# dongyangli-del/EEG_Image_decode

Hardware: AMD Instinct MI355X
Metric: EEG-CLIP contrastive train samples/sec (global batch) (higher is better)
Workload: dtype f32; 1 GPU; configs[1]: full ATM-S EEG encoder (63ch x 250t -> 1024-d) contrastive train step vs frozen 1024-d CLIP embeddings, 256 samples/GPU; global_batch=256, per_gpu_batch=256, parallelism=dp1, n_classes_for_accuracy=1654, optimizer=AdamW lr 3e-4 (fused)

## Files before the change

eeg_image_decode_amd/_abi.py:

```python
import ctypes as C

BIG = 1 << 62


class Dim(C.Structure):
    _fields_ = [("div", C.c_longlong), ("so", C.c_longlong), ("si", C.c_longlong)]


def dim(si, div=BIG, so=0):
    return Dim(int(div), int(so), int(si))


class GemmDesc(C.Structure):
    _fields_ = [
        ("M", C.c_int), ("N", C.c_int), ("K", C.c_int),
        ("A", C.c_void_p), ("Am", Dim), ("Ak", Dim),
        ("B", C.c_void_p), ("Bk", Dim), ("Bn", Dim),
        ("C", C.c_void_p), ("Cm", Dim), ("Cn", Dim),
        ("Cpre", C.c_void_p),
        ("bias_n", C.c_void_p), ("bias_m", C.c_void_p),
        ("R", C.c_void_p), ("Rm", Dim), ("Rn", Dim),
        ("alpha", C.c_float), ("accumulate", C.c_int), ("act", C.c_int),
        ("drop_p", C.c_float), ("seed", C.c_ulonglong), ("drop_site", C.c_uint),
        ("split_k", C.c_int),
        ("rowsum_a", C.c_void_p),
        ("precision", C.c_int),
        ("workspace", C.c_void_p), ("workspace_bytes", C.c_longlong),
    ]


class SplitItem(C.Structure):
    _fields_ = [("src", C.c_void_p), ("hi", C.c_void_p), ("lo", C.c_void_p), ("rows", C.c_int), ("cols", C.c_int), ("ld_src", C.c_longlong),
                ("ld_out", C.c_longlong), ("transpose", C.c_int), ("copy", C.c_void_p), ("ld_copy", C.c_longlong)]


class InfonceProblem(C.Structure):
    _fields_ = [("q_hi", C.c_void_p), ("q_lo", C.c_void_p), ("k_hi", C.c_void_p), ("k_lo", C.c_void_p), ("col0", C.c_int), ("weight", C.c_float),
                ("part", C.c_void_p), ("diag", C.c_void_p), ("lse", C.c_void_p), ("lse_k", C.c_void_p), ("G", C.c_void_p), ("ldg", C.c_longlong),
                ("part_k", C.c_void_p), ("diag_k", C.c_void_p), ("G_hi", C.c_void_p), ("G_lo", C.c_void_p)]


class TokenBlockDesc(C.Structure):
    _fields_ = ([("B", C.c_int), ("x", C.c_void_p), ("packed", C.c_void_p), ("bv", C.c_void_p), ("pe", C.c_void_p), ("tokens", C.c_void_p), ("ids", C.c_void_p)]
                + [(k, C.c_void_p) for k in ("bqkv", "bo", "ln1_g", "ln1_b", "b1", "b2", "ln2_g", "ln2_b", "ln3_g", "ln3_b")]
                + [(k, C.c_void_p) for k in ("h", "qkv", "r1", "mu1", "rs1", "f1", "r2", "n2", "mu2", "rs2", "n3", "mu3", "rs3")]
                + [(k, C.c_void_p) for k in ("xp", "hp", "ctxp", "n1p", "g1p")]
                + [("drop_p", C.c_float), ("eps", C.c_float), ("scale", C.c_float), ("seed", C.c_ulonglong)]
                + [(k, C.c_uint) for k in ("site_embed", "site_attn", "site_attn_out", "site_ffn_act", "site_ffn_out")]
                + [("packed_embed", C.c_void_p), ("embed_subject", C.c_void_p), ("bv_stride", C.c_longlong)]
                + [("cs_w25", C.c_void_p), ("cs_bias", C.c_void_p), ("cs_rows", C.c_void_p), ("cs_H", C.c_int)])


class TokenBlockBwdDesc(C.Structure):
    _fields_ = ([("B", C.c_int), ("packed", C.c_void_p)]
                + [(k, C.c_void_p) for k in ("dn3", "n2", "r2", "r1", "f1", "mu1", "rs1", "mu2", "rs2", "mu3", "rs3", "ln1_g", "ln2_g", "ln2_b", "ln3_g")]
                + [(k, C.c_void_p) for k in ("dr1", "dctx", "partials", "df2p", "dg1p", "da1p", "dr1p", "dqkvp")]
                + [(k, C.c_void_p) for k in ("dln3_g", "dln3_b", "dln2_g", "dln2_b", "dln1_g", "dln1_b")]
                + [("drop_p", C.c_float), ("seed", C.c_ulonglong)]
                + [(k, C.c_uint) for k in ("site_embed", "site_attn_out", "site_ffn_act", "site_ffn_out")])


class GemmPlanesDesc(C.Structure):
    _fields_ = [("a_hi", C.c_void_p), ("a_lo", C.c_void_p), ("b_hi", C.c_void_p), ("b_lo", C.c_void_p), ("lda", C.c_longlong), ("ldb", C.c_longlong),
                ("M", C.c_int), ("N", C.c_int), ("K", C.c_int), ("C", C.c_void_p), ("ldc", C.c_longlong), ("Cpre", C.c_void_p), ("ldcpre", C.c_longlong),
                ("bias", C.c_void_p), ("R", C.c_void_p), ("ldr", C.c_longlong), ("p_hi", C.c_void_p), ("p_lo", C.c_void_p), ("ldp", C.c_longlong),
                ("act", C.c_int), ("accumulate", C.c_int), ("planes_of", C.c_int)]


class HeadGemmDesc(C.Structure):
    _fields_ = [("a_hi", C.c_void_p), ("a_lo", C.c_void_p), ("b_hi", C.c_void_p), ("b_lo", C.c_void_p), ("lda", C.c_longlong), ("ldb", C.c_longlong),
                ("M", C.c_int), ("N", C.c_int), ("K", C.c_int), ("slices", C.c_int), ("slab_stride", C.c_longlong), ("bias", C.c_void_p),
                ("Cpre", C.c_void_p), ("ldcpre", C.c_longlong), ("act", C.c_int), ("aux", C.c_void_p), ("ldaux", C.c_longlong), ("R", C.c_void_p),
                ("ldr", C.c_longlong), ("C", C.c_void_p), ("ldc", C.c_longlong), ("p_hi", C.c_void_p), ("p_lo", C.c_void_p), ("ldp", C.c_longlong),
                ("b_kmajor", C.c_int)]


class Conv16Desc(C.Structure):
    _fields_ = [("in_", C.c_void_p), ("W", C.c_void_p), ("out", C.c_void_p), ("bias", C.c_void_p), ("residual", C.c_void_p),
                ("N", C.c_int), ("Hi", C.c_int), ("Wi", C.c_int), ("Cin", C.c_int), ("in_pad", C.c_int),
                ("Ho", C.c_int), ("Wo", C.c_int), ("Cout", C.c_int), ("out_pad", C.c_int),
                ("KS", C.c_int), ("stride", C.c_int), ("pad_top", C.c_int), ("pad_left", C.c_int), ("upsample", C.c_int), ("dtype", C.c_int),
                ("chan_bias", C.c_void_p)]


class Convt16Desc(C.Structure):
    _fields_ = [("in_", C.c_void_p), ("W", C.c_void_p), ("out", C.c_void_p), ("scale", C.c_void_p), ("shift", C.c_void_p),
                ("N", C.c_int), ("Hi", C.c_int), ("Wi", C.c_int), ("Cin", C.c_int), ("Ho", C.c_int), ("Wo", C.c_int), ("Cout", C.c_int),
                ("KS", C.c_int), ("stride", C.c_int), ("pad", C.c_int), ("relu", C.c_int), ("tap_mask", C.c_int), ("dtype", C.c_int)]


class Convt16BwdDataDesc(C.Structure):
    _fields_ = [("dz", C.c_void_p), ("W", C.c_void_p), ("dx", C.c_void_p), ("N", C.c_int), ("Hi", C.c_int), ("Wi", C.c_int), ("Cin", C.c_int), ("Cout", C.c_int),
                ("tap_mask", C.c_int), ("dtype", C.c_int)]


class Convt16BwdWeightDesc(C.Structure):
    _fields_ = [("x", C.c_void_p), ("dz", C.c_void_p), ("dW", C.c_void_p), ("db", C.c_void_p), ("workspace", C.c_void_p), ("workspace_floats", C.c_longlong),
                ("N", C.c_int), ("Hi", C.c_int), ("Wi", C.c_int), ("Cin", C.c_int), ("Cout", C.c_int), ("slabs", C.c_int), ("loss_scale", C.c_float),
                ("dtype", C.c_int)]


class Bn2d16FwdDesc(C.Structure):
    _fields_ = [("z", C.c_void_p), ("a", C.c_void_p), ("gamma", C.c_void_p), ("beta", C.c_void_p), ("mean", C.c_void_p), ("rstd", C.c_void_p),
                ("running_mean", C.c_void_p), ("running_var", C.c_void_p), ("workspace", C.c_void_p), ("workspace_floats", C.c_longlong), ("N", C.c_int), ("H", C.c_int), ("W", C.c_int), ("C", C.c_int),
                ("eps", C.c_float), ("momentum", C.c_float), ("dtype", C.c_int)]


class Bn2d16BwdDesc(C.Structure):
    _fields_ = [("da", C.c_void_p), ("a", C.c_void_p), ("z", C.c_void_p), ("gamma", C.c_void_p), ("mean", C.c_void_p), ("rstd", C.c_void_p), ("dgamma", C.c_void_p),
                ("dbeta", C.c_void_p), ("dz", C.c_void_p), ("workspace", C.c_void_p), ("workspace_floats", C.c_longlong), ("N", C.c_int), ("H", C.c_int), ("W", C.c_int), ("C", C.c_int),
                ("loss_scale", C.c_float), ("dtype", C.c_int)]


class WgradTokProblem(C.Structure):
    _fields_ = [("a", C.c_void_p), ("b", C.c_void_p), ("a_group_stride", C.c_longlong), ("m_groups", C.c_int), ("heads_m", C.c_int), ("heads_n", C.c_int),
                ("M", C.c_int), ("N", C.c_int), ("out", C.c_void_p), ("ldo", C.c_longlong), ("bias_out", C.c_void_p), ("bias_mfma", C.c_int),
                ("sample0", C.c_int), ("samples", C.c_int), ("sample_index", C.c_void_p)]


class CstackFwdDesc(C.Structure):
    _fields_ = [("B", C.c_int), ("H", C.c_int), ("x", C.c_void_p), ("xs_b", C.c_longlong), ("xs_h", C.c_longlong), ("w25", C.c_void_p), ("bias1", C.c_void_p),
                ("stat1", C.c_void_p), ("nstat1", C.c_int), ("count1", C.c_double), ("eps", C.c_float), ("momentum", C.c_float),
                ("gamma1", C.c_void_p), ("beta1", C.c_void_p), ("mean1", C.c_void_p), ("rstd1", C.c_void_p), ("run_mean1", C.c_void_p),
                ("run_var1", C.c_void_p), ("nbt1", C.c_void_p), ("packed", C.c_void_p), ("bias2", C.c_void_p), ("y2", C.c_void_p), ("stat2", C.c_void_p)]


class CstackBwdDesc(C.Structure):
    _fields_ = [("B", C.c_int), ("H", C.c_int), ("x", C.c_void_p), ("xs_b", C.c_longlong), ("xs_h", C.c_longlong), ("w25", C.c_void_p), ("bias1", C.c_void_p),
                ("mean1", C.c_void_p), ("rstd1", C.c_void_p), ("gamma1", C.c_void_p), ("beta1", C.c_void_p), ("packed_t", C.c_void_p), ("dy2", C.c_void_p),
                ("rows_out", C.c_void_p), ("stat", C.c_void_p), ("nstat", C.c_int), ("count", C.c_double), ("stat_local", C.c_void_p),
                ("nstat_local", C.c_int), ("dgamma", C.c_void_p), ("dbeta", C.c_void_p), ("dx", C.c_void_p), ("dw_partials", C.c_void_p), ("dw25", C.c_void_p)]


class WgradPlanesProblem(C.Structure):
    _fields_ = [("a_hi", C.c_void_p), ("a_lo", C.c_void_p), ("lda", C.c_longlong), ("b_hi", C.c_void_p), ("b_lo", C.c_void_p), ("ldb", C.c_longlong),
                ("rows", C.c_int), ("M", C.c_int), ("N", C.c_int), ("out", C.c_void_p), ("ldo", C.c_longlong), ("bias_out", C.c_void_p), ("slices", C.c_int)]


PLAN_MAX_ARGS = 28
PLAN_MEMSET, PLAN_JOIN, PLAN_SIDE, PLAN_SKIP, PLAN_SIDE2 = -2, -3, 1, 2, 4


class PlanArg(C.Union):
    _fields_ = [("p", C.c_void_p), ("i", C.c_longlong), ("u", C.c_ulonglong), ("d", C.c_double), ("f", C.c_float), ("i32", C.c_int), ("u32", C.c_uint)]


class PlanOp(C.Structure):
    _fields_ = [("fn", C.c_int), ("flags", C.c_int), ("a", PlanArg * PLAN_MAX_ARGS)]


ACT_NONE, ACT_GELU, ACT_SILU, ACT_GELU_GRAD = 0, 1, 2, 3
PREC_F32, PREC_BF16X3 = 0, 1
ABI_VERSION = 20
DT_BF16, DT_F16, DT_F32 = 0, 1, 2
SRC_U8_HWC, RESIZE_BILINEAR, RESIZE_BICUBIC = 3, 2, 3
_P, _I, _F, _L, _U64, _U, _D = C.c_void_p, C.c_int, C.c_float, C.c_longlong, C.c_ulonglong, C.c_uint, C.c_double

PROTOTYPES = {
    "eegclip_abi_version": [],
    "eegclip_gemm_f32": [C.POINTER(GemmDesc), _P],
    "eegclip_gemm_workspace_bytes": [C.POINTER(GemmDesc)],
    "eegclip_split_rows": [C.POINTER(SplitItem), _I, _P],
    "eegclip_gemm_f32_grouped": [_P, _I, _P],
    "eegclip_layernorm_fwd": [_P, _P, _P, _P, _P, _P, _I, _I, _F, _P],
    "eegclip_residual_layernorm_fwd": [_P, _P, _P, _F, _U64, _U, _P, _P, _P, _P, _P, _P, _P, _P, _P, _P, _I, _I, _F, _P],
    "eegclip_residual_layernorm_fwd_planes": [_P, _P, _P, _F, _U64, _U, _P, _P, _P, _P, _P, _P, _P, _P, _P, _P, _I, _I, _F, _P, _P, _P],
    "eegclip_layernorm_bwd": [_P, _P, _P, _P, _P, _P, _P, _P, _I, _I, _I, _P, _F, _U64, _U, _P],
    "eegclip_layernorm_bwd_full_workspace_floats": [_I, _I],
    "eegclip_layernorm_bwd_full": [_P, _P, _P, _P, _P, _P, _P, _P, _I, _I, _I, _P, _F, _U64, _U, _P, _P],
    "eegclip_layernorm_bwd_params_workspace_floats": [_I, _I],
    "eegclip_layernorm_bwd_params": [_P, _P, _P, _P, _P, _P, _I, _I, _P, _P],
    "eegclip_layernorm_silu_fwd": [_P, _P, _P, _P, _P, _P, _P, _I, _I, _F, _F, _U64, _U, _P],
    "eegclip_silu_bwd": [_P, _P, _P, _L, _I, _F, _U64, _U, _P],
    "eegclip_timestep_embedding": [_P, _I, _I, _P, _P],
    "eegclip_ddpm_add_noise": [_P, _P, _P, _P, _P, _P, _I, _I, _P],
    "eegclip_ddpm_step": [_P, _P, _P, _F, _F, _F, _F, _F, _F, _P, _P, _P, _L, _P],
    "eegclip_prior_stage_infer": [_P, _P, _P, _P, _P, _P, _P, _I, _P, _I, _I, _F, _P],
    "eegclip_mse_loss_grad": [_P, _P, _L, _P, _P, _P],
    "eegclip_mse_loss_grad_scaled": [_P, _P, _L, _F, _P, _P, _P],
    "eegclip_bn_stats": [_P, _I, _I, _I, _P, _P],
    "eegclip_bn_finalize": [_P, _D, _F, _F, _I, _P, _P, _P, _P, _I, _P, _P],
    "eegclip_bn_finalize_rows": [_P, _I, _D, _F, _F, _I, _P, _P, _P, _P, _P, _P, _P],
    "eegclip_bn_elu_fwd": [_P, _P, _P, _P, _P, _P, _I, _I, _I, _F, _U64, _U, _P],
    "eegclip_bn_elu_bwd": [_P, _P, _P, _P, _P, _P, _P, _P, _P, _P, _I, _I, _I, _F, _U64, _U, _P],
    "eegclip_bn_elu_bwd_stats": [_P, _P, _P, _P, _P, _P, _P, _I, _I, _I, _F, _U64, _U, _P],
    "eegclip_bn_elu_bwd_apply": [_P, _P, _P, _P, _P, _P, _P, _P, _D, _P, _P, _P, _I, _I, _I, _F, _U64, _U, _P],
    "eegclip_embed_finish": [_P, _P, _P, _I, _I, _I, _F, _U64, _U, _P],
    "eegclip_embed_finish_bwd": [_P, _P, _P, _I, _I, _I, _F, _U64, _U, _P],
    "eegclip_dropout_scale": [_P, _L, _F, _U64, _U, _P],
    "eegclip_gelu_bwd": [_P, _P, _P, _L, _I, _F, _U64, _U, _P],
    "eegclip_bias_act": [_P, _P, _P, _P, _P, _I, _I, _I, _F, _U64, _U, _P],
    "eegclip_axpby": [_P, _P, _L, _F, _F, _P],
    "eegclip_reduce_mid": [_P, _I, _I, _I, _P, _P],
    "eegclip_colsum_blocks": [_P, _I, _I, _I, _I, _L, _P, _P],
    "eegclip_sumsq": [_P, _L, _P, _P],
    "eegclip_stage_eeg": [_P, _P, _L, _I, _I, _I, _P, _I, _I, _P],
    "eegclip_gather_rows": [_P, _L, _P, _L, _P, _I, _I, _I, _P],
    "eegclip_adamw_step": [_P, _P, _P, _P, _L, _F, _F, _F, _F, _F, _L, _F, _P, _P],
    "eegclip_adamw_step_zero_grad": [_P, _P, _P, _P, _L, _F, _F, _F, _F, _F, _L, _F, _P, _P],
    "eegclip_clip_scale": [_P, _F, _P, _P],
    "eegclip_attention_fwd": [_P, _P, _I, _I, _I, _I, _I, _F, _F, _U64, _U, _P],
    "eegclip_attention_bwd": [_P, _P, _P, _I, _I, _I, _I, _I, _F, _F, _U64, _U, _P],
    "eegclip_attention_bwd_x3": [_P, _P, _P, _I, _I, _I, _I, _I, _I, _F, _F, _U64, _U, _P],
    "eegclip_proj1x1_fwd": [_P, _P, _P, _P, _P, _P, _P, _P, _P, _I, _F, _U64, _U, _P],
    "eegclip_proj1x1_fwd_rows": [_P, _P, _I, _D, _F, _F, _P, _P, _P, _P, _P, _P, _P, _P, _P, _P, _P, _I, _F, _U64, _U, _P],
    "eegclip_proj1x1_bwd_workspace_floats": [_I],
    "eegclip_proj1x1_bwd": [_P, _P, _P, _P, _P, _P, _P, _P, _P, _P, _P, _P, _P, _I, _F, _U64, _U, _P],
    "eegclip_cast_bf16": [_P, _P, _L, _P],
    "eegclip_logits_bf16": [_P, _P, _P, _I, _I, _I, _L, _P, _P],
    "eegclip_tsconv_fwd_workspace_floats": [_I, _I],
    "eegclip_tsconv_fwd": [_P, _L, _L, _P, _P, _P, _I, _I, _I, _I, _P, _P, _P],
    "eegclip_tsconv_bwd_w": [_P, _L, _L, _P, _P, _P, _I, _I, _I, _I, _P],
    "eegclip_tsconv_bwd_w_workspace_floats": [_I, _I],
    "eegclip_tsconv_bwd_x": [_P, _P, _P, _L, _L, _I, _I, _I, _I, _P],
    "eegclip_cross_attn_fwd": [_P, _P, _P, _P, _P, _P, _I, _I, _I, _I, _I, _I, _F, _I, _P],
    "eegclip_self_attn_supported": [_I, _L, _L, _L, _L],
    "eegclip_self_attn_fwd": [_P, _L, _P, _L, _P, _L, _P, _L, _I, _I, _I, _I, _I, _F, _I, _P],
    "eegclip_self_attn_causal_fwd": [_P, _L, _P, _L, _P, _L, _P, _L, _I, _I, _I, _I, _I, _F, _I, _P],
    "eegclip_self_attn_prefix_fwd": [_P, _L, _P, _L, _P, _L, _P, _L, _I, _I, _I, _I, _I, _F, _I, _P],
    "eegclip_attn80_supported": [_L, _L, _L, _L],
    "eegclip_attn80_fwd": [_P, _L, _P, _L, _P, _L, _P, _L, _I, _I, _I, _I, _F, _I, _P],
    "eegclip_gemm16_skinny": [_P, _L, _P, _L, _P, _L, _P, _P, _L, _I, _I, _I, _I, _I, _P],
    "eegclip_decode_attn16": [_P, _L, _P, _L, _L, _P, _L, _I, _I, _I, _I, _F, _I, _P],
    "eegclip_convt16": [C.POINTER(Convt16Desc), _P],
    "eegclip_convt16_pack_train": [_P, _P, _P, _I, _I, _I, _P],
    "eegclip_convt16_bwd_data": [C.POINTER(Convt16BwdDataDesc), _P],
    "eegclip_convt16_bwd_weight_slabs": [_I, _I, _I, _I, _I],
    "eegclip_convt16_bwd_weight_workspace_floats": [_I, _I, _I, _I, _I, _I],
    "eegclip_convt16_bwd_weight": [C.POINTER(Convt16BwdWeightDesc), _P],
    "eegclip_bn2d16_workspace_floats": [_I, _I, _I, _I],
    "eegclip_bn2d16_fwd": [C.POINTER(Bn2d16FwdDesc), _P],
    "eegclip_bn2d16_bwd": [C.POINTER(Bn2d16BwdDesc), _P],
    "eegclip_sconv_fwd": [_P, _P, _P, _P, _P, _P, _P, _P, _P, _I, _I, _I, _P, _P],
    "eegclip_sconv_fwd_workspace_floats": [_I],
    "eegclip_sconv_bwd_w_workspace_floats": [_I, _I],
    "eegclip_sconv_bwd_w": [_P, _P, _P, _P, _P, _P, _P, _P, _I, _I, _I, _P],
# ... 111 lines not shown
```

eeg_image_decode_amd/atms.py:

```python
import os
import weakref
import ctypes
import math

import numpy as np
import torch
import torch.nn as nn

from . import _abi
from ._lib import EegclipError, current_stream, lib, raw_stream, require_cuda
from .loss import ClipLoss
from .plan import Plan

D = _abi.dim
ACT_GELU = _abi.ACT_GELU
ACT_GELU_GRAD = _abi.ACT_GELU_GRAD

N_CH, T_LEN, D_MODEL, N_HEADS, D_HEAD, D_FF = 63, 250, 250, 4, 62, 256
L_TOK = N_CH + 1
HE = N_HEADS * D_HEAD
C_TS, W_TS, F_TS, P_DIM = 40, 36, 1440, 1024
EPS = 1e-5
SITE_EMBED, SITE_ATTN, SITE_ATTN_OUT, SITE_FFN_ACT, SITE_FFN_OUT, SITE_CONV, SITE_PROJ = range(7)

# ... 312 lines not shown
        self.n_subj = model.table_subjects if self.joint else 0
        self.ve_keys = [(_E + f"value_embedding.{s}.weight", _E + f"value_embedding.{s}.bias") for s in range(self.n_subj)]
        if self.joint:
            self.live_base = [k for k in _LIVE if ".value_embedding." not in k]
            live = self.live_base + [k for pair in self.ve_keys for k in pair]
        else:
            live = self.live_base = list(_LIVE)
        dead = [k for k in sd_params if k not in live and k not in (_TOK_TABLE, _TOK_SHARED)]
        order = live + [_TOK_TABLE, _TOK_SHARED] + dead
        assert sorted(order) == sorted(sd_params), "parameter list drifted from the reference state_dict"
        offs, off = {}, 0
        for k in order:
            offs[k] = off
            off += (sd_params[k].numel() + 3) // 4 * 4
        self.flat = torch.zeros(off, dtype=torch.float32, device=dev)
        self.gflat = torch.zeros(off, dtype=torch.float32, device=dev)
        self.anchor = torch.zeros(1, device=dev, requires_grad=True)
        self._clear_for = self._attached = None
        self._live_cache, self._attached_ptrs = {}, {}
        self.P, self.G, self.params = {}, {}, {}
        for k in order:
            p = sd_params[k]
            n = p.numel()
            view = self.flat[offs[k]:offs[k] + n].view(p.shape)
            view.copy_(p.data)
            p.data = view
            self.P[k] = view
            self.G[k] = self.gflat[offs[k]:offs[k] + n].view(p.shape)
            self.params[k] = p
            p._eegclip_grad_owner = weakref.ref(self)
        n_live = offs[_TOK_TABLE]
        self.segments = [(0, n_live, list(live)),
                         (offs[_TOK_TABLE], sd_params[_TOK_TABLE].numel(), [_TOK_TABLE]),
                         (offs[_TOK_SHARED], sd_params[_TOK_SHARED].numel(), [_TOK_SHARED]),
                         (offs[dead[0]] if dead else off, off - (offs[dead[0]] if dead else off), dead)]
        self.offs = offs
        a0, a1 = 0, offs["proj_eeg.2.bias"] + (sd_params["proj_eeg.2.bias"].numel() + 3) // 4 * 4
        assert offs["logit_scale"] == 0 and a1 == offs[self.live_base[self.live_base.index("proj_eeg.2.bias") + 1]]
        self.early_bucket = (a0, a1)
        self.early_work = None
        self._check = (self.params["logit_scale"], self.params[_CHECK_KEY])
        self.buffers = dict(model.named_buffers())
        self.bufs, self.plans, self.version = {}, {}, {}
        self.last_key = None
        self.grad_fresh = True
        lib()

    def _head_planes_enabled(self, pl):
        return pl.precision == _abi.PREC_BF16X3 and os.environ.get("EEGCLIP_HEAD_GEMM", "1") != "0"

    def _head_weight_planes(self):
        P = self.P
        w1, w2 = P["proj_eeg.0.weight"], P["proj_eeg.1.fn.1.weight"]
        span = (w2.data_ptr() - w1.data_ptr()) // 4 + w2.numel()
        assert w2.data_ptr() > w1.data_ptr() and span % 8 == 0 and span < 4 * w1.numel(), "projection-head weights are not adjacent in the flat buffer"
        if not hasattr(self, "hw_planes"):
            self.hw_planes = torch.empty(2, span, dtype=torch.bfloat16, device=self.device)
        o2 = (w2.data_ptr() - w1.data_ptr()) // 4
        self.hw = dict(w1=(_p(self.hw_planes[0]), _p(self.hw_planes[1])), w2=(_p(self.hw_planes[0]) + 2 * o2, _p(self.hw_planes[1]) + 2 * o2))
        return _abi.SplitItem(src=_p(w1), hi=_p(self.hw_planes[0]), lo=_p(self.hw_planes[1]), rows=1, cols=span, ld_src=span, ld_out=span, transpose=0)

    def _lean(self, pl, train, W):
        return bool(train and W == 1 and self._cstack_enabled(pl) and self._head_planes_enabled(pl))

    def _head_gemm(self, pl, b, tag, a_planes, K, w, N, B, kmajor=False):
        S = int(lib().eegclip_head_gemm_slices(B, N, K))
        if tag not in b or b[tag].shape != (S, B, N):
            b[tag] = torch.empty(S, B, N, dtype=torch.float32, device=self.device)
        pl.call_desc("eegclip_head_gemm", _abi.HeadGemmDesc(a_hi=a_planes[0], a_lo=a_planes[1], b_hi=w[0], b_lo=w[1], lda=K, ldb=N if kmajor else K, M=B, N=N, K=K,
                                                           slices=S, slab_stride=B * N, C=_p(b[tag]), ldc=N, b_kmajor=int(kmajor)))
        return _p(b[tag]), S, B * N

    def _token_block_enabled(self, pl):
        if self.joint and self.n_subj > WGRAD_TOK_MAX_PROBLEMS:
            return False
        return pl.precision == _abi.PREC_BF16X3 and os.environ.get("EEGCLIP_TOKEN_BLOCK", "1") != "0"

    def _token_planes(self, b, B, *names):
        for n in names:
            if n not in b:
                b[n] = torch.empty((3, B, 2, L_TOK, 256) if n == "dqkvp" else (B, 2, L_TOK, 256), dtype=torch.bfloat16, device=self.device)
        return [_p(b[n]) for n in names]

    def saved_f32(self, B, name):
        b = self.bufs[B]
        key = name + "p"
        if key not in b:
            return b[name]
        t = b[key].to(torch.float32)
        v = t[..., 0, :, :] + t[..., 1, :, :]
        if name in ("ctx", "dqkv"):
            v = v.reshape(*v.shape[:-1], N_HEADS, 64)[..., :D_HEAD].reshape(*v.shape[:-1], HE)
            if name == "dqkv":
                v = v.permute(1, 2, 0, 3).reshape(B * L_TOK, 3 * HE)
                return v
        else:
            v = v[..., :D_FF if name in ("g1", "dg1") else D_MODEL]
        return v.reshape(B * L_TOK, -1)

    def stale(self, model):
        a, b = self._check
        return (a.data_ptr() != self.flat.data_ptr() or b.data.data_ptr() != self.P[_CHECK_KEY].data_ptr()
                or model.logit_scale.device != self.device)

    def _alloc(self, B):
        dev = self.device

        def f(*s):
            return torch.empty(*s, dtype=torch.float32, device=dev)

        R = B * L_TOK
        b = dict(
            h=f(B, L_TOK, D_MODEL), qkv=f(R, 3 * HE), ctx=f(R, HE), r1=f(R, D_MODEL), n1=f(R, D_MODEL), mu1=f(R), rs1=f(R),
            f1=f(R, D_FF), g1=f(R, D_FF), r2=f(R, D_MODEL), n2=f(R, D_MODEL), mu2=f(R), rs2=f(R), n3=f(B, L_TOK, D_MODEL), mu3=f(R), rs3=f(R),
            z2=f(B, C_TS, W_TS),
            feat=f(B, F_TS), u=f(B, P_DIM), gu=f(B, P_DIM), s=f(B, P_DIM), out=f(B, P_DIM), mu4=f(B), rs4=f(B),
            bn=f(4, C_TS), ids=torch.zeros(B, dtype=torch.long, device=dev),
        )
        if self.joint:
            jmeta = torch.zeros(2 * B, dtype=torch.int32, device=dev)
            b.update(xs=f(B, N_CH, T_LEN), hs=f(B, L_TOK, D_MODEL), jmeta=jmeta, subj32=jmeta[:B], perm=jmeta[B:])
        nsum = 2 * 2 * C_TS
        ny2 = (B * C_TS * W_TS + 1) // 2
        nzf, nzb = nsum + B * P_DIM + ny2, nsum + (B * P_DIM + B * F_TS + 1) // 2
        zfb = torch.zeros(nzf + nzb, dtype=torch.float64, device=dev)
        zf, zb = zfb[:nzf], zfb[nzf:]
        sf, sb = zf[:nsum].view(2, 2 * C_TS), zb[:nsum].view(2, 2 * C_TS)
        zbf = zb[nsum:].view(torch.float32)
        b.update(zf=zf, zb=zb, zfb=zfb, zb_clean=True, sums=[sf[0], sf[1], sb[0], sb[1]], hacc=zf[nsum:nsum + B * P_DIM].view(torch.float32).view(2, B, P_DIM),
                 y2=zf[nsum + B * P_DIM:].view(torch.float32)[:B * C_TS * W_TS].view(B, C_TS, W_TS),
                 dgu=zbf[:B * P_DIM].view(B, P_DIM), dfeat=zbf[B * P_DIM:B * P_DIM + B * F_TS].view(B, F_TS))
        return b

    def _alloc_bwd(self, B, b):
        dev = self.device

        def f(*s):
            return torch.empty(*s, dtype=torch.float32, device=dev)

        R = B * L_TOK
        b.update(ds=f(B, P_DIM), dv=f(B, P_DIM), dz2=f(B, C_TS, W_TS), dy2=f(B, C_TS, W_TS),
                 dn3=torch.zeros(B, L_TOK, D_MODEL, dtype=torch.float32, device=dev),
                 dn2=f(R, D_MODEL), dr2=f(R, D_MODEL), df2=f(R, D_MODEL), dg1=f(R, D_FF), dr1=f(R, D_MODEL), da1=f(R, D_MODEL),
                 dctx=f(R, HE), dqkv=f(R, 3 * HE))

    def _build_fwd(self, B, train, shared, probs):
        P, b = self.P, self.bufs[B]
        pe_, pc_, pp_ = probs
        pl = Plan(f"atms_fwd[B={B}]")
        R = B * L_TOK
        pe = self.buffers[_E + "position_embedding.pe"]
        pl.tb_desc = None
        cstack = self._cstack_enabled(pl)
        head_planes = self._head_planes_enabled(pl)
        W = self._world() if train else 1
        lean = self._lean(pl, train, W)
        pl.lean = lean
        if cstack:
            if not lean:
                pl.memset(b["zfb"] if train else b["zf"], side=os.environ.get("EEGCLIP_START_SIDE", "1") != "0")
                pl.clears_zb = train
            if not hasattr(self, "cs_packed"):
                self.cs_packed = torch.empty(int(lib().eegclip_cstack_packed_bytes(N_CH)) // 2, dtype=torch.bfloat16, device=self.device)
                self.cs_packed_t = torch.empty(int(lib().eegclip_cstack_packed_t_bytes(N_CH)) // 2, dtype=torch.bfloat16, device=self.device)
            cs_prep = (_p(P[_TS + "4.weight"]), _p(self.cs_packed), _p(self.cs_packed_t), N_CH)
            if not self._token_block_enabled(pl):
                pl.call("eegclip_cstack_pack_all", *cs_prep)
        if self._token_block_enabled(pl):
            if not hasattr(self, "tb_packed"):
                self.tb_packed = torch.empty(int(lib().eegclip_token_block_packed_bytes()) // 2, dtype=torch.bfloat16, device=self.device)
            ve_w0, ve_b0 = (self.ve_keys[0] if self.joint else (_E + "value_embedding.weight", _E + "value_embedding.bias"))
            tb_prep = (_p(P[ve_w0]), _p(P[_LY + "attention.query_projection.weight"]), _p(P[_LY + "attention.out_projection.weight"]),
                       _p(P[_LY + "conv1.weight"]), _p(P[_LY + "conv2.weight"]), _p(self.tb_packed))
            if cstack:
                pl.call("eegclip_weight_prep", *tb_prep, *cs_prep)
            else:
                pl.call("eegclip_token_block_pack", *tb_prep)
            joint_args = {}
            if self.joint:
                ve_stride = (P[self.ve_keys[1][0]].data_ptr() - P[ve_w0].data_ptr()) // 4 if self.n_subj > 1 else D_MODEL * T_LEN
                assert all(P[w].data_ptr() - P[ve_w0].data_ptr() == 4 * ve_stride * i and P[bk].data_ptr() - P[ve_b0].data_ptr() == 4 * ve_stride * i
                           for i, (w, bk) in enumerate(self.ve_keys)), "value embeddings are not equally spaced in the flat buffer"
                if not hasattr(self, "tb_packed_embed"):
                    self.tb_packed_embed = torch.empty(int(lib().eegclip_token_block_packed_embed_bytes(self.n_subj)) // 2, dtype=torch.bfloat16,
                                                       device=self.device)
                pl.call("eegclip_token_block_pack_embed", _p(P[ve_w0]), ve_stride, self.n_subj, _p(self.tb_packed_embed))
                joint_args = dict(packed_embed=_p(self.tb_packed_embed), embed_subject=_p(b["subj32"]), bv_stride=ve_stride)
            tok = P[_TOK_SHARED] if shared else P[_TOK_TABLE]
            xp, hp, ctxp, n1p, g1p = self._token_planes(b, B, "xp", "hp", "ctxp", "n1p", "g1p")
            stats_args = {}
            pl.stats1_in_block = bool(cstack and train and os.environ.get("EEGCLIP_STATS1_TAIL", "1") != "0")
            if pl.stats1_in_block:
                if "cs_rows" not in b:
                    b["cs_rows"] = torch.empty(2, B, 2 * C_TS, dtype=torch.float64, device=self.device)
                stats_args = dict(cs_w25=_p(P[_TS + "0.weight"]), cs_bias=_p(P[_TS + "0.bias"]), cs_rows=_p(b["cs_rows"][0]), cs_H=N_CH)
            pl.tb_desc = pl.call_desc("eegclip_token_block_fwd", _abi.TokenBlockDesc(
                B=B, x=0, packed=_p(self.tb_packed), bv=_p(P[ve_b0]), pe=_p(pe), tokens=_p(tok), ids=None if shared else _p(b["ids"]), **joint_args, **stats_args,
                bqkv=_p(P[_LY + "attention.query_projection.bias"]), bo=_p(P[_LY + "attention.out_projection.bias"]), ln1_g=_p(P[_LY + "norm1.weight"]),
                ln1_b=_p(P[_LY + "norm1.bias"]), b1=_p(P[_LY + "conv1.bias"]), b2=_p(P[_LY + "conv2.bias"]), ln2_g=_p(P[_LY + "norm2.weight"]),
                ln2_b=_p(P[_LY + "norm2.bias"]), ln3_g=_p(P["encoder.encoder.norm.weight"]), ln3_b=_p(P["encoder.encoder.norm.bias"]),
                h=_p(b["h"]), qkv=_p(b["qkv"]), r1=_p(b["r1"]), mu1=_p(b["mu1"]), rs1=_p(b["rs1"]), f1=_p(b["f1"]),
                r2=_p(b["r2"]), n2=None, mu2=_p(b["mu2"]), rs2=_p(b["rs2"]), n3=_p(b["n3"]), mu3=_p(b["mu3"]), rs3=_p(b["rs3"]),
                xp=xp, hp=hp, ctxp=ctxp, n1p=n1p, g1p=g1p,
                drop_p=pe_, eps=EPS, scale=1.0 / math.sqrt(D_HEAD), seed=0, site_embed=SITE_EMBED, site_attn=SITE_ATTN, site_attn_out=SITE_ATTN_OUT,
                site_ffn_act=SITE_FFN_ACT, site_ffn_out=SITE_FFN_OUT), seeded=pe_ > 0.0)
        else:
            hmap = D(D_MODEL, div=N_CH, so=L_TOK * D_MODEL)
            if not self.joint:
                pl.x_gemm = pl.gemm(B * N_CH, D_MODEL, T_LEN, 0, D(T_LEN), D(1), _p(P[_E + "value_embedding.weight"]), D(1), D(T_LEN),
                        _p(b["h"]) + 4 * D_MODEL, hmap, D(1), bias_n=_p(P[_E + "value_embedding.bias"]),
                        R=_p(pe), Rm=D(D_MODEL, div=N_CH, so=0), Rn=D(1))
            else:
                XR = N_CH * T_LEN
                pl.j_gather = len(pl.ops)
                pl.call("eegclip_gather_rows", _p(b["xs"]), XR, 0, XR, _p(b["perm"]), B, XR, 0)
                pl.j_gemm = [pl.desc(N_CH, D_MODEL, T_LEN, 0, D(T_LEN), D(1), _p(P[w]), D(1), D(T_LEN), 0, hmap, D(1), bias_n=_p(P[bk]),
                                     R=_p(pe), Rm=D(D_MODEL, div=N_CH, so=0), Rn=D(1)) for w, bk in self.ve_keys]
                pl.j_arr, pl.j_group = pl.gemm_grouped(self.n_subj)
                pl.j_scatter = len(pl.ops)
                pl.call("eegclip_gather_rows", _p(b["h"]) + 4 * D_MODEL, L_TOK * D_MODEL, _p(b["hs"]) + 4 * D_MODEL, L_TOK * D_MODEL, _p(b["perm"]), B,
                        N_CH * D_MODEL, 1)
            tok = P[_TOK_SHARED] if shared else P[_TOK_TABLE]
            pl.call("eegclip_embed_finish", _p(b["h"]), _p(tok), None if shared else _p(b["ids"]), B, L_TOK, D_MODEL, pe_, 0, SITE_EMBED, seed_at=7)
            pl.gemm(R, 3 * HE, D_MODEL, _p(b["h"]), D(D_MODEL), D(1), _p(P[_LY + "attention.query_projection.weight"]), D(1), D(D_MODEL),
                    _p(b["qkv"]), D(3 * HE), D(1), bias_n=_p(P[_LY + "attention.query_projection.bias"]))
            pl.call("eegclip_attention_fwd", _p(b["qkv"]), _p(b["ctx"]), B, L_TOK, N_HEADS, D_HEAD, 3 * HE, 1.0 / math.sqrt(D_HEAD), pe_, 0,
                    SITE_ATTN, seed_at=9)
            pl.gemm(R, D_MODEL, HE, _p(b["ctx"]), D(HE), D(1), _p(P[_LY + "attention.out_projection.weight"]), D(1), D(HE),
                    _p(b["r1"]), D(D_MODEL), D(1), bias_n=_p(P[_LY + "attention.out_projection.bias"]))
            pl.call("eegclip_residual_layernorm_fwd", _p(b["r1"]), _p(b["h"]), _p(b["r1"]), pe_, 0, SITE_ATTN_OUT, _p(P[_LY + "norm1.weight"]),
                    _p(P[_LY + "norm1.bias"]), _p(b["n1"]), _p(b["mu1"]), _p(b["rs1"]), None, None, None, None, None, R, D_MODEL, EPS, seed_at=4)
            pl.gemm(R, D_FF, D_MODEL, _p(b["n1"]), D(D_MODEL), D(1), _p(P[_LY + "conv1.weight"]), D(1), D(D_MODEL), _p(b["g1"]), D(D_FF), D(1),
                    Cpre=_p(b["f1"]), bias_n=_p(P[_LY + "conv1.bias"]), act=ACT_GELU, drop_p=pe_, drop_site=SITE_FFN_ACT)
            pl.gemm(R, D_MODEL, D_FF, _p(b["g1"]), D(D_FF), D(1), _p(P[_LY + "conv2.weight"]), D(1), D(D_FF), _p(b["r2"]), D(D_MODEL), D(1),
                    bias_n=_p(P[_LY + "conv2.bias"]))
            pl.call("eegclip_residual_layernorm_fwd", _p(b["r2"]), _p(b["n1"]), _p(b["r2"]), pe_, 0, SITE_FFN_OUT, _p(P[_LY + "norm2.weight"]),
                    _p(P[_LY + "norm2.bias"]), _p(b["n2"]), _p(b["mu2"]), _p(b["rs2"]), _p(P["encoder.encoder.norm.weight"]),
                    _p(P["encoder.encoder.norm.bias"]), _p(b["n3"]), _p(b["mu3"]), _p(b["rs3"]), R, D_MODEL, EPS, seed_at=4)
        sums, bn = b["sums"], b["bn"]
        bn2_rows = None
        if cstack:
            if not lean:
                pl.join()
            bn2_rows = self._build_fwd_cstack(pl, b, B, train, W)
        else:
            pl.memset(b["zfb"] if train else b["zf"])
            pl.clears_zb = train
            self._build_fwd_conv_y1(pl, b, B, train, W)
        run2 = (_p(self.buffers[_TS + "5.running_mean"]), _p(self.buffers[_TS + "5.running_var"]), _p(self.buffers[_TS + "5.num_batches_tracked"]))
        if head_planes:
            if "featp" not in b:
                b["featp_buf"] = torch.zeros(2 * B * F_TS + 128, dtype=torch.bfloat16, device=self.device)
                b["featp"] = b["featp_buf"][:2 * B * F_TS].view(2, B, F_TS)
                b["gup"] = torch.empty(2, B, P_DIM, dtype=torch.bfloat16, device=self.device)
            rows_args = (_p(bn2_rows), B, float(B * W_TS), EPS, 0.1, _p(bn[2]), _p(bn[3]), *run2) if bn2_rows is not None else \
                (None, 0, 1.0, EPS, 0.1, _p(bn[2]), _p(bn[3]), None, None, None)
            pl.rider_items = (_abi.SplitItem * 4)()
            pl.rider_items[0] = self._head_weight_planes()
            pl._keep.append(pl.rider_items)
            pl.rider_op = len(pl.ops)
            pl.call("eegclip_proj1x1_fwd_rows_planes", _p(b["y2"]), *rows_args, _p(P[_TS + "5.weight"]), _p(P[_TS + "5.bias"]),
                    _p(P["enc_eeg.0.projection.0.weight"]), _p(P["enc_eeg.0.projection.0.bias"]), _p(b["z2"]), _p(b["feat"]), B, pc_, 0, SITE_CONV,
                    _p(b["featp"][0]), _p(b["featp"][1]), pl.rider_items, 1, seed_at=19)
        elif bn2_rows is not None:
            pl.call("eegclip_proj1x1_fwd_rows", _p(b["y2"]), _p(bn2_rows), B, float(B * W_TS), EPS, 0.1, _p(bn[2]), _p(bn[3]), *run2,
                    _p(P[_TS + "5.weight"]), _p(P[_TS + "5.bias"]), _p(P["enc_eeg.0.projection.0.weight"]), _p(P["enc_eeg.0.projection.0.bias"]),
                    _p(b["z2"]), _p(b["feat"]), B, pc_, 0, SITE_CONV, seed_at=19)
        else:
            pl.call("eegclip_proj1x1_fwd", _p(b["y2"]), _p(bn[2]), _p(bn[3]), _p(P[_TS + "5.weight"]), _p(P[_TS + "5.bias"]),
                    _p(P["enc_eeg.0.projection.0.weight"]), _p(P["enc_eeg.0.projection.0.bias"]), _p(b["z2"]), _p(b["feat"]), B, pc_, 0, SITE_CONV,
                    seed_at=11)
        pl.head_planes = head_planes
        if head_planes:
            fp, gp = (_p(b["featp"][0]), _p(b["featp"][1])), (_p(b["gup"][0]), _p(b["gup"][1]))
            fused_epi = os.environ.get("EEGCLIP_HEAD_FUSED_EPI", "0") == "1"
            if fused_epi:
                pl.call_desc("eegclip_head_gemm", _abi.HeadGemmDesc(a_hi=fp[0], a_lo=fp[1], b_hi=self.hw["w1"][0], b_lo=self.hw["w1"][1], lda=F_TS, ldb=F_TS, M=B,
                                                                   N=P_DIM, K=F_TS, slices=1, slab_stride=0, bias=_p(P["proj_eeg.0.bias"]), Cpre=_p(b["u"]),
                                                                   ldcpre=P_DIM, act=ACT_GELU, C=_p(b["gu"]), ldc=P_DIM, p_hi=gp[0], p_lo=gp[1], ldp=P_DIM))
            else:
                sl1 = self._head_gemm(pl, b, "hslab1", fp, F_TS, self.hw["w1"], P_DIM, B)
                pl.call("eegclip_head_act", *sl1, _p(P["proj_eeg.0.bias"]), _p(b["u"]), _p(b["gu"]), *gp, B, P_DIM)
            sl2 = self._head_gemm(pl, b, "hslab2", gp, P_DIM, self.hw["w2"], P_DIM, B)
            pl.out_op = len(pl.ops)
            pl.call("eegclip_residual_layernorm_fwd_slabs", sl2[0], _p(b["u"]), _p(b["s"]), pp_, 0, SITE_PROJ, _p(P["proj_eeg.2.weight"]),
                    _p(P["proj_eeg.2.bias"]), 0, _p(b["mu4"]), _p(b["rs4"]), None, None, None, None, None, B, P_DIM, EPS, None, None, sl2[1], sl2[2],
                    _p(P["proj_eeg.1.fn.1.bias"]), seed_at=4)
            return pl
        skh = _head_split(B)
        if skh > 1:
            pl.gemm(B, P_DIM, F_TS, _p(b["feat"]), D(F_TS), D(1), _p(P["proj_eeg.0.weight"]), D(1), D(F_TS), _p(b["hacc"][0]), D(P_DIM), D(1),
                    accumulate=1, split_k=skh)
            pl.call("eegclip_bias_act", _p(b["hacc"][0]), _p(P["proj_eeg.0.bias"]), _p(b["u"]), None, _p(b["gu"]), B, P_DIM, ACT_GELU, 0.0, 0, 0)
            pl.gemm(B, P_DIM, P_DIM, _p(b["gu"]), D(P_DIM), D(1), _p(P["proj_eeg.1.fn.1.weight"]), D(1), D(P_DIM), _p(b["hacc"][1]), D(P_DIM), D(1),
                    bias_n=_p(P["proj_eeg.1.fn.1.bias"]), accumulate=1, split_k=skh)
            w_lin = b["hacc"][1]
        else:
            pl.gemm(B, P_DIM, F_TS, _p(b["feat"]), D(F_TS), D(1), _p(P["proj_eeg.0.weight"]), D(1), D(F_TS), _p(b["gu"]), D(P_DIM), D(1),
                    Cpre=_p(b["u"]), bias_n=_p(P["proj_eeg.0.bias"]), act=ACT_GELU)
            pl.gemm(B, P_DIM, P_DIM, _p(b["gu"]), D(P_DIM), D(1), _p(P["proj_eeg.1.fn.1.weight"]), D(1), D(P_DIM), _p(b["s"]), D(P_DIM), D(1),
                    bias_n=_p(P["proj_eeg.1.fn.1.bias"]))
            w_lin = b["s"]
        pl.out_op = len(pl.ops)
        pl.call("eegclip_residual_layernorm_fwd", _p(w_lin), _p(b["u"]), _p(b["s"]), pp_, 0, SITE_PROJ, _p(P["proj_eeg.2.weight"]),
                _p(P["proj_eeg.2.bias"]), 0, _p(b["mu4"]), _p(b["rs4"]), None, None, None, None, None, B, P_DIM, EPS, seed_at=4)
        return pl
# ... 126 lines not shown
                pl.call_desc("eegclip_head_gemm", _abi.HeadGemmDesc(a_hi=vp[0], a_lo=vp[1], b_hi=self.hw["w2"][0], b_lo=self.hw["w2"][1], lda=P_DIM, ldb=P_DIM, M=B,
                                                                   N=P_DIM, K=P_DIM, slices=1, slab_stride=0, act=ACT_GELU_GRAD, aux=_p(b["u"]), ldaux=P_DIM,
                                                                   R=_p(b["ds"]), ldr=P_DIM, C=_p(b["ds"]), ldc=P_DIM, p_hi=up[0], p_lo=up[1], ldp=P_DIM, b_kmajor=1))
            else:
                sl = self._head_gemm(pl, b, "dgu_slabs", vp, P_DIM, self.hw["w2"], P_DIM, B, kmajor=True)
                pl.call("eegclip_head_act_bwd", *sl, _p(b["u"]), _p(b["ds"]), _p(b["ds"]), *up, B * P_DIM)
            if wplanes:
                gp_, fp_ = (_p(b["gup"][0]), _p(b["gup"][1])), (_p(b["featp"][0]), _p(b["featp"][1]))
                probs = (_abi.WgradPlanesProblem * 2)(
                    _abi.WgradPlanesProblem(a_hi=vp[0], a_lo=vp[1], lda=P_DIM, b_hi=gp_[0], b_lo=gp_[1], ldb=P_DIM, rows=B, M=P_DIM, N=P_DIM,
                                            out=_p(G["proj_eeg.1.fn.1.weight"]), ldo=P_DIM, bias_out=_p(G["proj_eeg.1.fn.1.bias"]), slices=1),
                    _abi.WgradPlanesProblem(a_hi=up[0], a_lo=up[1], lda=P_DIM, b_hi=fp_[0], b_lo=fp_[1], ldb=F_TS, rows=B, M=P_DIM, N=F_TS,
                                            out=_p(G["proj_eeg.0.weight"]), ldo=F_TS, bias_out=_p(G["proj_eeg.0.bias"]), slices=1))
                pl._keep.append(probs)
                later(lambda: pl.call("eegclip_wgrad_planes", probs, 2, side=head_side))
            else:
                later(lambda: wgrad("proj_eeg.0.weight", _p(b["ds"]), P_DIM, _p(b["feat"]), F_TS, P_DIM, F_TS, B, bias="proj_eeg.0.bias"))
            dfeat_slabs = self._head_gemm(pl, b, "dfeat_slabs", up, P_DIM, self.hw["w1"], F_TS, B, kmajor=True)
        else:
            head_side_ops = []
            self._build_bwd_head_f32(pl, b, B, pp_, ln_side, wgrad)
        W = self._world() if train else 1
        zsum = None
        if not train:
            zsum = torch.zeros(2 * C_TS, dtype=torch.float64, device=self.device)
            pl._keep.append(zsum)

            def conv_bias_grad(bias_key, gamma_key, rstd, s):
                return lambda: G[bias_key].add_((P[gamma_key] * rstd * s[:C_TS].to(torch.float32)))
        if "pj_ws" not in b:
            b["pj_ws"] = torch.empty(int(lib().eegclip_proj1x1_bwd_workspace_floats(B)) // 2, dtype=torch.float64, device=self.device)
        lean = dfeat_slabs is not None and self._lean(pl, train, W)
        pl.lean = lean
        if lean:
            if "pj_bn_rows" not in b:
                b["pj_bn_rows"] = torch.empty(B, 2 * C_TS, dtype=torch.float64, device=self.device)
            pl.call("eegclip_proj1x1_bwd_rows", *dfeat_slabs, _p(b["z2"]), _p(P["enc_eeg.0.projection.0.weight"]), _p(b["y2"]), _p(bn[2]), _p(bn[3]),
                    _p(P[_TS + "5.weight"]), _p(P[_TS + "5.bias"]), _p(b["dz2"]), _p(b["pj_ws"]), _p(b["pj_bn_rows"]), B, pc_, 0, SITE_CONV, seed_at=15)
            pl.call("eegclip_bn_elu_bwd_apply_rows", _p(b["dz2"]), _p(b["y2"]), _p(bn[2]), _p(bn[3]), _p(P[_TS + "5.weight"]), _p(P[_TS + "5.bias"]),
                    _p(b["pj_bn_rows"]), B, 2 * C_TS, 0, float(B * W_TS),
                    _p(b["dy2"]), _p(G[_TS + "5.weight"]), _p(G[_TS + "5.bias"]), B, C_TS, W_TS, pc_, 0, SITE_CONV, seed_at=18)
            for f in head_side_ops:
                f()
            pl.call("eegclip_proj1x1_bwd_reduce", _p(b["pj_ws"]), B, _p(G["enc_eeg.0.projection.0.weight"]), _p(G["enc_eeg.0.projection.0.bias"]), None, side=True)
        else:
            if dfeat_slabs is not None:
                pl.call("eegclip_proj1x1_bwd_slabs", *dfeat_slabs, _p(b["z2"]), _p(P["enc_eeg.0.projection.0.weight"]), _p(b["y2"]), _p(bn[2]), _p(bn[3]),
                        _p(P[_TS + "5.weight"]), _p(P[_TS + "5.bias"]), _p(b["dz2"]), _p(G["enc_eeg.0.projection.0.weight"]),
                        _p(G["enc_eeg.0.projection.0.bias"]), _p(sums[2]), _p(b["pj_ws"]), B, pc_, 0, SITE_CONV, seed_at=17)
            else:
                pl.call("eegclip_proj1x1_bwd", _p(b["dfeat"]), _p(b["z2"]), _p(P["enc_eeg.0.projection.0.weight"]), _p(b["y2"]), _p(bn[2]), _p(bn[3]),
                        _p(P[_TS + "5.weight"]), _p(P[_TS + "5.bias"]), _p(b["dz2"]), _p(G["enc_eeg.0.projection.0.weight"]),
                        _p(G["enc_eeg.0.projection.0.bias"]), _p(sums[2]), _p(b["pj_ws"]), B, pc_, 0, SITE_CONV, seed_at=15)
            local2 = None
            if W > 1:
                local2 = torch.zeros_like(sums[2])
                pl._keep.append(local2)

                def exchange2():
                    local2.copy_(sums[2])
                    self._allreduce(sums[2])
                pl.callback(exchange2, "allreduce_bn2_bwd")
            if not train:
                pl.callback(conv_bias_grad(_TS + "4.bias", _TS + "5.weight", bn[3], sums[2]), "conv2_bias_grad_eval")
            pl.call("eegclip_bn_elu_bwd_apply", _p(b["dz2"]), _p(b["y2"]), _p(bn[2]), _p(bn[3]), _p(P[_TS + "5.weight"]), _p(P[_TS + "5.bias"]),
                    _p(sums[2]) if train else _p(zsum), (_p(local2) if local2 is not None else None) if train else _p(sums[2]), float(W * B * W_TS), _p(b["dy2"]), _p(G[_TS + "5.weight"]), _p(G[_TS + "5.bias"]), B, C_TS,
                    W_TS, pc_, 0, SITE_CONV, seed_at=16)
            for f in head_side_ops:
                f()
        if self._cstack_bwd_enabled(pl):
            self._build_bwd_cstack(pl, b, B, train, W, zsum, conv_bias_grad if not train else None, early_reduce, defer_small)
        else:
            self._build_bwd_conv_y1(pl, b, B, train, W, zsum, conv_bias_grad if not train else None, early_reduce)
        fused = self._token_block_enabled(pl) and hasattr(self, "tb_packed")
        if fused:
            if "tb_part" not in b:
                b["tb_part"] = torch.empty(int(lib().eegclip_token_block_bwd_workspace_floats(B)), dtype=torch.float32, device=self.device)
            df2p, dg1p, da1p, dr1p, dqkvp = self._token_planes(b, B, "df2p", "dg1p", "da1p", "dr1p", "dqkvp")
            xp, hp, ctxp, n1p, g1p = self._token_planes(b, B, "xp", "hp", "ctxp", "n1p", "g1p")
            bd = _abi.TokenBlockBwdDesc(
                B=B, packed=_p(self.tb_packed), dn3=_p(b["dn3"]), n2=None, r2=_p(b["r2"]), r1=_p(b["r1"]), f1=_p(b["f1"]), mu1=_p(b["mu1"]),
                rs1=_p(b["rs1"]), mu2=_p(b["mu2"]), rs2=_p(b["rs2"]), mu3=_p(b["mu3"]), rs3=_p(b["rs3"]), ln1_g=_p(P[_LY + "norm1.weight"]),
                ln2_g=_p(P[_LY + "norm2.weight"]), ln2_b=_p(P[_LY + "norm2.bias"]), ln3_g=_p(P["encoder.encoder.norm.weight"]),
                dr1=_p(b["dr1"]), dctx=_p(b["dctx"]), partials=_p(b["tb_part"]), df2p=df2p, dg1p=dg1p, da1p=da1p, dr1p=dr1p, dqkvp=dqkvp,
                dln3_g=_p(G["encoder.encoder.norm.weight"]), dln3_b=_p(G["encoder.encoder.norm.bias"]), dln2_g=_p(G[_LY + "norm2.weight"]),
                dln2_b=_p(G[_LY + "norm2.bias"]), dln1_g=_p(G[_LY + "norm1.weight"]), dln1_b=_p(G[_LY + "norm1.bias"]),
                drop_p=pe_, seed=0, site_embed=SITE_EMBED, site_attn_out=SITE_ATTN_OUT, site_ffn_act=SITE_FFN_ACT, site_ffn_out=SITE_FFN_OUT)
            pl._keep.append(bd)
            if pe_ > 0.0:
                pl._seed_descs.append(bd)
            variant = 0

            def wgrad_tok(tag, problems, side=True, slices=None, index=None):
                arr = (_abi.WgradTokProblem * len(problems))()
                for i, (name, a, mg, x, M, N, hm, hn, bias, bm) in enumerate(problems):
                    arr[i] = _abi.WgradTokProblem(a=a, b=x, a_group_stride=B * 65536 if mg > 1 else 0, m_groups=mg, heads_m=hm, heads_n=hn, M=M, N=N,
                                                  out=_p(G[name]), ldo=N, bias_out=_p(G[bias]) if bias else None, bias_mfma=bm, sample_index=index)
                groups = sum(q[2] for q in problems)
                slices = slices or (wsk if wsk > 0 else int(lib().eegclip_wgrad_tok_slices(groups, B)))
                key = "wk:" + tag
                if key not in b:
                    b[key] = torch.empty(int(lib().eegclip_wgrad_tok_workspace_floats(arr, len(problems), B, slices)), dtype=torch.float32, device=self.device)
                pl._keep.append(arr)
                ops = (len(pl.ops), len(pl.ops) + 1)
                pl.call("eegclip_wgrad_tok", arr, len(problems), B, slices, _p(b[key]), variant, side=side)
                pl.call("eegclip_wgrad_tok_reduce", arr, len(problems), B, slices, _p(b[key]), side=side)
                return arr, ops

            merge = int(os.environ.get("EEGCLIP_WGRAD_MERGE", "2"))
            late = []
            ffn_out = [
                (_LY + "conv2.weight", df2p, 1, g1p, D_MODEL, D_FF, 0, 0, _LY + "conv2.bias", 1),
                (_LY + "conv1.weight", dg1p, 1, n1p, D_FF, D_MODEL, 0, 0, _LY + "conv1.bias", 0),
                (_LY + "attention.out_projection.weight", da1p, 1, ctxp, D_MODEL, HE, 0, 1, _LY + "attention.out_projection.bias", 0)]
            qkv_w = [(_LY + "attention.query_projection.weight", dqkvp, 3, hp, 3 * HE, D_MODEL, 1, 0, _LY + "attention.query_projection.bias", 0)]
            pl.call("eegclip_token_block_bwd", ctypes.byref(bd), 0)
            if defer_small:
                pl.deferred.append(lambda: pl.call("eegclip_token_block_bwd", ctypes.byref(bd), 2, side=True))
            else:
                pl.call("eegclip_token_block_bwd", ctypes.byref(bd), 2, side=ln_side)
            if merge >= 2:
                late += ffn_out
            else:
                wgrad_tok("ffn_out", ffn_out)
            pl.call(attn_bwd, _p(b["qkv"]), _p(b["dctx"]), dqkvp, 1, B, L_TOK, N_HEADS, D_HEAD, 3 * HE, 1.0 / math.sqrt(D_HEAD),
                    pe_, 0, SITE_ATTN, seed_at=11)
            if merge >= 1:
                late += qkv_w
            else:
                wgrad_tok("qkv", qkv_w)
            pl.call("eegclip_token_block_bwd", ctypes.byref(bd), 1)
        else:
            pl.call("eegclip_layernorm_bwd_full", _p(b["dn3"]), _p(b["n2"]), _p(P["encoder.encoder.norm.weight"]), _p(b["mu3"]), _p(b["rs3"]), _p(b["dn2"]),
                    _p(G["encoder.encoder.norm.weight"]), _p(G["encoder.encoder.norm.bias"]), R, D_MODEL, 0, None, 0.0, 0, 0, lnf_ws)
            pl.call("eegclip_layernorm_bwd_full", _p(b["dn2"]), _p(b["r2"]), _p(P[_LY + "norm2.weight"]), _p(b["mu2"]), _p(b["rs2"]), _p(b["dr2"]),
                    _p(G[_LY + "norm2.weight"]), _p(G[_LY + "norm2.bias"]), R, D_MODEL, 0, _p(b["df2"]), pe_, 0, SITE_FFN_OUT, lnf_ws, seed_at=13)
            wgrad(_LY + "conv2.weight", _p(b["df2"]), D_MODEL, _p(b["g1"]), D_FF, D_MODEL, D_FF, R, bias=_LY + "conv2.bias")
            pl.gemm(R, D_FF, D_MODEL, _p(b["df2"]), D(D_MODEL), D(1), _p(P[_LY + "conv2.weight"]), D(D_FF), D(1), _p(b["dg1"]), D(D_FF), D(1),
                    act=ACT_GELU_GRAD, R=_p(b["f1"]), Rm=D(D_FF), Rn=D(1), drop_p=pe_, drop_site=SITE_FFN_ACT)
            wgrad(_LY + "conv1.weight", _p(b["dg1"]), D_FF, _p(b["n1"]), D_MODEL, D_FF, D_MODEL, R, bias=_LY + "conv1.bias")
            pl.gemm(R, D_MODEL, D_FF, _p(b["dg1"]), D(D_FF), D(1), _p(P[_LY + "conv1.weight"]), D(D_MODEL), D(1), _p(b["dr2"]), D(D_MODEL), D(1),
                    accumulate=1)
            pl.call("eegclip_layernorm_bwd_full", _p(b["dr2"]), _p(b["r1"]), _p(P[_LY + "norm1.weight"]), _p(b["mu1"]), _p(b["rs1"]), _p(b["dr1"]),
                    _p(G[_LY + "norm1.weight"]), _p(G[_LY + "norm1.bias"]), R, D_MODEL, 0, _p(b["da1"]), pe_, 0, SITE_ATTN_OUT, lnf_ws, seed_at=13)
            wgrad(_LY + "attention.out_projection.weight", _p(b["da1"]), D_MODEL, _p(b["ctx"]), HE, D_MODEL, HE, R,
                  bias=_LY + "attention.out_projection.bias")
            pl.gemm(R, HE, D_MODEL, _p(b["da1"]), D(D_MODEL), D(1), _p(P[_LY + "attention.out_projection.weight"]), D(HE), D(1), _p(b["dctx"]), D(HE), D(1))
            if attn_bwd == "eegclip_attention_bwd_x3":
                pl.call(attn_bwd, _p(b["qkv"]), _p(b["dctx"]), _p(b["dqkv"]), 0, B, L_TOK, N_HEADS, D_HEAD, 3 * HE, 1.0 / math.sqrt(D_HEAD),
                        pe_, 0, SITE_ATTN, seed_at=11)
            else:
                pl.call(attn_bwd, _p(b["qkv"]), _p(b["dctx"]), _p(b["dqkv"]), B, L_TOK, N_HEADS, D_HEAD, 3 * HE, 1.0 / math.sqrt(D_HEAD),
                        pe_, 0, SITE_ATTN, seed_at=10)
            wgrad(_LY + "attention.query_projection.weight", _p(b["dqkv"]), 3 * HE, _p(b["h"]), D_MODEL, 3 * HE, D_MODEL, R,
                  bias=_LY + "attention.query_projection.bias")
            pl.gemm(R, D_MODEL, 3 * HE, _p(b["dqkv"]), D(3 * HE), D(1), _p(P[_LY + "attention.query_projection.weight"]), D(D_MODEL), D(1),
                    _p(b["dr1"]), D(D_MODEL), D(1), accumulate=2, drop_p=pe_, drop_site=SITE_EMBED)
        tokg = G[_TOK_SHARED] if shared else G[_TOK_TABLE]
        pl.call("eegclip_embed_finish_bwd", _p(b["dr1"]), _p(tokg), None if shared else _p(b["ids"]), B, L_TOK, D_MODEL, 0.0, 0, SITE_EMBED, side=True)
        for f in pl.deferred:
            f()
        hmap = D(D_MODEL, div=N_CH, so=L_TOK * D_MODEL)
        if want_dx:
            b["dx"] = torch.empty(B, N_CH, T_LEN, dtype=torch.float32, device=self.device)
        pl.x_gemm = None
        if fused:
            if not self.joint:
                wgrad_tok("embed" + ("+%d" % len(late) if late else ""), late + [(_E + "value_embedding.weight", dr1p, 1, xp, D_MODEL, T_LEN, 0, 0, _E + "value_embedding.bias", 0)], side=False)
            else:
                if late:
                    wgrad_tok("block", late, side=False)
                pl.j_wk_template = [(w, dr1p, 1, xp, D_MODEL, T_LEN, 0, 0, bk, 0) for w, bk in self.ve_keys]
                pl.j_wk_slices = [0] + [max(1, min(32, 2 * B // 4, (64 // n) // 8 * 8 if 64 // n >= 8 else 64 // n)) for n in range(1, self.n_subj + 1)]
                pl.j_wk_arr, pl.j_wk_ops = wgrad_tok("embed_joint", pl.j_wk_template, side=False, slices=8, index=_p(b["perm"]))
                need = max(int(lib().eegclip_wgrad_tok_workspace_floats(pl.j_wk_arr, n, B, pl.j_wk_slices[n])) for n in range(1, self.n_subj + 1))
                if b["wk:embed_joint"].numel() < need:
                    b["wk:embed_joint"] = torch.empty(need, dtype=torch.float32, device=self.device)
                    for op in pl.j_wk_ops:
                        pl.set_arg(op, 4, _p(b["wk:embed_joint"]))
                pl.j_wk_all = (_abi.WgradTokProblem * self.n_subj)(*pl.j_wk_arr)
                pl._keep.append(pl.j_wk_all)
        elif not self.joint:
            pl.x_gemm = pl.gemm(D_MODEL, T_LEN, B * N_CH, _p(b["dr1"]) + 4 * D_MODEL, D(1), hmap, 0, D(T_LEN), D(1),
                    _p(G[_E + "value_embedding.weight"]), D(T_LEN), D(1), accumulate=1, split_k=sk(B * N_CH),
                    rowsum_a=_p(G[_E + "value_embedding.bias"]))
        if not self.joint:
            if want_dx:
                pl.gemm(B * N_CH, T_LEN, D_MODEL, _p(b["dr1"]) + 4 * D_MODEL, hmap, D(1),
                        _p(P[_E + "value_embedding.weight"]), D(T_LEN), D(1), _p(b["dx"]), D(T_LEN), D(1))
        elif fused and not want_dx:
            pass
        else:
            XR = N_CH * T_LEN
            pl.j_gather = len(pl.ops)
            pl.call("eegclip_gather_rows", _p(b["hs"]) + 4 * D_MODEL, L_TOK * D_MODEL, _p(b["dr1"]) + 4 * D_MODEL, L_TOK * D_MODEL, _p(b["perm"]), B,
                    N_CH * D_MODEL, 0)
            if not fused:
                pl.j_gemm = [pl.desc(D_MODEL, T_LEN, N_CH, 0, D(1), hmap, 0, D(T_LEN), D(1), _p(G[w]), D(T_LEN), D(1), accumulate=1, split_k=1,
                                     rowsum_a=_p(G[bk])) for w, bk in self.ve_keys]
                pl.j_arr, pl.j_group = pl.gemm_grouped(self.n_subj)
            if want_dx:
                b["dxs"] = torch.empty(B, N_CH, T_LEN, dtype=torch.float32, device=self.device)
                pl.j_dx = [pl.desc(N_CH, T_LEN, D_MODEL, 0, hmap, D(1), _p(P[w]), D(T_LEN), D(1), 0, D(T_LEN), D(1)) for w, _ in self.ve_keys]
                pl.j_dx_arr, pl.j_dx_group = pl.gemm_grouped(self.n_subj)
                pl.j_scatter = len(pl.ops)
                pl.call("eegclip_gather_rows", _p(b["dx"]), XR, _p(b["dxs"]), XR, _p(b["perm"]), B, XR, 1)
        return pl

    def _build_bwd_head_f32(self, pl, b, B, pp_, ln_side, wgrad):
        P, G = self.P, self.G
        pl.call("eegclip_layernorm_bwd", 0, _p(b["s"]), _p(P["proj_eeg.2.weight"]), _p(b["mu4"]), _p(b["rs4"]), _p(b["ds"]),
                None, None, B, P_DIM, 0, _p(b["dv"]), pp_, 0, SITE_PROJ, seed_at=13)
        pl.dout_par_op = len(pl.ops)
        pl.call("eegclip_layernorm_bwd", 0, _p(b["s"]), None, _p(b["mu4"]), _p(b["rs4"]), None,
                _p(G["proj_eeg.2.weight"]), _p(G["proj_eeg.2.bias"]), B, P_DIM, 0, None, 0.0, 0, 0, side=ln_side)
        wgrad("proj_eeg.1.fn.1.weight", _p(b["dv"]), P_DIM, _p(b["gu"]), P_DIM, P_DIM, P_DIM, B, bias="proj_eeg.1.fn.1.bias")
        skh = _head_split(B)
        pl.gemm(B, P_DIM, P_DIM, _p(b["dv"]), D(P_DIM), D(1), _p(P["proj_eeg.1.fn.1.weight"]), D(P_DIM), D(1), _p(b["dgu"]), D(P_DIM), D(1),
                accumulate=int(skh > 1), split_k=skh)
        pl.call("eegclip_gelu_bwd", _p(b["dgu"]), _p(b["u"]), _p(b["ds"]), B * P_DIM, 1, 0.0, 0, 0)
        wgrad("proj_eeg.0.weight", _p(b["ds"]), P_DIM, _p(b["feat"]), F_TS, P_DIM, F_TS, B, bias="proj_eeg.0.bias")
        pl.gemm(B, F_TS, P_DIM, _p(b["ds"]), D(P_DIM), D(1), _p(P["proj_eeg.0.weight"]), D(F_TS), D(1), _p(b["dfeat"]), D(F_TS), D(1),
                accumulate=int(skh > 1), split_k=skh)

    def _build_bwd_cstack(self, pl, b, B, train, W, zsum, conv_bias_grad, early_reduce, defer_small=False):
# ... 275 lines not shown
```

eeg_image_decode_amd/csrc/attention_x3.hip:

```cpp
#include "eeg_common.h"

namespace eeg {

constexpr int AX_L = 64;
constexpr int AX_RS = 144;
constexpr int AX_PLANE = AX_L * AX_RS;
constexpr int AX_TENSOR = 2 * AX_PLANE;

struct ax_args {
    const float* qkv;
    const float* dctx;
    float* dqkv;
    unsigned char* dqkvp;
    int B, H, E, ld;
    float scale, drop_p;
    unsigned long long seed;
    unsigned site;
};

typedef float ax_f2 __attribute__((ext_vector_type(2)));
typedef float ax_f4u __attribute__((ext_vector_type(4), aligned(4)));

__device__ __forceinline__ bf16x8 ax_tr_frag(const unsigned char* plane, int r0, int r1, int c0, int lane) {
    const int l = lane & 15;
    const s16x4 a = lds_read_tr16(plane + (r0 + (l >> 2)) * AX_RS + 2 * (c0 + 4 * (l & 3)));
    const s16x4 b = lds_read_tr16(plane + (r1 + (l >> 2)) * AX_RS + 2 * (c0 + 4 * (l & 3)));
    return bf16x8{a[0], a[1], a[2], a[3], b[0], b[1], b[2], b[3]};
}
__device__ __forceinline__ bf16x8 ax_frag(const unsigned char* plane, int row, int k0) {
    return *reinterpret_cast<const bf16x8*>(plane + row * AX_RS + 2 * k0);
}
__device__ __forceinline__ bf16x8 ax_pack8(u32x2_t a, u32x2_t b) {
    typedef unsigned u4 __attribute__((ext_vector_type(4)));
    const u4 v{a[0], a[1], b[0], b[1]};
    return __builtin_bit_cast(bf16x8, v);
}
__device__ __forceinline__ f32x4 ax_mfma3(bf16x8 ah, bf16x8 al, bf16x8 bh, bf16x8 bl, f32x4 c) {
    c = mfma_bf16_16x16x32(al, bh, c);
    c = mfma_bf16_16x16x32(ah, bl, c);
    return mfma_bf16_16x16x32(ah, bh, c);
}
__device__ __forceinline__ void ax_store4(float* p, int valid, f32x4 v) {
    if (valid >= 4) *reinterpret_cast<ax_f4u*>(p) = ax_f4u{v[0], v[1], v[2], v[3]};
    else if (valid >= 2) {
        *reinterpret_cast<ax_f2*>(p) = ax_f2{v[0], v[1]};
        if (valid == 3) p[2] = v[2];
    } else if (valid == 1) p[0] = v[0];
}

__device__ __forceinline__ void ax_store4_planes(unsigned char* row_base, int e0, f32x4 v) {
    u32x2_t hi, lo;
    x3_split4(v[0], v[1], v[2], v[3], hi, lo);
    *reinterpret_cast<u32x2_t*>(row_base + 2 * e0) = hi;
    *reinterpret_cast<u32x2_t*>(row_base + 32768 + 2 * e0) = lo;
}

template <bool TRAIN>
__global__ __launch_bounds__(256, 2) void attention_bwd_x3_kernel(const ax_args a) {
    EEG_LDS_BASE(float, ldsf);
    unsigned char* lds = reinterpret_cast<unsigned char*>(ldsf);
    unsigned char* Qp = lds;
    unsigned char* Kp = lds + AX_TENSOR;
    unsigned char* Vp = lds + 2 * AX_TENSOR;
    unsigned char* Op = lds + 3 * AX_TENSOR;
    const int t = threadIdx.x, lane = t & 63, w = wave_uniform(t >> 6), fr = lane & 15, g = lane >> 4;
    const int bh = blockIdx.x, b = bh / a.H, h = bh - b * a.H;
    const int E = a.E, HE = a.H * E;
    const float* qrow0 = a.qkv + (long long)b * AX_L * a.ld + h * E;
    const float* orow0 = a.dctx + (long long)b * AX_L * HE + h * E;

    {
        ax_f2 v[4][8];
#pragma unroll
        for (int j = 0; j < 8; ++j) {
            const int idx = t + 256 * j, row = idx >> 5, col = 2 * (idx & 31);
            const bool ok = col < E;
            const float* qr = qrow0 + (long long)row * a.ld + col;
            v[0][j] = ok ? *reinterpret_cast<const ax_f2*>(qr) : ax_f2{0.f, 0.f};
            v[1][j] = ok ? *reinterpret_cast<const ax_f2*>(qr + HE) : ax_f2{0.f, 0.f};
            v[2][j] = ok ? *reinterpret_cast<const ax_f2*>(qr + 2 * HE) : ax_f2{0.f, 0.f};
            v[3][j] = ok ? *reinterpret_cast<const ax_f2*>(orow0 + (long long)row * HE + col) : ax_f2{0.f, 0.f};
        }
#pragma unroll
        for (int x = 0; x < 4; ++x)
#pragma unroll
            for (int j = 0; j < 8; ++j) {
                const int idx = t + 256 * j, row = idx >> 5, col = 2 * (idx & 31);
                const unsigned hi = x3_pack2(v[x][j][0], v[x][j][1]);
                const float r0 = v[x][j][0] - __uint_as_float(hi << 16), r1 = v[x][j][1] - __uint_as_float(hi & 0xffff0000u);
                unsigned char* dst = lds + x * AX_TENSOR + row * AX_RS + 2 * col;
                *reinterpret_cast<unsigned*>(dst) = hi;
                *reinterpret_cast<unsigned*>(dst + AX_PLANE) = x3_pack2(r0, r1);
            }
    }
    __syncthreads();

    f32x4 s[4], dp[4];
#pragma unroll
    for (int kt = 0; kt < 4; ++kt) { s[kt] = f32x4{0.f, 0.f, 0.f, 0.f}; dp[kt] = f32x4{0.f, 0.f, 0.f, 0.f}; }
#pragma unroll
    for (int ks = 0; ks < 2; ++ks) {
        const int k0 = 32 * ks + 8 * g;
        const bf16x8 qh = ax_frag(Qp, 16 * w + fr, k0), ql = ax_frag(Qp + AX_PLANE, 16 * w + fr, k0);
        const bf16x8 oh = ax_frag(Op, 16 * w + fr, k0), ol = ax_frag(Op + AX_PLANE, 16 * w + fr, k0);
#pragma unroll
        for (int kt = 0; kt < 4; ++kt) {
            const bf16x8 kh = ax_frag(Kp, 16 * kt + fr, k0), kl = ax_frag(Kp + AX_PLANE, 16 * kt + fr, k0);
            const bf16x8 vh = ax_frag(Vp, 16 * kt + fr, k0), vl = ax_frag(Vp + AX_PLANE, 16 * kt + fr, k0);
            s[kt] = ax_mfma3(kh, kl, qh, ql, s[kt]);
            dp[kt] = ax_mfma3(vh, vl, oh, ol, dp[kt]);
        }
    }
    float mx = -INFINITY;
#pragma unroll
    for (int kt = 0; kt < 4; ++kt)
#pragma unroll
        for (int r = 0; r < 4; ++r) {
            s[kt][r] *= a.scale;
            mx = fmaxf(mx, s[kt][r]);
        }
    mx = fmaxf(mx, __shfl_xor(mx, 16, 64));
    mx = fmaxf(mx, __shfl_xor(mx, 32, 64));
    float sum = 0.f;
#pragma unroll
    for (int kt = 0; kt < 4; ++kt)
#pragma unroll
        for (int r = 0; r < 4; ++r) {
            s[kt][r] = expf(s[kt][r] - mx);
            sum += s[kt][r];
        }
    sum += __shfl_xor(sum, 16, 64);
    sum += __shfl_xor(sum, 32, 64);
    const float inv = 1.0f / sum;
    const bool drop = TRAIN && a.drop_p > 0.f;
    const float ksc = drop ? 1.f / (1.f - a.drop_p) : 1.f;
    f32x4 pd[4];
    float dq_sum = 0.f;
#pragma unroll
    for (int kt = 0; kt < 4; ++kt) {
        bool keep[4] = {true, true, true, true};
        if (drop) {
            const unsigned long long idx0 = ((unsigned long long)bh * AX_L + 16 * w + fr) * AX_L + 16 * kt + 4 * g;
            dropout_keep4(a.seed, a.site, idx0, a.drop_p, keep);
        }
#pragma unroll
        for (int r = 0; r < 4; ++r) {
            const float p = s[kt][r] * inv;
            const float d = keep[r] ? dp[kt][r] * ksc : 0.f;
            pd[kt][r] = keep[r] ? p * ksc : 0.f;
            s[kt][r] = p;
            dp[kt][r] = d;
            dq_sum += p * d;
        }
    }
    dq_sum += __shfl_xor(dq_sum, 16, 64);
    dq_sum += __shfl_xor(dq_sum, 32, 64);
#pragma unroll
    for (int kt = 0; kt < 4; ++kt)
#pragma unroll
        for (int r = 0; r < 4; ++r) dp[kt][r] = s[kt][r] * (dp[kt][r] - dq_sum);

    {
        f32x4 dq[4];
#pragma unroll
        for (int et = 0; et < 4; ++et) dq[et] = f32x4{0.f, 0.f, 0.f, 0.f};
#pragma unroll
        for (int m = 0; m < 2; ++m) {
            u32x2_t h0, l0, h1, l1;
            x3_split4(dp[2 * m][0], dp[2 * m][1], dp[2 * m][2], dp[2 * m][3], h0, l0);
            x3_split4(dp[2 * m + 1][0], dp[2 * m + 1][1], dp[2 * m + 1][2], dp[2 * m + 1][3], h1, l1);
            const bf16x8 bhf = ax_pack8(h0, h1), blf = ax_pack8(l0, l1);
#pragma unroll
            for (int et = 0; et < 4; ++et) {
                const bf16x8 ah = ax_tr_frag(Kp, 32 * m + 4 * g, 32 * m + 16 + 4 * g, 16 * et, lane);
                const bf16x8 al = ax_tr_frag(Kp + AX_PLANE, 32 * m + 4 * g, 32 * m + 16 + 4 * g, 16 * et, lane);
                dq[et] = ax_mfma3(ah, al, bhf, blf, dq[et]);
            }
        }
        float* out = a.dqkv + ((long long)b * AX_L + 16 * w + fr) * a.ld + h * E;
        unsigned char* outp = a.dqkvp + (long long)b * 65536 + (16 * w + fr) * 512 + 128 * h;
#pragma unroll
        for (int et = 0; et < 4; ++et) {
            const int e0 = 16 * et + 4 * g;
            f32x4 v = dq[et];
#pragma unroll
            for (int r = 0; r < 4; ++r) v[r] *= a.scale;
            if (a.dqkvp) ax_store4_planes(outp, e0, v);
            else if (e0 < E) ax_store4(out + e0, E - e0, v);
        }
    }
    __syncthreads();
#pragma unroll
    for (int kt = 0; kt < 4; ++kt) {
        u32x2_t hi, lo;
        const int off = (16 * w + fr) * AX_RS + 2 * (16 * kt + 4 * g);
        x3_split4(pd[kt][0], pd[kt][1], pd[kt][2], pd[kt][3], hi, lo);
        *reinterpret_cast<u32x2_t*>(Kp + off) = hi;
        *reinterpret_cast<u32x2_t*>(Kp + AX_PLANE + off) = lo;
        x3_split4(dp[kt][0], dp[kt][1], dp[kt][2], dp[kt][3], hi, lo);
        *reinterpret_cast<u32x2_t*>(Vp + off) = hi;
        *reinterpret_cast<u32x2_t*>(Vp + AX_PLANE + off) = lo;
    }
    __syncthreads();

    f32x4 dv[4], dk[4];
#pragma unroll
    for (int et = 0; et < 4; ++et) { dv[et] = f32x4{0.f, 0.f, 0.f, 0.f}; dk[et] = f32x4{0.f, 0.f, 0.f, 0.f}; }
#pragma unroll
    for (int ks = 0; ks < 2; ++ks) {
        const int q0 = 32 * ks + 8 * g;
        const bf16x8 ph = ax_tr_frag(Kp, q0, q0 + 4, 16 * w, lane), pl = ax_tr_frag(Kp + AX_PLANE, q0, q0 + 4, 16 * w, lane);
        const bf16x8 sh = ax_tr_frag(Vp, q0, q0 + 4, 16 * w, lane), sl = ax_tr_frag(Vp + AX_PLANE, q0, q0 + 4, 16 * w, lane);
#pragma unroll
        for (int et = 0; et < 4; ++et) {
            const bf16x8 oh = ax_tr_frag(Op, q0, q0 + 4, 16 * et, lane), ol = ax_tr_frag(Op + AX_PLANE, q0, q0 + 4, 16 * et, lane);
            const bf16x8 qh = ax_tr_frag(Qp, q0, q0 + 4, 16 * et, lane), ql = ax_tr_frag(Qp + AX_PLANE, q0, q0 + 4, 16 * et, lane);
            dv[et] = ax_mfma3(oh, ol, ph, pl, dv[et]);
            dk[et] = ax_mfma3(qh, ql, sh, sl, dk[et]);
        }
    }
    if (a.dqkvp) {
        const long long grp = (long long)a.B * 65536;
        unsigned char* outp = a.dqkvp + (long long)b * 65536 + (16 * w + fr) * 512 + 128 * h;
#pragma unroll
        for (int et = 0; et < 4; ++et) {
            const int e0 = 16 * et + 4 * g;
            f32x4 v = dk[et];
#pragma unroll
            for (int r = 0; r < 4; ++r) v[r] *= a.scale;
            ax_store4_planes(outp + grp, e0, v);
            ax_store4_planes(outp + 2 * grp, e0, dv[et]);
        }
        return;
    }
    float* outk = a.dqkv + ((long long)b * AX_L + 16 * w + fr) * a.ld + HE + h * E;
#pragma unroll
    for (int et = 0; et < 4; ++et) {
        const int e0 = 16 * et + 4 * g;
        if (e0 < E) {
            f32x4 v = dk[et];
#pragma unroll
            for (int r = 0; r < 4; ++r) v[r] *= a.scale;
            ax_store4(outk + e0, E - e0, v);
            ax_store4(outk + HE + e0, E - e0, dv[et]);
        }
    }
}

}

using namespace eeg;

extern "C" int eegclip_attention_bwd_x3(const float* qkv, const float* dctx, void* dqkv, int dqkv_planes, int B, int L, int H, int E, int ld, float scale,
                                        float drop_p, unsigned long long seed, unsigned site, void* stream) {
    if (dqkv_planes && (H > 4 || (reinterpret_cast<uintptr_t>(dqkv) & 15u))) return dqkv && H <= 4 ? EEGCLIP_EALIGN : EEGCLIP_EINVAL;
    if (!qkv || !dctx || !dqkv || B < 1 || L != AX_L || H < 1 || E < 2 || E > 64 || (E & 1) || (ld & 1) || ld < 3 * H * E || drop_p < 0.f || drop_p >= 1.f)
        return EEGCLIP_EINVAL;
    if ((reinterpret_cast<uintptr_t>(qkv) | reinterpret_cast<uintptr_t>(dctx) | reinterpret_cast<uintptr_t>(dqkv)) & 7u) return EEGCLIP_EALIGN;
    const ax_args a{qkv, dctx, dqkv_planes ? nullptr : static_cast<float*>(dqkv), dqkv_planes ? static_cast<unsigned char*>(dqkv) : nullptr, B, H, E, ld, scale,
                    drop_p, seed, site};
    const size_t lds = 4 * AX_TENSOR;
    if (drop_p > 0.f) EEG_LAUNCH(attention_bwd_x3_kernel<true>, dim3(B * H), dim3(256), lds, stream, a);
    else              EEG_LAUNCH(attention_bwd_x3_kernel<false>, dim3(B * H), dim3(256), lds, stream, a);
    return (int)hipGetLastError();
}
```

eeg_image_decode_amd/csrc/token_block.hip:

```cpp
#include "cstack_common.h"

#include <stdio.h>
#include <stdlib.h>

namespace eeg {

constexpr int TB_THREADS = 512;
constexpr int TB_L = 64, TB_D = 250, TB_T = 250, TB_NCH = 63, TB_H = 4, TB_E = 62, TB_HE = 248, TB_FF = 256;
constexpr int TB_AP_PLANE = 64 * 512;
constexpr int TB_AP_BYTES = 2 * TB_AP_PLANE;
constexpr int TB_XF_BYTES = 64 * 1024;
constexpr int TB_HQ_PLANE = 64 * 128;
constexpr int TB_HQ_BYTES = 6 * TB_HQ_PLANE;
constexpr int TB_LDS = TB_AP_BYTES + 2 * TB_HQ_BYTES;
constexpr int TB_KS = 8;
constexpr int TB_TILE = 1024;
constexpr int TB_NT_V = 16, TB_NT_QKV = 48, TB_NT_O = 16, TB_NT_1 = 16, TB_NT_2 = 16;
constexpr int TB_NMAT = 11;
constexpr long long TB_OFF_V = 0;
constexpr long long TB_OFF_QKV = TB_OFF_V + (long long)TB_NT_V * TB_KS * TB_TILE;
constexpr long long TB_OFF_O = TB_OFF_QKV + (long long)TB_NT_QKV * TB_KS * TB_TILE;
constexpr long long TB_OFF_1 = TB_OFF_O + (long long)TB_NT_O * TB_KS * TB_TILE;
constexpr long long TB_OFF_2 = TB_OFF_1 + (long long)TB_NT_1 * TB_KS * TB_TILE;
constexpr long long TB_MAT_ELEMS = 16LL * TB_KS * TB_TILE;
// ... 128 lines not shown

template <int NT, unsigned TM, int PF = 2, bool ZERO = true, class PRE = tb_none, class NEXT = tb_none, bool RING = true>
__device__ __forceinline__ void tb_gemm(const unsigned char* AP, const unsigned short* wp, int lane, f32x4 (&acc)[4][NT], PRE& pre, const unsigned short* wpn,
                                        NEXT& nxt) {
    constexpr bool HAS_PRE = tb_frag_nt<PRE>::nt != 0;
    constexpr int NTN = tb_frag_nt<NEXT>::nt;
    static_assert(!HAS_PRE || tb_frag_nt<PRE>::nt == NT, "the carried fragments are this GEMM's");
    const int fr = lane & 15, g = lane >> 4;
    if (ZERO) {
#pragma unroll
        for (int mt = 0; mt < 4; ++mt)
#pragma unroll
            for (int j = 0; j < NT; ++j) acc[mt][j] = f32x4{0.f, 0.f, 0.f, 0.f};
    }
    bf16x8 bh[PF + 1][NT], bl[PF + 1][NT];
    auto issue = [&](int ks) {
        const int slot = ks % (PF + 1);
#pragma unroll
        for (int j = 0; j < NT; ++j) tb_load_frag<RING>(bh[slot][j], bl[slot][j], reinterpret_cast<const bf16x8*>(wp + (long long)(j * TB_KS + ks) * TB_TILE) + lane);
    };
    if constexpr (HAS_PRE) {
#pragma unroll
        for (int p = 0; p < PF; ++p)
#pragma unroll
            for (int j = 0; j < NT; ++j) { bh[p][j] = pre.h[p][j]; bl[p][j] = pre.l[p][j]; }
    } else {
#pragma unroll
        for (int p = 0; p < PF; ++p) issue(p);
    }
#pragma unroll
    for (int ks = 0; ks < TB_KS; ++ks) {
        const int cur = ks % (PF + 1);
        int younger = 0;
        if (ks + PF < TB_KS) {
            issue(ks + PF);
            younger = 2 * NT * PF;
        } else {
            younger = 2 * NT * (TB_KS - 1 - ks);
            if constexpr (NTN != 0) {
                tb_request(wpn, lane, ks + PF - TB_KS, nxt);
                younger += 2 * NTN * (ks + PF - TB_KS + 1);
            }
        }
        if (RING && !(HAS_PRE && ks < PF)) tb_wait_frags<NT>(younger, bh[cur], bl[cur]);
        bf16x8 ah[4], al[4];
#pragma unroll
        for (int mt = 0; mt < 4; ++mt) {
            const int off = (16 * mt + fr) * 512 + (((4 * ks + g) ^ fr) << 4);
            ah[mt] = *reinterpret_cast<const bf16x8*>(AP + off);
            al[mt] = *reinterpret_cast<const bf16x8*>(AP + TB_AP_PLANE + off);
        }
#pragma unroll
        for (int pr = 0; pr < 3; ++pr)
#pragma unroll
            for (int j = 0; j < NT; ++j)
#pragma unroll
                for (int mt = 0; mt < 4; ++mt) {
                    const bf16x8 bw = pr == 0 ? bl[cur][j] : bh[cur][j];
                    const bf16x8 aw = pr == 1 ? al[mt] : ah[mt];
                    if ((TM >> j) & 1u) acc[mt][j] = mfma_bf16_16x16x32(bw, aw, acc[mt][j]);
                    else acc[mt][j] = mfma_bf16_16x16x32(aw, bw, acc[mt][j]);
                }
    }
}
template <int NT, unsigned TM, int PF = 2, bool ZERO = true>
__device__ __forceinline__ void tb_gemm(const unsigned char* AP, const unsigned short* wp, int lane, f32x4 (&acc)[4][NT]) {
    tb_none none;
    tb_gemm<NT, TM, PF, ZERO>(AP, wp, lane, acc, none, nullptr, none);
}

__device__ __forceinline__ void tb_store_planes4(unsigned char* hi_plane, int plane_stride, int off, float v0, float v1, float v2, float v3) {
    u32x2_t h, l;
    x3_split4(v0, v1, v2, v3, h, l);
    *reinterpret_cast<u32x2_t*>(hi_plane + off) = h;
    *reinterpret_cast<u32x2_t*>(hi_plane + plane_stride + off) = l;
}
__device__ __forceinline__ void tb_store_planes2(unsigned char* hi_plane, int plane_stride, int off, float v0, float v1) {
    const unsigned h = x3_pack2(v0, v1);
    const float r0 = v0 - __uint_as_float(h << 16), r1 = v1 - __uint_as_float(h & 0xffff0000u);
    *reinterpret_cast<unsigned*>(hi_plane + off) = h;
    *reinterpret_cast<unsigned*>(hi_plane + plane_stride + off) = x3_pack2(r0, r1);
}

__device__ __forceinline__ f32x4 tb_ld4(const float* p, int valid) {
    if (valid >= 4) {
        const tb_f4u t = *reinterpret_cast<const tb_f4u*>(p);
        return f32x4{t[0], t[1], t[2], t[3]};
    }
    const tb_f2 t = *reinterpret_cast<const tb_f2*>(p);
    return f32x4{t[0], t[1], 0.f, 0.f};
}
__device__ __forceinline__ void tb_st4(float* p, int valid, f32x4 v) {
    if (valid >= 4) *reinterpret_cast<tb_f4u*>(p) = tb_f4u{v[0], v[1], v[2], v[3]};
    else *reinterpret_cast<tb_f2*>(p) = tb_f2{v[0], v[1]};
}


template <int ONES_FROM>
__device__ __forceinline__ void tb_planes_out(const unsigned char* AP, unsigned char* dst, int t) {
    const unsigned lds_off = (unsigned)((t >> 5) * 512 + (((t & 31) ^ (t >> 5)) << 4)), g_off = (unsigned)t * 16u;
#pragma unroll
    for (int half = 0; half < 2; ++half) {
        tb_u4 v[4];
#pragma unroll
        for (int j = 0; j < 4; ++j) {
            v[j] = *reinterpret_cast<const tb_u4*>(AP + half * TB_AP_PLANE + j * 8192 + lds_off);
            if (ONES_FROM < 64 && half == 0 && (t & 31) == 31 && (ONES_FROM == 0 || j > 0 || (t >> 5) >= ONES_FROM)) v[j][3] = (v[j][3] & 0xffffu) | 0x3F800000u;
        }
#pragma unroll
        for (int j = 0; j < 4; ++j) *reinterpret_cast<tb_u4*>(dst + (half * 4 + j) * 8192 + g_off) = v[j];
    }
}

struct tb_fwd_args {
    const float* x;
    const unsigned short* packed;
    const float *bv, *pe, *tokens;
    const long long* ids;
    const float *bqkv, *bo, *ln1_g, *ln1_b, *b1, *b2, *ln2_g, *ln2_b, *ln3_g, *ln3_b;
    float *h, *qkv, *r1, *mu1, *rs1, *f1, *r2, *n2, *mu2, *rs2, *n3, *mu3, *rs3;
    unsigned char *xp, *hp, *ctxp, *n1p, *g1p;
    float drop_p, eps, scale;
    unsigned long long seed;
    unsigned site_embed, site_attn, site_attn_out, site_ffn_act, site_ffn_out;
    unsigned dbg;
    unsigned long long* tstamp;
    const unsigned short* packed_embed;
    const int* embed_subject;
    long long bv_stride;
    const float *cs_w25, *cs_bias;
    double* cs_rows;
    int cs_H;
};

template <class ARGS>
__device__ __forceinline__ ARGS tb_args_again(const ARGS& a) {
#if defined(EEG_EMU) || !defined(__HIP_DEVICE_COMPILE__)
    return a;
#else
    auto p = (const __attribute__((address_space(4))) ARGS*)__builtin_amdgcn_kernarg_segment_ptr();
    asm volatile("" : "+s"(p));
    return *p;
#endif
}

__device__ __forceinline__ void tb_stamp(const tb_fwd_args& a, int b, int t, int k) {
#if !defined(EEG_EMU)
    if (a.tstamp && t == 0) a.tstamp[b * 16 + k] = __builtin_amdgcn_s_memtime();
#endif
}

template <bool TRANS>
__device__ __forceinline__ void tb_qkv_tile_out(const tb_fwd_args& a, int b, int head, int which, int tt, int lane, f32x4 bias, f32x4 (&v)[4]) {
    const int fr = lane & 15, g = lane >> 4;
    const int cbase = which * TB_HE + head * TB_E;
    if (TRANS) {
        const int d0 = 16 * tt + 4 * g, valid = TB_E - d0;
#pragma unroll
        for (int mt = 0; mt < 4; ++mt) {
            const int m = 16 * mt + fr;
#pragma unroll
            for (int i = 0; i < 4; ++i) v[mt][i] = i < valid ? v[mt][i] + bias[i] : 0.f;
            if (!(a.dbg & 1u)) tb_st4(a.qkv + (long long)b * (TB_L * 3 * TB_HE) + (unsigned)(m * (3 * TB_HE) + cbase + d0), valid, v[mt]);
        }
    } else {
        const int d = 16 * tt + fr;
#pragma unroll
        for (int mt = 0; mt < 4; ++mt)
#pragma unroll
            for (int i = 0; i < 4; ++i) {
                v[mt][i] = d < TB_E ? v[mt][i] + bias[0] : 0.f;
                if (d < TB_E && !(a.dbg & 1u)) (a.qkv + (long long)b * (TB_L * 3 * TB_HE))[(unsigned)((16 * mt + 4 * g + i) * (3 * TB_HE) + cbase + d)] = v[mt][i];
            }
    }
}
template <bool TRANS>
__device__ __forceinline__ void tb_qkv_tile_lds(unsigned char* HQ, int which, int tt, int lane, const f32x4 (&v)[4]) {
    const int fr = lane & 15, g = lane >> 4;
    unsigned char* base = HQ + which * (2 * TB_HQ_PLANE);
#pragma unroll
    for (int mt = 0; mt < 4; ++mt) {
        const int off = TRANS ? hq_off(16 * mt + fr, 16 * tt + 4 * g) : hq_off(16 * tt + fr, 16 * mt + 4 * g);
        tb_store_planes4(base, TB_HQ_PLANE, off, v[mt][0], v[mt][1], v[mt][2], v[mt][3]);
    }
}

template <int V>
struct tb_qkv_variant {
    static constexpr unsigned mask = V == 0 ? 7u : V == 1 ? 7u : V == 2 ? 3u : 0u;
};

template <int V, class PRE, class NEXT>
__device__ __forceinline__ void tb_qkv_pass(const tb_fwd_args& a, const unsigned char* AP, int b, int head, int lane, f32x4 (&acc)[4][3], PRE& pre,
                                            const unsigned short* wpn, NEXT& nxt) {
    tb_gemm<3, tb_qkv_variant<V>::mask, 2, true>(AP, a.packed + TB_OFF_QKV + (long long)(head * 12 + 3 * V) * TB_KS * TB_TILE, lane, acc, pre, wpn, nxt);
    const int fr = lane & 15, g = lane >> 4;
    f32x4 bias[3];
#pragma unroll
    for (int jj = 0; jj < 3; ++jj) {
        const int j = 3 * V + jj, which = j >> 2, tt = j & 3, cbase = which * TB_HE + head * TB_E;
        if ((tb_qkv_variant<V>::mask >> jj) & 1u) {
            const int d0 = 16 * tt + 4 * g;
            bias[jj] = tb_ld4(a.bqkv + cbase + d0, TB_E - d0 >= 4 ? 4 : 2);
        } else {
            const int d = 16 * tt + fr;
            const float bv = d < TB_E ? a.bqkv[cbase + d] : 0.f;
            bias[jj] = f32x4{bv, bv, bv, bv};
        }
    }
    tb_retire(nxt);
#pragma unroll
    for (int jj = 0; jj < 3; ++jj) {
        const int j = 3 * V + jj, which = j >> 2, tt = j & 3;
        f32x4 v[4] = {acc[0][jj], acc[1][jj], acc[2][jj], acc[3][jj]};
        if ((tb_qkv_variant<V>::mask >> jj) & 1u) tb_qkv_tile_out<true>(a, b, head, which, tt, lane, bias[jj], v);
        else tb_qkv_tile_out<false>(a, b, head, which, tt, lane, bias[jj], v);
#pragma unroll
        for (int mt = 0; mt < 4; ++mt) acc[mt][jj] = v[mt];
    }
}
template <int V>
__device__ __forceinline__ void tb_qkv_to_lds(unsigned char* HQ, int lane, const f32x4 (&acc)[4][3]) {
#pragma unroll
    for (int jj = 0; jj < 3; ++jj) {
        const int j = 3 * V + jj, which = j >> 2, tt = j & 3;
        const f32x4 v[4] = {acc[0][jj], acc[1][jj], acc[2][jj], acc[3][jj]};
        if ((tb_qkv_variant<V>::mask >> jj) & 1u) tb_qkv_tile_lds<true>(HQ, which, tt, lane, v);
        else tb_qkv_tile_lds<false>(HQ, which, tt, lane, v);
    }
}

template <class PRE, class NEXT>
__device__ __forceinline__ void tb_qkv_round(const tb_fwd_args& a, const unsigned char* AP, unsigned char* HQ, int b, int head, int w, int lane, PRE& pre,
                                             const unsigned short* wpn, NEXT& nxt) {
    f32x4 cur[4][3];
    switch (w & 3) {
        case 0: tb_qkv_pass<0>(a, AP, b, head, lane, cur, pre, wpn, nxt); tb_qkv_to_lds<0>(HQ, lane, cur); break;
        case 1: tb_qkv_pass<1>(a, AP, b, head, lane, cur, pre, wpn, nxt); tb_qkv_to_lds<1>(HQ, lane, cur); break;
        case 2: tb_qkv_pass<2>(a, AP, b, head, lane, cur, pre, wpn, nxt); tb_qkv_to_lds<2>(HQ, lane, cur); break;
        default: tb_qkv_pass<3>(a, AP, b, head, lane, cur, pre, wpn, nxt); tb_qkv_to_lds<3>(HQ, lane, cur); break;
    }
}

template <bool TRAIN>
__device__ __forceinline__ void tb_attention(const tb_fwd_args& a, unsigned char* HQ, int b, int head, int qt, int lane, f32x4 (&c)[4]) {
    const int fr = lane & 15, g = lane >> 4;
    unsigned char* Q = HQ;
    const unsigned char* K = HQ + 2 * TB_HQ_PLANE;
    const unsigned char* VT = HQ + 4 * TB_HQ_PLANE;
    f32x4 s[4];
#pragma unroll
    for (int kt = 0; kt < 4; ++kt) s[kt] = f32x4{0.f, 0.f, 0.f, 0.f};
#pragma unroll
    for (int ks = 0; ks < 2; ++ks) {
        const int qo = hq_off(16 * qt + fr, 32 * ks + 8 * g);
        const bf16x8 qh = *reinterpret_cast<const bf16x8*>(Q + qo), ql = *reinterpret_cast<const bf16x8*>(Q + TB_HQ_PLANE + qo);
#pragma unroll
        for (int kt = 0; kt < 4; ++kt) {
            const int ko = hq_off(16 * kt + fr, 32 * ks + 8 * g);
            const bf16x8 kh = *reinterpret_cast<const bf16x8*>(K + ko), kl = *reinterpret_cast<const bf16x8*>(K + TB_HQ_PLANE + ko);
            s[kt] = mfma_bf16_16x16x32(kl, qh, s[kt]);
            s[kt] = mfma_bf16_16x16x32(kh, ql, s[kt]);
            s[kt] = mfma_bf16_16x16x32(kh, qh, s[kt]);
        }
    }
    float mx = -INFINITY;
#pragma unroll
    for (int kt = 0; kt < 4; ++kt)
#pragma unroll
        for (int i = 0; i < 4; ++i) {
            s[kt][i] *= a.scale;
            mx = fmaxf(mx, s[kt][i]);
        }
    mx = fmaxf(mx, __shfl_xor(mx, 16, 64));
    mx = fmaxf(mx, __shfl_xor(mx, 32, 64));
    float sum = 0.f;
#pragma unroll
    for (int kt = 0; kt < 4; ++kt)
#pragma unroll
        for (int i = 0; i < 4; ++i) {
            s[kt][i] = expf(s[kt][i] - mx);
            sum += s[kt][i];
        }
    sum += __shfl_xor(sum, 16, 64);
    sum += __shfl_xor(sum, 32, 64);
    const float inv = 1.0f / sum;
    const float ksc = (TRAIN && a.drop_p > 0.f) ? 1.f / (1.f - a.drop_p) : 1.f;
    wave_sync();
#pragma unroll
    for (int kt = 0; kt < 4; ++kt) {
        bool keep[4] = {true, true, true, true};
        if (TRAIN && a.drop_p > 0.f) {
            const unsigned long long idx0 = (((unsigned long long)(b * TB_H + head) * TB_L + 16 * qt + fr) * TB_L) + 16 * kt + 4 * g;
            dropout_keep4(a.seed, a.site_attn, idx0, a.drop_p, keep);
        }
        float p[4];
#pragma unroll
        for (int i = 0; i < 4; ++i) p[i] = keep[i] ? s[kt][i] * inv * ksc : 0.f;
        tb_store_planes4(Q, TB_HQ_PLANE, hq_off(16 * qt + fr, 16 * kt + 4 * g), p[0], p[1], p[2], p[3]);
    }
    wave_sync();
#pragma unroll
    for (int dt = 0; dt < 4; ++dt) c[dt] = f32x4{0.f, 0.f, 0.f, 0.f};
#pragma unroll
    for (int ks = 0; ks < 2; ++ks) {
        const int po = hq_off(16 * qt + fr, 32 * ks + 8 * g);
        const bf16x8 ph = *reinterpret_cast<const bf16x8*>(Q + po), pl = *reinterpret_cast<const bf16x8*>(Q + TB_HQ_PLANE + po);
#pragma unroll
        for (int dt = 0; dt < 4; ++dt) {
            const int vo = hq_off(16 * dt + fr, 32 * ks + 8 * g);
            const bf16x8 vh = *reinterpret_cast<const bf16x8*>(VT + vo), vl = *reinterpret_cast<const bf16x8*>(VT + TB_HQ_PLANE + vo);
            c[dt] = mfma_bf16_16x16x32(vl, ph, c[dt]);
            c[dt] = mfma_bf16_16x16x32(vh, pl, c[dt]);
            c[dt] = mfma_bf16_16x16x32(vh, ph, c[dt]);
        }
    }
}

struct tb_rows {
    tb_f2 v[8][2];
};
__device__ __forceinline__ void tb_request_rows(const float* rows, int w, int lane, tb_rows& o) {
#pragma unroll
// ... 308 lines not shown
        f32x4 acc[4][2];
        tb_gemm<2, 3u, 2, true, tb_none, tb_none, false>(AP, p6.packed + TB_OFF_1 + (long long)(2 * w) * TB_KS * TB_TILE, lane, acc, none, nullptr, none);
        f32x4 bias1[2];
#pragma unroll
        for (int j = 0; j < 2; ++j) bias1[j] = *reinterpret_cast<const f32x4*>(p6.b1 + 32 * w + 16 * j + 4 * g);
        tb_for_tiles(w, lane, TB_FF, acc, [&](int m, int n0, int valid, f32x4& v) {
            const f32x4 bias = bias1[(n0 >> 4) & 1];
            const long long ob = (long long)b * (TB_L * TB_FF);
            const unsigned ol = (unsigned)(m * TB_FF + n0);
            f32x4 f, gq;
#pragma unroll
            for (int i = 0; i < 4; ++i) f[i] = v[i] + bias[i];
            if (!(p6.dbg & 1u)) *reinterpret_cast<f32x4*>(p6.f1 + ob + ol) = f;
            bool keep[4] = {true, true, true, true};
            if (TRAIN && p6.drop_p > 0.f) dropout_keep4(p6.seed, p6.site_ffn_act, (unsigned long long)ob + ol, p6.drop_p, keep);
#pragma unroll
            for (int i = 0; i < 4; ++i) {
                const float ge = gelu_erf(f[i]);
                gq[i] = (TRAIN && p6.drop_p > 0.f) ? (keep[i] ? ge * ksc : 0.f) : ge;
            }
            v = gq;
        });
        if (!(p6.dbg & 1u)) tb_planes_out<0>(AP, p6.n1p + (long long)b * (2 * TB_AP_PLANE), t);
        raw_barrier();
#pragma unroll
        for (int p = 0; p < 2; ++p) tb_request(p6.packed + TB_OFF_2 + (long long)(2 * w) * TB_KS * TB_TILE, lane, p, c7);
        tb_for_tiles(w, lane, TB_FF, acc, [&](int m, int n0, int valid, f32x4& v) {
            tb_store_planes4(AP, TB_AP_PLANE, ap_off(m, n0), v[0], v[1], v[2], v[3]);
        });
    }
    raw_barrier();

    tb_stamp(a0, b, t, 7);
    const tb_fwd_args p7 = tb_args_again(a0);
    {
        f32x4 acc[4][2];
        tb_retire(c7);
        tb_gemm<2, 3u, 2, true>(AP, p7.packed + TB_OFF_2 + (long long)(2 * w) * TB_KS * TB_TILE, lane, acc, c7, nullptr, none);
        f32x4 bias2[2];
#pragma unroll
        for (int j = 0; j < 2; ++j) {
            const int n0 = 32 * w + 16 * j + 4 * g;
            bias2[j] = n0 < TB_D ? tb_ld4(p7.b2 + n0, TB_D - n0 >= 4 ? 4 : 2) : f32x4{0.f, 0.f, 0.f, 0.f};
        }
        if (!(p7.dbg & 1u)) tb_planes_out<64>(AP, p7.g1p + (long long)b * (2 * TB_AP_PLANE), t);
        raw_barrier();
#pragma unroll
        for (int j = 0; j < 2; ++j) {
            const int n0 = 32 * w + 16 * j + 4 * g;
            if (n0 >= TB_D) continue;
            const int valid = TB_D - n0 >= 4 ? 4 : TB_D - n0;
#pragma unroll
            for (int mt = 0; mt < 4; ++mt) {
                f32x4 o;
#pragma unroll
                for (int i = 0; i < 4; ++i) o[i] = i < valid ? acc[mt][j][i] + bias2[j][i] : 0.f;
                *reinterpret_cast<f32x4*>(AP + xf_off(16 * mt + fr, n0)) = o;
            }
        }
    }
    raw_barrier();
    tb_stamp(a0, b, t, 8);
    const tb_fwd_args p8 = tb_args_again(a0);
    tb_ln_rows<TRAIN, true>(p8, b, w, lane, AP, XF, nullptr, p8.site_ffn_out, p8.r2, p8.ln2_g, p8.ln2_b, p8.n2, p8.mu2, p8.rs2, p8.ln3_g, p8.ln3_b, p8.n3, p8.mu3, p8.rs3,
                            nullptr, nullptr, none);
    tb_stamp(a0, b, t, 9);
    if (a0.cs_rows) {
        __syncthreads();
        const tb_fwd_args p9 = tb_args_again(a0);
        cs_stats1_sample(lds, p9.n3, (long long)(TB_L * TB_D), (long long)TB_D, p9.cs_w25, p9.cs_bias, p9.cs_rows, b, p9.cs_H, 1);
    }
}


struct tb_bwd_args {
    const unsigned short* packed;
    const float *dn3, *n2, *r2, *r1, *f1, *mu1, *rs1, *mu2, *rs2, *mu3, *rs3, *ln1_g, *ln2_g, *ln2_b, *ln3_g;
    float *dr1, *dctx, *partials;
    unsigned char *df2p, *dg1p, *da1p, *dr1p;
    const unsigned char* dqkvp;
    float drop_p;
    unsigned long long seed;
    unsigned site_embed, site_attn_out, site_ffn_act, site_ffn_out;
};

__device__ __forceinline__ float tb_lane_value(float v, int src) {
#if defined(EEG_EMU)
    return __shfl(v, src, 64);
#else
    return __builtin_bit_cast(float, __builtin_amdgcn_readlane(__builtin_bit_cast(int, v), src));
#endif
}

__device__ __forceinline__ void tb_ln_bwd_row(const float (&dy)[4], const float (&x)[4], const float (&gam)[4], const bool (&ok)[2], float mu, float rs,
                                              float (&dx)[4], float (&pg)[4], float (&pb)[4]) {
    float xh[4], gq[4];
    float s1 = 0.f, s2 = 0.f;
#pragma unroll
    for (int e = 0; e < 4; ++e) {
        xh[e] = ok[e >> 1] ? (x[e] - mu) * rs : 0.f;
        gq[e] = dy[e] * gam[e];
        s1 += gq[e];
        s2 += gq[e] * xh[e];
        pg[e] += dy[e] * xh[e];
        pb[e] += dy[e];
    }
    const float c1 = wave_sum(s1) * (1.0f / (float)TB_D), c2 = wave_sum(s2) * (1.0f / (float)TB_D);
#pragma unroll
    for (int e = 0; e < 4; ++e) dx[e] = ok[e >> 1] ? rs * (gq[e] - c1 - xh[e] * c2) : 0.f;
}

template <int NV, class CARRY>
__device__ __forceinline__ void tb_reduce_partials(float* slab, int w, int lane, int t, const float (&pe)[NV][4], const float (&po)[NV][4], float* out, CARRY& carry) {
    float* mine = slab + w * (NV * 256);
#pragma unroll
    for (int v = 0; v < NV; ++v) *reinterpret_cast<f32x4*>(mine + v * 256 + 4 * lane) = f32x4{pe[v][0], pe[v][1], pe[v][2], pe[v][3]};
    wave_sync();
#pragma unroll
    for (int v = 0; v < NV; ++v)
#pragma unroll
        for (int e = 0; e < 4; ++e) {
            const int c = 4 * lane - 2 + e;
            if (c >= 0) mine[v * 256 + c] += po[v][e];
        }
    raw_barrier();
    tb_retire(carry);
    for (int i = t; i < NV * 256; i += TB_THREADS) {
        float sum = 0.f;
#pragma unroll
        for (int ww = 0; ww < 8; ++ww) sum += slab[ww * (NV * 256) + i];
        out[i] = sum;
    }
}

template <bool TRAIN>
__global__ __launch_bounds__(TB_THREADS, 2) void token_block_bwd_a_kernel(const tb_bwd_args a0) {
    EEG_LDS_BASE(unsigned char, lds);
    unsigned char* const AP = lds;
    unsigned char* const XF = lds + TB_AP_BYTES;
    float* const SC = reinterpret_cast<float*>(lds + TB_AP_BYTES + TB_XF_BYTES);
    const int t = threadIdx.x, lane = t & 63, w = wave_uniform(t >> 6);
    const int b = blockIdx.x;
    const float ksc = (TRAIN && a0.drop_p > 0.f) ? 1.f / (1.f - a0.drop_p) : 1.f;
    tb_none none;
    tb_frags<2> c2, c3, c5;

    const tb_bwd_args q1 = tb_args_again(a0);
    {
        float pe[4][4], po[4][4];
#pragma unroll
        for (int v = 0; v < 4; ++v)
#pragma unroll
            for (int e = 0; e < 4; ++e) { pe[v][e] = 0.f; po[v][e] = 0.f; }
        tb_f2 pg3[2][2], pg2[2][2], pb2[2][2];
#pragma unroll
        for (int par = 0; par < 2; ++par)
#pragma unroll
            for (int p = 0; p < 2; ++p) {
                const int cp = 4 * lane - 2 * par + 2 * p;
                const bool okc = cp >= 0 && cp < TB_D;
                pg3[par][p] = okc ? *reinterpret_cast<const tb_f2*>(q1.ln3_g + cp) : tb_f2{0.f, 0.f};
                pg2[par][p] = okc ? *reinterpret_cast<const tb_f2*>(q1.ln2_g + cp) : tb_f2{0.f, 0.f};
                pb2[par][p] = (okc && !q1.n2) ? *reinterpret_cast<const tb_f2*>(q1.ln2_b + cp) : tb_f2{0.f, 0.f};
            }
        float stat = 0.f;
        if (lane < 32) {
// ... 97 lines not shown
        tb_gemm<2, 3u, 2, true>(AP, q3.packed + TB_OFF_1T + (long long)(2 * w) * TB_KS * TB_TILE, lane, acc, c3, q3.packed + TB_OFF_OT + (long long)(2 * w) * TB_KS * TB_TILE, c5);
        tb_for_tiles(w, lane, TB_D, acc, [&](int m, int n0, int valid, f32x4& v) {
            f32x4* p = reinterpret_cast<f32x4*>(XF + xf_off(m, n0));
            f32x4 o = *p;
#pragma unroll
            for (int i = 0; i < 4; ++i) o[i] = i < valid ? o[i] + v[i] : 0.f;
            *p = o;
        });
        tb_retire(c5);
        tb_planes_out<64>(AP, q3.dg1p + (long long)b * (2 * TB_AP_PLANE), t);
    }
    raw_barrier();

    const tb_bwd_args q4 = tb_args_again(a0);
    {
        int lane4 = lane;
#if !defined(EEG_EMU)
        asm volatile("" : "+v"(lane4));
#endif
        float pe[2][4], po[2][4];
#pragma unroll
        for (int v = 0; v < 2; ++v)
#pragma unroll
            for (int e = 0; e < 4; ++e) { pe[v][e] = 0.f; po[v][e] = 0.f; }
        tb_f2 pg1[2][2], in_r1[8][2];
#pragma unroll
        for (int par = 0; par < 2; ++par)
#pragma unroll
            for (int p = 0; p < 2; ++p) {
                const int cp = 4 * lane4 - 2 * par + 2 * p;
                pg1[par][p] = (cp >= 0 && cp < TB_D) ? *reinterpret_cast<const tb_f2*>(q4.ln1_g + cp) : tb_f2{0.f, 0.f};
            }
#pragma unroll
        for (int rr = 0; rr < 8; ++rr)
#pragma unroll
            for (int p = 0; p < 2; ++p) {
                const int cp = 4 * lane4 - ((rr & 1) ? 2 : 0) + 2 * p;
                in_r1[rr][p] = (cp >= 0 && cp < TB_D) ? *reinterpret_cast<const tb_f2*>(q4.r1 + (long long)b * (TB_L * TB_D) + (unsigned)((8 * w + rr) * TB_D + cp)) : tb_f2{0.f, 0.f};
            }
#pragma unroll
        for (int rr = 0; rr < 8; ++rr) {
            const int r = 8 * w + rr, c0 = 4 * lane4 - ((rr & 1) ? 2 : 0);
            const long long row = (long long)b * TB_L + r, rbase = row * TB_D;
            float dy[4], x1[4], g1[4];
            bool ok[2];
#pragma unroll
            for (int p = 0; p < 2; ++p) {
                const int cp = c0 + 2 * p;
                ok[p] = cp >= 0 && cp < TB_D;
                tb_f2 v0 = tb_f2{0.f, 0.f};
                const tb_f2 v1 = in_r1[rr][p], v2 = pg1[rr & 1][p];
                if (ok[p]) v0 = *reinterpret_cast<const tb_f2*>(XF + xf_off(r, cp));
#pragma unroll
                for (int e = 0; e < 2; ++e) { dy[2 * p + e] = v0[e]; x1[2 * p + e] = v1[e]; g1[2 * p + e] = v2[e]; }
            }
            float dr1[4];
            if (rr & 1) tb_ln_bwd_row(dy, x1, g1, ok, q4.mu1[row], q4.rs1[row], dr1, po[0], po[1]);
            else tb_ln_bwd_row(dy, x1, g1, ok, q4.mu1[row], q4.rs1[row], dr1, pe[0], pe[1]);
            bool keep[4] = {true, true, true, true};
            if (TRAIN && q4.drop_p > 0.f && c0 < TB_D) dropout_keep4(q4.seed, q4.site_attn_out, (unsigned long long)(rbase + c0), q4.drop_p, keep);
#pragma unroll
            for (int p = 0; p < 2; ++p) {
                const int cp = c0 + 2 * p;
                const float d0 = (TRAIN && q4.drop_p > 0.f) ? (keep[2 * p] ? dr1[2 * p] * ksc : 0.f) : dr1[2 * p];
                const float d1 = (TRAIN && q4.drop_p > 0.f) ? (keep[2 * p + 1] ? dr1[2 * p + 1] * ksc : 0.f) : dr1[2 * p + 1];
                if (ok[p]) {
                    *reinterpret_cast<tb_f2*>(q4.dr1 + rbase + (unsigned)cp) = tb_f2{dr1[2 * p], dr1[2 * p + 1]};
                }
                if (cp >= 0 && cp < 256) tb_store_planes2(AP, TB_AP_PLANE, ap_off(r, cp), ok[p] ? d0 : 0.f, ok[p] ? d1 : 0.f);
            }
            if ((rr & 1) && lane4 == 63) tb_store_planes2(AP, TB_AP_PLANE, ap_off(r, 254), 0.f, 0.f);
        }
        raw_barrier();
        tb_reduce_partials<2>(SC, w, lane4, t, pe, po, tb_args_again(a0).partials + (long long)b * (6 * 256) + 4 * 256, none);
    }
    raw_barrier();

    const tb_bwd_args q5 = tb_args_again(a0);
    {
        f32x4 acc[4][2];
        tb_gemm<2, 3u, 2, true>(AP, q5.packed + TB_OFF_OT + (long long)(2 * w) * TB_KS * TB_TILE, lane, acc, c5, nullptr, none);
        tb_for_tiles(w, lane, 256, acc, [&](int m, int n0, int valid, f32x4& v) {
            const int head = n0 >> 6, d0 = n0 & 63;
            if (d0 < TB_E) tb_st4(q5.dctx + (long long)b * (TB_L * TB_HE) + (unsigned)(m * TB_HE + head * TB_E + d0), TB_E - d0 >= 4 ? 4 : 2, v);
        });
        tb_planes_out<64>(AP, q5.da1p + (long long)b * (2 * TB_AP_PLANE), t);
    }
}

template <bool TRAIN>
__global__ __launch_bounds__(TB_THREADS, 2) void token_block_bwd_b_kernel(const tb_bwd_args a) {
    EEG_LDS_BASE(unsigned char, lds);
    unsigned char* const AP = lds;
    unsigned char* const XF = lds + TB_AP_BYTES;
    const int t = threadIdx.x, lane = t & 63, w = wave_uniform(t >> 6);
    const int b = blockIdx.x;
    const float ksc = (TRAIN && a.drop_p > 0.f) ? 1.f / (1.f - a.drop_p) : 1.f;
    f32x4 acc[4][2];
    tb_none none;
    tb_frags<2> ck, cv;
    auto dma_planes = [&](int which, unsigned char* dst) {
        const unsigned char* src = a.dqkvp + ((long long)which * gridDim.x + b) * (2 * TB_AP_PLANE);
#pragma unroll
        for (int i = 0; i < 8; ++i) {
            const int plane = i >> 2, row = 8 * w + 2 * (i & 3) + (lane >> 5), c = lane & 31;
            lds_dma16(dst + plane * TB_AP_PLANE + (8 * w + 2 * (i & 3)) * 512, src + plane * TB_AP_PLANE + row * 512 + ((c ^ (row & 15)) << 4));
        }
    };
    dma_planes(0, AP);
    dma_planes(1, XF);
    wait_vmcnt<8>();
    raw_barrier();
    tb_gemm<2, 3u, 2, true>(AP, a.packed + TB_OFF_QT + (long long)(2 * w) * TB_KS * TB_TILE, lane, acc, none, a.packed + TB_OFF_QT + TB_MAT_ELEMS + (long long)(2 * w) * TB_KS * TB_TILE, ck);
    raw_barrier();
    dma_planes(2, AP);
#pragma unroll
    for (int p = 0; p < 2; ++p) tb_wait_frags<2>(8, ck.h[p], ck.l[p]);
    raw_barrier();
    tb_gemm<2, 3u, 2, false>(XF, a.packed + TB_OFF_QT + TB_MAT_ELEMS + (long long)(2 * w) * TB_KS * TB_TILE, lane, acc, ck, a.packed + TB_OFF_QT + 2 * TB_MAT_ELEMS + (long long)(2 * w) * TB_KS * TB_TILE, cv);
    tb_retire(cv);
    raw_barrier();
    tb_gemm<2, 3u, 2, false>(AP, a.packed + TB_OFF_QT + 2 * TB_MAT_ELEMS + (long long)(2 * w) * TB_KS * TB_TILE, lane, acc, cv, nullptr, none);
    raw_barrier();
    tb_for_tiles(w, lane, TB_D, acc, [&](int m, int n0, int valid, f32x4& v) {
        const f32x4 r = tb_ld4(a.dr1 + (long long)b * (TB_L * TB_D) + (unsigned)(m * TB_D + n0), valid);
        f32x4 o;
#pragma unroll
        for (int i = 0; i < 4; ++i) o[i] = i < valid ? r[i] + v[i] : 0.f;
        *reinterpret_cast<f32x4*>(XF + xf_off(m, n0)) = o;
    });
    __syncthreads();
    float* ob = a.dr1 + (long long)b * (TB_L * TB_D);
#pragma unroll
    for (int j = 0; j < 8; ++j) {
        const int q = t + TB_THREADS * j;
        if (q < TB_L * TB_D / 4) {
            const int i0 = 4 * q, row = i0 / TB_D, col = i0 - TB_D * row;
            const bool wrap = col + 2 >= TB_D;
            const int row2 = wrap ? row + 1 : row, col2 = wrap ? col + 2 - TB_D : col + 2;
            const tb_f2 p0 = *reinterpret_cast<const tb_f2*>(XF + xf_off(row, col)), p1 = *reinterpret_cast<const tb_f2*>(XF + xf_off(row2, col2));
            float v[4] = {p0[0], p0[1], p1[0], p1[1]};
            if (TRAIN && a.drop_p > 0.f) {
                bool keep[4];
                dropout_keep4(a.seed, a.site_embed, (unsigned long long)b * (TB_L * TB_D) + i0, a.drop_p, keep);
#pragma unroll
                for (int e = 0; e < 4; ++e) v[e] = keep[e] ? v[e] * ksc : 0.f;
            }
            *reinterpret_cast<f32x4*>(ob + i0) = f32x4{v[0], v[1], v[2], v[3]};
            if (a.dr1p) {
                tb_store_planes2(AP, TB_AP_PLANE, ap_off(row, col), v[0], v[1]);
                tb_store_planes2(AP, TB_AP_PLANE, ap_off(row2, col2), v[2], v[3]);
            }
        }
    }
    if (a.dr1p) {
        if (t < 128) {
            const int row = t & 63, plane = t >> 6;
#pragma unroll
            for (int k = 250; k < 256; k += 2) *reinterpret_cast<unsigned*>(AP + plane * TB_AP_PLANE + ap_off(row, k)) = 0u;
        }
        raw_barrier();
        tb_planes_out<64>(AP, a.dr1p + (long long)b * (2 * TB_AP_PLANE), t);
    }
}

struct tb_param_args {
    const float* partials;
    float* out[6];
    int B;
};
__global__ __launch_bounds__(256) void token_block_param_reduce_kernel(const tb_param_args a) {
    EEG_LDS_BASE(float, red);
    const int v = blockIdx.y, lane = threadIdx.x & 63, g = threadIdx.x >> 6;
    const int c = blockIdx.x * 64 + lane;
    const int per = (a.B + (int)gridDim.z - 1) / (int)gridDim.z, b0 = (int)blockIdx.z * per, b1 = b0 + per < a.B ? b0 + per : a.B;
    float s = 0.f;
#pragma unroll 4
    for (int b = b0 + g; b < b1; b += 4) s += a.partials[((long long)b * 6 + v) * 256 + c];
    red[g * 64 + lane] = s;
    __syncthreads();
    if (g == 0 && c < TB_D) atomicAdd(a.out[v] + c, (red[lane] + red[64 + lane]) + (red[128 + lane] + red[192 + lane]));
}

}

using namespace eeg;

extern "C" long long eegclip_token_block_packed_bytes(void) { return TB_PACKED_ELEMS * 2; }

extern "C" int eegclip_token_block_pack(const float* wv, const float* wqkv, const float* wo, const float* w1, const float* w2, void* packed, void* stream) {
    if (!wv || !wqkv || !wo || !w1 || !w2 || !packed) return EEGCLIP_EINVAL;
    if (reinterpret_cast<uintptr_t>(packed) & 15u) return EEGCLIP_EALIGN;
    const int tiles = (int)(TB_PACKED_ELEMS / TB_TILE);
    tb_pack_args a{{wv, wqkv, wo, w1, w2, w2, w1, wo, wqkv, wqkv, wqkv}, static_cast<unsigned short*>(packed), tiles, nullptr, nullptr, nullptr, 0};
    EEG_LAUNCH(token_block_pack_kernel, dim3(tiles), dim3(64), 0, stream, a);
    return (int)hipGetLastError();
}

extern "C" int eegclip_weight_prep(const float* wv, const float* wqkv, const float* wo, const float* w1, const float* w2, void* packed, const float* Ws,
                                   void* cs_packed, void* cs_packed_t, int H, void* stream) {
    if (!wv || !wqkv || !wo || !w1 || !w2 || !packed || !Ws || !cs_packed || H < 1 || H > CS_MAXH) return EEGCLIP_EINVAL;
    if ((reinterpret_cast<uintptr_t>(packed) | reinterpret_cast<uintptr_t>(cs_packed) | reinterpret_cast<uintptr_t>(cs_packed_t)) & 15u) return EEGCLIP_EALIGN;
    const int tiles = (int)(TB_PACKED_ELEMS / TB_TILE);
    tb_pack_args a{{wv, wqkv, wo, w1, w2, w2, w1, wo, wqkv, wqkv, wqkv}, static_cast<unsigned short*>(packed), tiles, Ws, static_cast<unsigned char*>(cs_packed),
                   static_cast<unsigned char*>(cs_packed_t), H};
    const int extra = (cs_pack_items(H, cs_packed_t != nullptr) + 63) / 64;
    EEG_LAUNCH(token_block_pack_kernel, dim3(tiles + extra), dim3(64), 0, stream, a);
    return (int)hipGetLastError();
}

namespace eeg {
__global__ __launch_bounds__(64) void token_block_pack_embed_kernel(const float* __restrict__ w0, long long w_stride, unsigned short* __restrict__ out) {
    const int tile = blockIdx.x, s = blockIdx.y;
    const int nt = tile / TB_KS, ks = tile % TB_KS;
    const int lane = threadIdx.x & 63;
    const int n = 16 * nt + (lane & 15), k0 = 32 * ks + 8 * (lane >> 4);
    const float* src = w0 + (long long)s * w_stride;
    unsigned hb[8], lb[8];
#pragma unroll
    for (int e = 0; e < 8; ++e) {
        const long long si = tb_src_index(0, n, k0 + e);
        const float v = si >= 0 ? src[si] : 0.f;
        const unsigned short h = f32_to_bf16_bits(v);
        hb[e] = h;
        lb[e] = f32_to_bf16_bits(v - bf16_bits_to_f32(h));
    }
    unsigned short* dst = out + (long long)s * TB_MAT_ELEMS + (long long)tile * TB_TILE + lane * 8;
    tb_u4 oh, ol;
#pragma unroll
    for (int e = 0; e < 4; ++e) {
        oh[e] = hb[2 * e] | (hb[2 * e + 1] << 16);
        ol[e] = lb[2 * e] | (lb[2 * e + 1] << 16);
    }
    *reinterpret_cast<tb_u4*>(dst) = oh;
    *reinterpret_cast<tb_u4*>(dst + 512) = ol;
}
}

extern "C" long long eegclip_token_block_packed_embed_bytes(int n_subjects) { return n_subjects < 1 ? 0 : (long long)n_subjects * TB_MAT_ELEMS * 2; }

extern "C" int eegclip_token_block_pack_embed(const float* w0, long long w_stride, int n_subjects, void* out, void* stream) {
    if (!w0 || !out || n_subjects < 1 || n_subjects > 65535 || w_stride < (long long)TB_D * TB_T) return EEGCLIP_EINVAL;
    if (reinterpret_cast<uintptr_t>(out) & 15u) return EEGCLIP_EALIGN;
    EEG_LAUNCH(token_block_pack_embed_kernel, dim3(16 * TB_KS, (unsigned)n_subjects), dim3(64), 0, stream, w0, w_stride, static_cast<unsigned short*>(out));
    return (int)hipGetLastError();
}

extern "C" int eegclip_token_block_fwd(const eegclip_token_block_desc* d, void* stream) {
    if (!d || d->B < 1 || !d->x || !d->packed || !d->bv || !d->pe || !d->tokens || !d->bqkv || !d->bo || !d->ln1_g || !d->ln1_b || !d->b1 || !d->b2 ||
        !d->ln2_g || !d->ln2_b || !d->ln3_g || !d->ln3_b || !d->h || !d->qkv || !d->ctxp || !d->r1 || !d->n1p || !d->mu1 || !d->rs1 || !d->f1 || !d->g1p ||
        !d->hp || !d->r2 || !d->mu2 || !d->rs2 || !d->n3 || !d->mu3 || !d->rs3 || d->drop_p < 0.f || d->drop_p >= 1.f)
        return EEGCLIP_EINVAL;
    const uintptr_t al16 = reinterpret_cast<uintptr_t>(d->packed) | reinterpret_cast<uintptr_t>(d->h) | reinterpret_cast<uintptr_t>(d->f1) |
                           reinterpret_cast<uintptr_t>(d->b1) | reinterpret_cast<uintptr_t>(d->xp) | reinterpret_cast<uintptr_t>(d->hp) |
                           reinterpret_cast<uintptr_t>(d->ctxp) | reinterpret_cast<uintptr_t>(d->n1p) | reinterpret_cast<uintptr_t>(d->g1p);
    const uintptr_t al8 = reinterpret_cast<uintptr_t>(d->x) | reinterpret_cast<uintptr_t>(d->qkv) |
                          reinterpret_cast<uintptr_t>(d->r1) | reinterpret_cast<uintptr_t>(d->r2) |
                          reinterpret_cast<uintptr_t>(d->n2) | reinterpret_cast<uintptr_t>(d->n3) | reinterpret_cast<uintptr_t>(d->bv) |
                          reinterpret_cast<uintptr_t>(d->pe) | reinterpret_cast<uintptr_t>(d->tokens) | reinterpret_cast<uintptr_t>(d->bqkv) |
                          reinterpret_cast<uintptr_t>(d->bo) | reinterpret_cast<uintptr_t>(d->b2) | reinterpret_cast<uintptr_t>(d->ln1_g) |
                          reinterpret_cast<uintptr_t>(d->ln1_b) | reinterpret_cast<uintptr_t>(d->ln2_g) | reinterpret_cast<uintptr_t>(d->ln2_b) |
                          reinterpret_cast<uintptr_t>(d->ln3_g) | reinterpret_cast<uintptr_t>(d->ln3_b);
    if ((al16 & 15u) || (al8 & 7u)) return EEGCLIP_EALIGN;
    tb_fwd_args a{d->x, static_cast<const unsigned short*>(d->packed), d->bv, d->pe, d->tokens, d->ids, d->bqkv, d->bo, d->ln1_g, d->ln1_b, d->b1, d->b2,
                  d->ln2_g, d->ln2_b, d->ln3_g, d->ln3_b, d->h, d->qkv, d->r1, d->mu1, d->rs1, d->f1, d->r2, d->n2, d->mu2, d->rs2,
                  d->n3, d->mu3, d->rs3, static_cast<unsigned char*>(d->xp), static_cast<unsigned char*>(d->hp), static_cast<unsigned char*>(d->ctxp),
                  static_cast<unsigned char*>(d->n1p), static_cast<unsigned char*>(d->g1p), d->drop_p, d->eps, d->scale, d->seed, d->site_embed, d->site_attn,
                  d->site_attn_out, d->site_ffn_act, d->site_ffn_out, 0u, nullptr, static_cast<const unsigned short*>(d->packed_embed), d->embed_subject,
                  d->embed_subject ? d->bv_stride : 0, d->cs_w25, d->cs_bias, d->cs_rows, d->cs_H};
    if (d->cs_rows && (!d->cs_w25 || !d->cs_bias || d->cs_H < 1 || d->cs_H > CS_MAXH || (reinterpret_cast<uintptr_t>(d->cs_rows) & 7u))) return EEGCLIP_EINVAL;
    static_assert(CS_LDS_S + CS_LDS_PS <= TB_LDS && CS_NT == TB_THREADS, "the conv stack's statistics pass runs in the block kernel's workgroup");
    if (d->embed_subject && (!d->packed_embed || (reinterpret_cast<uintptr_t>(d->packed_embed) & 15u) || d->bv_stride < 0 || (d->bv_stride & 1))) return EEGCLIP_EINVAL;
    static const unsigned dbg = getenv("EEGCLIP_TB_DEBUG") ? (unsigned)atoi(getenv("EEGCLIP_TB_DEBUG")) : 0u;
    if ((dbg & 1u) && (d->xp || d->hp || d->ctxp || d->n1p || d->g1p)) return EEGCLIP_EINVAL;
    a.dbg = dbg;
    a.tstamp = nullptr;
#if !defined(EEG_EMU)
    static unsigned long long* stamps = nullptr;
    static int calls = 0;
    if ((dbg & 2u) && d->B <= 4096) {
        if (!stamps && hipMalloc(&stamps, 4096 * 16 * sizeof(unsigned long long)) != hipSuccess) stamps = nullptr;
        a.tstamp = stamps;
    }
#endif
    if (d->drop_p > 0.f) EEG_LAUNCH(token_block_fwd_kernel<true>, dim3(d->B), dim3(TB_THREADS), TB_LDS, stream, a);
    else EEG_LAUNCH(token_block_fwd_kernel<false>, dim3(d->B), dim3(TB_THREADS), TB_LDS, stream, a);
#if !defined(EEG_EMU)
    if (a.tstamp && ++calls % 20 == 0) {
        hipStreamSynchronize((hipStream_t)stream);
        static unsigned long long host[4096 * 16];
        hipMemcpy(host, stamps, (size_t)d->B * 16 * sizeof(unsigned long long), hipMemcpyDeviceToHost);
        double ph[9] = {0};
        for (int b = 0; b < d->B; ++b)
            for (int k = 0; k < 9; ++k) ph[k] += (double)(host[b * 16 + k + 1] - host[b * 16 + k]);
        fprintf(stderr, "token_block_fwd phases (s_memtime ticks, mean of %d workgroups): x->planes %.0f | embed GEMM %.0f | dropout+h %.0f | qkv+attention %.0f | out-proj %.0f | "
                        "LN1 %.0f | FFN1 %.0f | FFN2 %.0f | LN2+LN3 %.0f\n", d->B, ph[0] / d->B, ph[1] / d->B, ph[2] / d->B, ph[3] / d->B, ph[4] / d->B, ph[5] / d->B,
                ph[6] / d->B, ph[7] / d->B, ph[8] / d->B);
        double q[4] = {0};
        for (int b = 0; b < d->B; ++b) {
            const unsigned long long* h = host + b * 16;
            q[0] += (double)(h[10] - h[3]); q[1] += (double)(h[11] - h[10]); q[2] += (double)(h[12] - h[11]); q[3] += (double)(h[13] - h[12]);
        }
        fprintf(stderr, "  qkv+attention: qkv(heads 0,1) %.0f | attention %.0f | qkv(heads 2,3) + h planes out %.0f | attention %.0f\n", q[0] / d->B, q[1] / d->B, q[2] / d->B,
                q[3] / d->B);
    }
#endif
    return (int)hipGetLastError();
}

extern "C" long long eegclip_token_block_bwd_workspace_floats(int B) { return B < 1 ? 0 : (long long)B * 6 * 256; }

extern "C" int eegclip_token_block_bwd(const eegclip_token_block_bwd_desc* d, int part, void* stream) {
    if (!d || d->B < 1 || !d->packed || d->drop_p < 0.f || d->drop_p >= 1.f || part < 0 || part > 2) return EEGCLIP_EINVAL;
    tb_bwd_args a{static_cast<const unsigned short*>(d->packed), d->dn3, d->n2, d->r2, d->r1, d->f1, d->mu1, d->rs1, d->mu2, d->rs2, d->mu3, d->rs3,
                  d->ln1_g, d->ln2_g, d->ln2_b, d->ln3_g, d->dr1, d->dctx, d->partials, static_cast<unsigned char*>(d->df2p), static_cast<unsigned char*>(d->dg1p),
                  static_cast<unsigned char*>(d->da1p), static_cast<unsigned char*>(d->dr1p), static_cast<const unsigned char*>(d->dqkvp), d->drop_p, d->seed,
                  d->site_embed, d->site_attn_out, d->site_ffn_act, d->site_ffn_out};
    if (part == 0) {
        if (!d->dn3 || (!d->n2 && !d->ln2_b) || !d->r2 || !d->r1 || !d->f1 || !d->mu1 || !d->rs1 || !d->mu2 || !d->rs2 || !d->mu3 || !d->rs3 || !d->ln1_g || !d->ln2_g ||
            !d->ln3_g || !d->df2p || !d->dg1p || !d->da1p || !d->dr1 || !d->dctx || !d->partials)
            return EEGCLIP_EINVAL;
        const uintptr_t al16 = reinterpret_cast<uintptr_t>(d->packed) | reinterpret_cast<uintptr_t>(d->f1) | reinterpret_cast<uintptr_t>(d->df2p) |
                               reinterpret_cast<uintptr_t>(d->dg1p) | reinterpret_cast<uintptr_t>(d->da1p);
        const uintptr_t al8 = reinterpret_cast<uintptr_t>(d->dn3) | reinterpret_cast<uintptr_t>(d->n2) | reinterpret_cast<uintptr_t>(d->r2) |
                              reinterpret_cast<uintptr_t>(d->r1) | reinterpret_cast<uintptr_t>(d->ln1_g) | reinterpret_cast<uintptr_t>(d->ln2_g) |
                              reinterpret_cast<uintptr_t>(d->ln3_g) | reinterpret_cast<uintptr_t>(d->dr1) | reinterpret_cast<uintptr_t>(d->dctx);
        if ((al16 & 15u) || (al8 & 7u)) return EEGCLIP_EALIGN;
        if (d->drop_p > 0.f) EEG_LAUNCH(token_block_bwd_a_kernel<true>, dim3(d->B), dim3(TB_THREADS), TB_LDS, stream, a);
        else EEG_LAUNCH(token_block_bwd_a_kernel<false>, dim3(d->B), dim3(TB_THREADS), TB_LDS, stream, a);
    } else if (part == 1) {
        if (!d->dqkvp || !d->dr1) return EEGCLIP_EINVAL;
        if ((reinterpret_cast<uintptr_t>(d->packed) | reinterpret_cast<uintptr_t>(d->dr1) | reinterpret_cast<uintptr_t>(d->dqkvp) | reinterpret_cast<uintptr_t>(d->dr1p)) & 15u)
            return EEGCLIP_EALIGN;
        if (d->drop_p > 0.f) EEG_LAUNCH(token_block_bwd_b_kernel<true>, dim3(d->B), dim3(TB_THREADS), TB_AP_BYTES + TB_XF_BYTES, stream, a);
        else EEG_LAUNCH(token_block_bwd_b_kernel<false>, dim3(d->B), dim3(TB_THREADS), TB_AP_BYTES + TB_XF_BYTES, stream, a);
    } else {
        if (!d->partials || !d->dln3_g || !d->dln3_b || !d->dln2_g || !d->dln2_b || !d->dln1_g || !d->dln1_b) return EEGCLIP_EINVAL;
        tb_param_args pa{d->partials, {d->dln3_g, d->dln3_b, d->dln2_g, d->dln2_b, d->dln1_g, d->dln1_b}, d->B};
        EEG_LAUNCH(token_block_param_reduce_kernel, dim3(4, 6, d->B < 16 ? d->B : 16), dim3(256), 256 * sizeof(float), stream, pa);
    }
    return (int)hipGetLastError();
}
```

include/eegclip.h:

```cpp
#ifndef EEGCLIP_H
#define EEGCLIP_H

#ifdef __cplusplus
extern "C" {
#endif

#define EEGCLIP_ABI_VERSION 20
#define EEGCLIP_EINVAL (-1)
#define EEGCLIP_EALIGN (-2)

int eegclip_abi_version(void);

typedef struct {
    long long div, so, si;
} eegclip_dim;

#define EEGCLIP_ACT_NONE 0
#define EEGCLIP_ACT_GELU 1
#define EEGCLIP_ACT_SILU 2
#define EEGCLIP_ACT_GELU_GRAD 3

#define EEGCLIP_PREC_F32 0
#define EEGCLIP_PREC_BF16X3 1

typedef struct {
    int M, N, K;
    const float* A;
    eegclip_dim Am, Ak;
    const float* B;
    eegclip_dim Bk, Bn;
    float* C;
    eegclip_dim Cm, Cn;
    float* Cpre;
    const float* bias_n;
    const float* bias_m;
    const float* R;
    eegclip_dim Rm, Rn;
    float alpha;
    int accumulate;
    int act;
    float drop_p;
    unsigned long long seed;
    unsigned int drop_site;
    int split_k;
    float* rowsum_a;
    int precision;
    float* workspace;
    long long workspace_bytes;
} eegclip_gemm_desc;

typedef struct {
    const float* src;
    void* hi;
    void* lo;
    int rows, cols;
    long long ld_src, ld_out;
    int transpose;
    float* copy;
    long long ld_copy;
} eegclip_split_item;
int eegclip_split_rows(const eegclip_split_item* items, int n, void* stream);
int eegclip_gemm_f32(const eegclip_gemm_desc* d, void* stream);
long long eegclip_gemm_workspace_bytes(const eegclip_gemm_desc* d);
int eegclip_gemm_f32_grouped(const eegclip_gemm_desc* descs, int n, void* stream);

int eegclip_layernorm_fwd(const float* x, const float* gamma, const float* beta, float* y, float* mean, float* rstd,
                          int rows, int cols, float eps, void* stream);
int eegclip_residual_layernorm_fwd(const float* x, const float* resid, float* x_out, float drop_p, unsigned long long seed, unsigned int site,
                                   const float* gamma, const float* beta, float* y, float* mean, float* rstd, const float* gamma2,
                                   const float* beta2, float* y2, float* mean2, float* rstd2, int rows, int cols, float eps, void* stream);
int eegclip_residual_layernorm_fwd_planes(const float* x, const float* resid, float* x_out, float drop_p, unsigned long long seed, unsigned int site,
                                          const float* gamma, const float* beta, float* y, float* mean, float* rstd, const float* gamma2,
                                          const float* beta2, float* y2, float* mean2, float* rstd2, int rows, int cols, float eps, void* y_hi, void* y_lo,
                                          void* stream);
int eegclip_layernorm_bwd(const float* dy, const float* x, const float* gamma, const float* mean, const float* rstd,
                          float* dx, float* dgamma, float* dbeta, int rows, int cols, int accumulate_dx, float* dx_drop, float drop_p,
                          unsigned long long seed, unsigned int site, void* stream);
long long eegclip_layernorm_bwd_full_workspace_floats(int rows, int cols);
int eegclip_layernorm_bwd_full(const float* dy, const float* x, const float* gamma, const float* mean, const float* rstd, float* dx, float* dgamma,
                               float* dbeta, int rows, int cols, int accumulate_dx, float* dx_drop, float drop_p, unsigned long long seed,
                               unsigned int site, float* workspace, void* stream);
long long eegclip_layernorm_bwd_params_workspace_floats(int rows, int cols);
int eegclip_layernorm_bwd_params(const float* dy, const float* x, const float* mean, const float* rstd, float* dgamma, float* dbeta,
                                 int rows, int cols, float* workspace, void* stream);

int eegclip_layernorm_silu_fwd(const float* x, const float* gamma, const float* beta, float* y_ln, float* y_act, float* mean, float* rstd,
                               int rows, int cols, float eps, float drop_p, unsigned long long seed, unsigned int site, void* stream);
int eegclip_silu_bwd(const float* dy, const float* pre, float* dx, long long n, int accumulate, float drop_p, unsigned long long seed,
                     unsigned int site, void* stream);

int eegclip_bn_stats(const float* x, int outer, int C, int inner, double* sums, void* stream);
int eegclip_bn_finalize(const double* sums, double count, float eps, float momentum, int C, float* mean, float* rstd,
                        float* running_mean, float* running_var, int train, long long* num_batches_tracked, void* stream);
int eegclip_bn_finalize_rows(const double* rows, int nrows, double count, float eps, float momentum, int C, float* mean, float* rstd,
                             float* running_mean, float* running_var, long long* num_batches_tracked, double* sums_out, void* stream);
int eegclip_bn_elu_fwd(const float* x, const float* mean, const float* rstd, const float* gamma, const float* beta, float* y,
                       int outer, int C, int inner, float drop_p, unsigned long long seed, unsigned int site, void* stream);
int eegclip_bn_elu_bwd(const float* dz, const float* x, const float* mean, const float* rstd, const float* gamma, const float* beta,
                       double* sums, float* dx, float* dgamma, float* dbeta, int outer, int C, int inner, float drop_p,
                       unsigned long long seed, unsigned int site, void* stream);

int eegclip_bn_elu_bwd_stats(const float* dz, const float* x, const float* mean, const float* rstd, const float* gamma, const float* beta,
                             double* sums, int outer, int C, int inner, float drop_p, unsigned long long seed, unsigned int site, void* stream);
int eegclip_bn_elu_bwd_apply(const float* dz, const float* x, const float* mean, const float* rstd, const float* gamma, const float* beta,
                             const double* sums, const double* sums_local, double count, float* dx, float* dgamma, float* dbeta, int outer, int C, int inner, float drop_p,
                             unsigned long long seed, unsigned int site, void* stream);

int eegclip_embed_finish(float* h, const float* tokens, const long long* ids, int B, int L, int D, float drop_p,
                         unsigned long long seed, unsigned int site, void* stream);
int eegclip_embed_finish_bwd(float* dh, float* dtokens, const long long* ids, int B, int L, int D, float drop_p,
                             unsigned long long seed, unsigned int site, void* stream);

int eegclip_dropout_scale(float* x, long long n, float drop_p, unsigned long long seed, unsigned int site, void* stream);
int eegclip_gelu_bwd(const float* dy, const float* pre, float* dx, long long n, int accumulate, float drop_p,
                     unsigned long long seed, unsigned int site, void* stream);
int eegclip_bias_act(const float* acc, const float* bias_n, float* pre, const float* resid, float* out, int M, int N, int act, float drop_p,
                     unsigned long long seed, unsigned int site, void* stream);
int eegclip_axpby(const float* x, float* y, long long n, float a, float b, void* stream);
int eegclip_reduce_mid(const float* x, int outer, int mid, int inner, float* out, void* stream);
int eegclip_colsum_blocks(const float* x, int nblk, int blk_rows, int row0, int cols, long long blk_stride, float* out, void* stream);
int eegclip_sumsq(const float* x, long long n, double* out, void* stream);
int eegclip_stage_eeg(const double* src, float* dst, long long n_items, int reps, int channels, int T, const int* tidx, int Tw, int mean_reps,
                      void* stream);
int eegclip_gather_rows(float* dst, long long dst_stride, const float* src, long long src_stride, const int* idx, int n, int row_floats,
                        int scatter, void* stream);

int eegclip_adamw_step(float* p, const float* g, float* m, float* v, long long n, float lr, float beta1, float beta2, float eps,
                       float weight_decay, long long step, float grad_scale, const float* grad_scale_dev, void* stream);
int eegclip_adamw_step_zero_grad(float* p, float* g, float* m, float* v, long long n, float lr, float beta1, float beta2, float eps,
                                 float weight_decay, long long step, float grad_scale, const float* grad_scale_dev, void* stream);
int eegclip_clip_scale(const double* sumsq, float max_norm, float* scale_out, void* stream);

int eegclip_timestep_embedding(const float* t, int n, int dim, float* out, void* stream);
int eegclip_ddpm_add_noise(const float* h, const float* noise, const long long* t, const float* sqrt_acp, const float* sqrt_1macp,
                           float* out, int n, int d, void* stream);
int eegclip_ddpm_step(const float* x, const float* eps_c, const float* eps_u, float guidance, float sa, float sb, float c0, float ct,
                      float sigma, const float* noise, float* out, float* out_dup, long long n, void* stream);
int eegclip_prior_stage_infer(const float* x, const float* gamma, const float* beta, const float* skip, float* act_out, const float* te,
                              const float* ce, int ce_rows, float* xin_out, int rows, int cols, float eps, void* stream);
int eegclip_mse_loss_grad(const float* pred, const float* target, long long n, float* loss, float* dpred, void* stream);
int eegclip_mse_loss_grad_scaled(const float* pred, const float* target, long long n, float weight, float* loss, float* dpred, void* stream);

int eegclip_attention_fwd(const float* qkv, float* ctx, int B, int L, int H, int E, int ld, float scale, float drop_p,
                          unsigned long long seed, unsigned int site, void* stream);
int eegclip_attention_bwd(const float* qkv, const float* dctx, float* dqkv, int B, int L, int H, int E, int ld, float scale,
                          float drop_p, unsigned long long seed, unsigned int site, void* stream);
int eegclip_attention_bwd_x3(const float* qkv, const float* dctx, void* dqkv, int dqkv_planes, int B, int L, int H, int E, int ld, float scale,
                          float drop_p, unsigned long long seed, unsigned int site, void* stream);

long long eegclip_tsconv_fwd_workspace_floats(int B, int H);
int eegclip_tsconv_fwd(const float* x, long long xs_b, long long xs_h, const float* w25, const float* bias, float* y, int B, int H,
                       int T, int C, double* sums, float* workspace, void* stream);
long long eegclip_tsconv_bwd_w_workspace_floats(int B, int H);
int eegclip_tsconv_bwd_w(const float* x, long long xs_b, long long xs_h, const float* dy, float* dw25, float* workspace, int B, int H,
                         int T, int C, void* stream);
int eegclip_tsconv_bwd_x(const float* dy, const float* w25, float* dx, long long xs_b, long long xs_h, int B, int H, int T, int C,
                         void* stream);

int eegclip_sconv_fwd(const float* y1, const float* mean, const float* rstd, const float* gamma, const float* beta, const float* Ws,
                      const float* bs, float* y2, double* sums2, int B, int H, int y2_is_zero, float* workspace, void* stream);
long long eegclip_sconv_fwd_workspace_floats(int B);
long long eegclip_sconv_bwd_w_workspace_floats(int B, int H);
int eegclip_sconv_bwd_w(const float* y1, const float* mean, const float* rstd, const float* gamma, const float* beta, const float* dy2,
                        float* dWs, float* workspace, int B, int H, int precision, void* stream);
long long eegclip_sconv_bwd_x_stats_workspace_floats(int B);
int eegclip_sconv_bwd_x_stats(const float* dy2, const float* Ws, const void* WsT_hi, const void* WsT_lo, const float* y1, const float* mean,
                              const float* rstd, const float* gamma, const float* beta, double* sums, float* workspace, int B, int H, void* stream);
int eegclip_sconv_bwd_x_apply(const float* dy2, const float* Ws, const void* WsT_hi, const void* WsT_lo, const float* y1, const float* mean,
                              const float* rstd, const float* gamma, const float* beta, const double* sums, const double* sums_local,
                              double count, float* dy1, float* dgamma, float* dbeta, int B, int H, void* stream);

int eegclip_lse_rows(const float* X, int rows, int cols, long long ld, const float* scale, float* lse, void* stream);
int eegclip_lse_cols(const float* X, int rows, int cols, long long ld, const float* scale, float* lse, void* stream);
int eegclip_infonce_grad(float* X, int rows, int cols, long long ld, int col0, int n_total, const float* scale, const float* lse_r,
                         const float* lse_c, float weight, float* loss, float* dscale, void* stream);
int eegclip_infonce_loss(const float* X, int n, long long ld, const float* scale, const float* lse_r, const float* lse_c, float weight,
                         float* loss, void* stream);

#define EEGCLIP_DT_BF16 0
#define EEGCLIP_DT_F16 1
#define EEGCLIP_DT_F32 2

int eegclip_gemm16(const void* A, long long lda, const void* W, long long ldw, void* C, long long ldc, const void* bias, const void* R, long long ldr,
                   int r_div, int M, int N, int K, int dtype, void* stream);
int eegclip_sampler_step(const void* x, const void* eps_u, const void* eps_c, const void* noise, void* out, void* scaled, float guidance, float cx,
                         float ce, float cn, float in_scale, long long n, int dtype, void* stream);

typedef struct {
    const void* q_hi;
    const void* q_lo;
    const void* k_hi;
    const void* k_lo;
    int col0;
    float weight;
    float* part;
    float* diag;
    float* lse;
    const float* lse_k;
    float* G;
    long long ldg;
    const float* part_k;
    const float* diag_k;
    void *G_hi, *G_lo;
} eegclip_infonce_problem;
int eegclip_split_bf16(const float* x, void* hi, void* lo, long long n, void* stream);
int eegclip_infonce_fused_supported(int n, int N, int D);
long long eegclip_infonce_fused_workspace_floats(int n, int N);
int eegclip_infonce_fused_fwd(const eegclip_infonce_problem* blocks, int n_blocks, int n, int N, int D, int planes, int n_total,
                              const float* scale, float* loss, void* stream);
int eegclip_infonce_fused_grad(const eegclip_infonce_problem* blocks, int n_blocks, int n, int N, int D, int planes, int n_total,
                               const float* scale, float* dscale, void* stream);
int eegclip_infonce_fused_grad_finalize(const eegclip_infonce_problem* blocks, int n_blocks, int n, int N, int D, int planes, int n_total,
                                        const float* scale, float* loss, float* dscale, void* stream);

int eegclip_proj1x1_fwd(const float* y2, const float* mean, const float* rstd, const float* gamma, const float* beta, const float* W,
                        const float* bias, float* z2, float* feat, int B, float drop_p, unsigned long long seed, unsigned int site, void* stream);
int eegclip_proj1x1_fwd_rows(const float* y2, const double* rows, int nrows, double count, float eps, float momentum, float* mean, float* rstd,
                             float* running_mean, float* running_var, long long* num_batches_tracked, const float* gamma, const float* beta, const float* W,
                             const float* bias, float* z2, float* feat, int B, float drop_p, unsigned long long seed, unsigned int site, void* stream);
long long eegclip_proj1x1_bwd_workspace_floats(int B);
int eegclip_proj1x1_bwd(const float* dfeat, const float* z2, const float* W, const float* y2, const float* mean, const float* rstd,
                        const float* gamma, const float* beta, float* dz2, float* dW, float* dbias, double* sums, float* workspace, int B,
                        float drop_p, unsigned long long seed, unsigned int site, void* stream);

int eegclip_cast_bf16(const float* x, void* y_bf16, long long n, void* stream);
int eegclip_logits_bf16(const void* a_bf16, const void* b_bf16, float* c, int M, int N, int K, long long ldc, const float* scale, void* stream);

int eegclip_cross_attn_fwd(const void* q, const void* k, const void* v, const void* k_ip, const void* v_ip, void* out, int B, int HW, int heads,
                           int head_dim, int S, int S_ip, float ip_scale, int dtype, void* stream);

int eegclip_self_attn_supported(int head_dim, long long ldq, long long ldk, long long ldv, long long ldo);
int eegclip_self_attn_fwd(const void* q, long long ldq, const void* k, long long ldk, const void* v, long long ldv, void* out, long long ldo, int B,
                          int Tq, int Tk, int heads, int head_dim, float scale, int dtype, void* stream);
int eegclip_self_attn_causal_fwd(const void* q, long long ldq, const void* k, long long ldk, const void* v, long long ldv, void* out, long long ldo, int B,
                                 int Tq, int Tk, int heads, int head_dim, float scale, int dtype, void* stream);
int eegclip_self_attn_prefix_fwd(const void* q, long long ldq, const void* k, long long ldk, const void* v, long long ldv, void* out, long long ldo, int B,
                                 int T, int prefix, int heads, int head_dim, float scale, int dtype, void* stream);

int eegclip_attn80_supported(long long ldq, long long ldk, long long ldv, long long ldo);
int eegclip_attn80_fwd(const void* q, long long ldq, const void* k, long long ldk, const void* v, long long ldv, void* out, long long ldo, int B, int Tq,
                       int Tk, int heads, float scale, int dtype, void* stream);

int eegclip_topk_rows(const float* X, int rows, int cols, long long ld, int k, const float* scale ,
                      long long* out_idx, void* stream);
int eegclip_count_equal(const long long* pred, int stride, const long long* labels, int n, int* count, void* stream);
int eegclip_top1_count(const float* X, int rows, int cols, long long ld, const float* scale, const long long* labels, int* count, void* stream);

typedef union {
    void* p;
    long long i;
    unsigned long long u;
    double d;
    float f;
    int i32;
    unsigned int u32;
} eegclip_plan_arg;
#define EEGCLIP_PLAN_MAX_ARGS 28
typedef struct {
    int fn;
    int flags;
    eegclip_plan_arg a[EEGCLIP_PLAN_MAX_ARGS];
} eegclip_plan_op;
#define EEGCLIP_PLAN_MEMSET (-2)
#define EEGCLIP_PLAN_JOIN (-3)
#define EEGCLIP_PLAN_SIDE 1
#define EEGCLIP_PLAN_SKIP 2
#define EEGCLIP_PLAN_SIDE2 4
int eegclip_plan_fn_id(const char* name);
int eegclip_plan_events(int n, void** out);
int eegclip_plan_events_destroy(int n, void* const* events);
int eegclip_plan_run(const eegclip_plan_op* ops, int begin, int end, int n_total, void* main_stream, void* side_stream, void* side_stream2,
                     void* const* events, void* join_event, void* join_event2, int* dirty, int* failed);

typedef struct {
    int B;
    const float* x;
    const void* packed;
    const float *bv, *pe, *tokens;
    const long long* ids;
    const float *bqkv, *bo, *ln1_g, *ln1_b, *b1, *b2, *ln2_g, *ln2_b, *ln3_g, *ln3_b;
    float *h, *qkv, *r1, *mu1, *rs1, *f1, *r2, *n2, *mu2, *rs2, *n3, *mu3, *rs3;
    void *xp, *hp, *ctxp, *n1p, *g1p;
    float drop_p, eps, scale;
    unsigned long long seed;
    unsigned int site_embed, site_attn, site_attn_out, site_ffn_act, site_ffn_out;
    const void* packed_embed;
    const int* embed_subject;
    long long bv_stride;
    const float *cs_w25, *cs_bias;
    double* cs_rows;
    int cs_H;
} eegclip_token_block_desc;
long long eegclip_token_block_packed_bytes(void);
int eegclip_token_block_pack(const float* wv, const float* wqkv, const float* wo, const float* w1, const float* w2, void* packed, void* stream);
int eegclip_weight_prep(const float* wv, const float* wqkv, const float* wo, const float* w1, const float* w2, void* packed, const float* Ws, void* cs_packed,
                        void* cs_packed_t, int H, void* stream);
long long eegclip_token_block_packed_embed_bytes(int n_subjects);
int eegclip_token_block_pack_embed(const float* w0, long long w_stride, int n_subjects, void* out, void* stream);
int eegclip_token_block_fwd(const eegclip_token_block_desc* d, void* stream);

typedef struct {
    int B;
    const void* packed;
    const float *dn3, *n2, *r2, *r1, *f1, *mu1, *rs1, *mu2, *rs2, *mu3, *rs3, *ln1_g, *ln2_g, *ln2_b, *ln3_g;
    float *dr1, *dctx, *partials;
    void *df2p, *dg1p, *da1p, *dr1p;
    const void* dqkvp;
    float *dln3_g, *dln3_b, *dln2_g, *dln2_b, *dln1_g, *dln1_b;
    float drop_p;
    unsigned long long seed;
    unsigned int site_embed, site_attn_out, site_ffn_act, site_ffn_out;
} eegclip_token_block_bwd_desc;
long long eegclip_token_block_bwd_workspace_floats(int B);
int eegclip_token_block_bwd(const eegclip_token_block_bwd_desc* d, int part, void* stream);

typedef struct {
    const void *a_hi, *a_lo, *b_hi, *b_lo;
    long long lda, ldb;
    int M, N, K;
    float* C;
    long long ldc;
    float* Cpre;
    long long ldcpre;
    const float* bias;
    const float* R;
    long long ldr;
    void *p_hi, *p_lo;
    long long ldp;
    int act, accumulate, planes_of;
} eegclip_gemm_planes_desc;
int eegclip_gemm_planes(const eegclip_gemm_planes_desc* d, void* stream);

int eegclip_split_transpose(const eegclip_split_item* items, int n, void* stream);

int eegclip_infonce_small_supported(int n, int T);
long long eegclip_infonce_small_workspace_floats(int n, int T);
int eegclip_infonce_small_fwd(const float* slabs, int nslabs, long long slab_stride, int n, int T, const float* scale, float* workspace, void* stream);
int eegclip_infonce_small_grad(int n, int T, const float* scale, const float* workspace, float w0, float w1, float w2, float w3, void* g_hi, void* g_lo,
                               long long ldg, float* loss, float* dscale, void* stream);

typedef struct {
    const void* in;
    const void* W;
    void* out;
    const void* bias;
    const void* residual;
    int N, Hi, Wi, Cin, in_pad;
    int Ho, Wo, Cout, out_pad;
    int KS, stride, pad_top, pad_left, upsample, dtype;
    const void* chan_bias;
} eegclip_conv16_desc;
int eegclip_conv16(const eegclip_conv16_desc* d, void* stream);
int eegclip_groupnorm16(const void* x, int N, int H, int W, int C, int pad, int groups, const void* gamma, const void* beta, float eps, int silu, void* y,
                        int out_pad, double* sums, int dtype, void* stream);
int eegclip_softmax_rows16(void* s, int rows, int cols, long long ld, float scale, int dtype, void* stream);
int eegclip_vae_sample16(const void* moments, const void* noise, void* z, long long pixels, int latent_channels, int dtype, void* stream);

int eegclip_vae_attn_supported(int head_dim, long long ldq, long long ldk, long long ldv, long long ldo);
int eegclip_vae_attn_fwd(const void* q, long long ldq, const void* k, long long ldk, const void* v, long long ldv, void* out, long long ldo, int B, int T,
                         int head_dim, float scale, int dtype, void* stream);

int eegclip_layernorm16(const void* x, long long ldx, const void* gamma, const void* beta, void* y, long long ldy, int rows, int C, float eps, int dtype,
                        void* stream);
int eegclip_geglu16(const void* x, void* y, int M, int D, int dtype, void* stream);
int eegclip_concat16(const void* a, const void* b, void* out, int N, int H, int W, int pad, int Ca, int Cb, int out_pad, int dtype, void* stream);

int eegclip_gather_rows16(const void* table, long long table_rows, const void* idx, int idx64, const void* add, int add_rows, void* out, int rows, int C,
                          int dtype, void* stream);
int eegclip_act16(const void* x, long long ldx, void* y, long long ldy, int M, int D, int kind, int dtype, void* stream);

int eegclip_patch_rows16(const void* pixels, int pix_dtype, const float* scale, const float* shift, void* out, int B, int H, int W, int patch, int dtype,
                         void* stream);
int eegclip_embed_ln16(const void* x, long long ldx, const void* pos, int T, const void* gamma, const void* beta, void* y, long long ldy, int rows, int C, float eps,
                       int dtype, void* stream);

#define EEGCLIP_SRC_U8_HWC 3
#define EEGCLIP_RESIZE_BILINEAR 2
#define EEGCLIP_RESIZE_BICUBIC 3
int eegclip_resize_coeffs(int in_size, int out_size, int first, int count, int filter, int* bounds, int* coeffs, int ksize);
int eegclip_resize_crop_normalize(const void* src, int src_kind, float a, float b, int B, int H, int W, int rh, int rw, int top, int left, int ch, int cw,
                                  int filter, const int* hbounds, const int* hcoeffs, int kh, const int* vbounds, const int* vcoeffs, int kv, const float* scale,
                                  const float* shift, void* out, int dtype, void* stream);

int eegclip_gemm16_skinny(const void* A, long long lda, const void* W, long long ldw, void* C, long long ldc, const void* bias, const void* R, long long ldr,
                          int M, int N, int K, int c_f32, int dtype, void* stream);
int eegclip_decode_attn16(const void* q, long long ldq, const void* kv, long long ld_row, long long sample_stride, void* out, long long ldo, int B, int Tk,
                          int heads, int head_dim, float scale, int dtype, void* stream);

typedef struct {
    const void* in;
    const void* W;
    void* out;
    const float* scale;
    const float* shift;
// ... 217 lines not shown
```

Baseline: 406,300 samples/s.

## Pass qkv and dctx to attention backward as pre-split bf16 planes

The fused token-block forward now writes Q/K/V directly as hi/lo bf16 planes (V transposed), and the backward block writes dctx as planes, instead of storing f32 tensors. The attention backward kernel gains a planes-input mode that copies these planes straight into LDS without per-element f32-to-bf16x3 splitting, and reads V through a transposed fragment loader. This is meant to cut global traffic and conversion work in attention backward. In exchange it adds buffer aliasing logic, a slow fallback path for reading f32 back out of the saved planes, and ABI changes.

```diff
diff --git a/eeg_image_decode_amd/_abi.py b/eeg_image_decode_amd/_abi.py
--- a/eeg_image_decode_amd/_abi.py
+++ b/eeg_image_decode_amd/_abi.py
@@ -48,7 +48,7 @@
                 + [("drop_p", C.c_float), ("eps", C.c_float), ("scale", C.c_float), ("seed", C.c_ulonglong)]
                 + [(k, C.c_uint) for k in ("site_embed", "site_attn", "site_attn_out", "site_ffn_act", "site_ffn_out")]
                 + [("packed_embed", C.c_void_p), ("embed_subject", C.c_void_p), ("bv_stride", C.c_longlong)]
-                + [("cs_w25", C.c_void_p), ("cs_bias", C.c_void_p), ("cs_rows", C.c_void_p), ("cs_H", C.c_int)])
+                + [("cs_w25", C.c_void_p), ("cs_bias", C.c_void_p), ("cs_rows", C.c_void_p), ("cs_H", C.c_int), ("qkvp", C.c_void_p)])
 
 
 class TokenBlockBwdDesc(C.Structure):
@@ -57,7 +57,8 @@
                 + [(k, C.c_void_p) for k in ("dr1", "dctx", "partials", "df2p", "dg1p", "da1p", "dr1p", "dqkvp")]
                 + [(k, C.c_void_p) for k in ("dln3_g", "dln3_b", "dln2_g", "dln2_b", "dln1_g", "dln1_b")]
                 + [("drop_p", C.c_float), ("seed", C.c_ulonglong)]
-                + [(k, C.c_uint) for k in ("site_embed", "site_attn_out", "site_ffn_act", "site_ffn_out")])
+                + [(k, C.c_uint) for k in ("site_embed", "site_attn_out", "site_ffn_act", "site_ffn_out")]
+                + [("dctxp", C.c_void_p)])
 
 
 class GemmPlanesDesc(C.Structure):
@@ -151,7 +152,7 @@
 
 ACT_NONE, ACT_GELU, ACT_SILU, ACT_GELU_GRAD = 0, 1, 2, 3
 PREC_F32, PREC_BF16X3 = 0, 1
-ABI_VERSION = 20
+ABI_VERSION = 21
 DT_BF16, DT_F16, DT_F32 = 0, 1, 2
 SRC_U8_HWC, RESIZE_BILINEAR, RESIZE_BICUBIC = 3, 2, 3
 _P, _I, _F, _L, _U64, _U, _D = C.c_void_p, C.c_int, C.c_float, C.c_longlong, C.c_ulonglong, C.c_uint, C.c_double
diff --git a/eeg_image_decode_amd/atms.py b/eeg_image_decode_amd/atms.py
--- a/eeg_image_decode_amd/atms.py
+++ b/eeg_image_decode_amd/atms.py
@@ -418,8 +418,25 @@
                 b[n] = torch.empty((3, B, 2, L_TOK, 256) if n == "dqkvp" else (B, 2, L_TOK, 256), dtype=torch.bfloat16, device=self.device)
         return [_p(b[n]) for n in names]
 
+    def _attn_io(self, b, B, name, planes):
+        key = name + (":planes" if planes else ":f32")
+        if key not in b:
+            if planes:
+                b[key] = torch.empty((3, B, 2, L_TOK, 256) if name == "qkv" else (B, 2, L_TOK, 256), dtype=torch.bfloat16, device=self.device)
+            else:
+                b[key] = torch.empty(B * L_TOK, 3 * HE if name == "qkv" else HE, dtype=torch.float32, device=self.device)
+        b[name] = b[key]
+        return _p(b[key])
+
     def saved_f32(self, B, name):
         b = self.bufs[B]
+        if name in ("qkv", "dctx") and b[name].dtype == torch.bfloat16:
+            t = b[name].to(torch.float32)
+            v = t[..., 0, :, :] + t[..., 1, :, :]
+            if name == "qkv":
+                v = torch.stack([v[0], v[1], v[2].reshape(B, 256, L_TOK).transpose(1, 2)])
+            v = v.reshape(*v.shape[:-1], N_HEADS, 64)[..., :D_HEAD].reshape(*v.shape[:-1], HE)
+            return v.permute(1, 2, 0, 3).reshape(B * L_TOK, 3 * HE) if name == "qkv" else v.reshape(B * L_TOK, HE)
         key = name + "p"
         if key not in b:
             return b[name]
@@ -447,7 +464,7 @@
 
         R = B * L_TOK
         b = dict(
-            h=f(B, L_TOK, D_MODEL), qkv=f(R, 3 * HE), ctx=f(R, HE), r1=f(R, D_MODEL), n1=f(R, D_MODEL), mu1=f(R), rs1=f(R),
+            h=f(B, L_TOK, D_MODEL), ctx=f(R, HE), r1=f(R, D_MODEL), n1=f(R, D_MODEL), mu1=f(R), rs1=f(R),
             f1=f(R, D_FF), g1=f(R, D_FF), r2=f(R, D_MODEL), n2=f(R, D_MODEL), mu2=f(R), rs2=f(R), n3=f(B, L_TOK, D_MODEL), mu3=f(R), rs3=f(R),
             z2=f(B, C_TS, W_TS),
             feat=f(B, F_TS), u=f(B, P_DIM), gu=f(B, P_DIM), s=f(B, P_DIM), out=f(B, P_DIM), mu4=f(B), rs4=f(B),
@@ -478,7 +495,7 @@
         b.update(ds=f(B, P_DIM), dv=f(B, P_DIM), dz2=f(B, C_TS, W_TS), dy2=f(B, C_TS, W_TS),
                  dn3=torch.zeros(B, L_TOK, D_MODEL, dtype=torch.float32, device=dev),
                  dn2=f(R, D_MODEL), dr2=f(R, D_MODEL), df2=f(R, D_MODEL), dg1=f(R, D_FF), dr1=f(R, D_MODEL), da1=f(R, D_MODEL),
-                 dctx=f(R, HE), dqkv=f(R, 3 * HE))
+                 dqkv=f(R, 3 * HE))
 
     def _build_fwd(self, B, train, shared, probs):
         P, b = self.P, self.bufs[B]
@@ -535,7 +552,7 @@
                 bqkv=_p(P[_LY + "attention.query_projection.bias"]), bo=_p(P[_LY + "attention.out_projection.bias"]), ln1_g=_p(P[_LY + "norm1.weight"]),
                 ln1_b=_p(P[_LY + "norm1.bias"]), b1=_p(P[_LY + "conv1.bias"]), b2=_p(P[_LY + "conv2.bias"]), ln2_g=_p(P[_LY + "norm2.weight"]),
                 ln2_b=_p(P[_LY + "norm2.bias"]), ln3_g=_p(P["encoder.encoder.norm.weight"]), ln3_b=_p(P["encoder.encoder.norm.bias"]),
-                h=_p(b["h"]), qkv=_p(b["qkv"]), r1=_p(b["r1"]), mu1=_p(b["mu1"]), rs1=_p(b["rs1"]), f1=_p(b["f1"]),
+                h=_p(b["h"]), qkv=None, qkvp=self._attn_io(b, B, "qkv", True), r1=_p(b["r1"]), mu1=_p(b["mu1"]), rs1=_p(b["rs1"]), f1=_p(b["f1"]),
                 r2=_p(b["r2"]), n2=None, mu2=_p(b["mu2"]), rs2=_p(b["rs2"]), n3=_p(b["n3"]), mu3=_p(b["mu3"]), rs3=_p(b["rs3"]),
                 xp=xp, hp=hp, ctxp=ctxp, n1p=n1p, g1p=g1p,
                 drop_p=pe_, eps=EPS, scale=1.0 / math.sqrt(D_HEAD), seed=0, site_embed=SITE_EMBED, site_attn=SITE_ATTN, site_attn_out=SITE_ATTN_OUT,
@@ -558,6 +575,7 @@
                         N_CH * D_MODEL, 1)
             tok = P[_TOK_SHARED] if shared else P[_TOK_TABLE]
             pl.call("eegclip_embed_finish", _p(b["h"]), _p(tok), None if shared else _p(b["ids"]), B, L_TOK, D_MODEL, pe_, 0, SITE_EMBED, seed_at=7)
+            self._attn_io(b, B, "qkv", False)
             pl.gemm(R, 3 * HE, D_MODEL, _p(b["h"]), D(D_MODEL), D(1), _p(P[_LY + "attention.query_projection.weight"]), D(1), D(D_MODEL),
                     _p(b["qkv"]), D(3 * HE), D(1), bias_n=_p(P[_LY + "attention.query_projection.bias"]))
             pl.call("eegclip_attention_fwd", _p(b["qkv"]), _p(b["ctx"]), B, L_TOK, N_HEADS, D_HEAD, 3 * HE, 1.0 / math.sqrt(D_HEAD), pe_, 0,
@@ -850,7 +868,7 @@
                 B=B, packed=_p(self.tb_packed), dn3=_p(b["dn3"]), n2=None, r2=_p(b["r2"]), r1=_p(b["r1"]), f1=_p(b["f1"]), mu1=_p(b["mu1"]),
                 rs1=_p(b["rs1"]), mu2=_p(b["mu2"]), rs2=_p(b["rs2"]), mu3=_p(b["mu3"]), rs3=_p(b["rs3"]), ln1_g=_p(P[_LY + "norm1.weight"]),
                 ln2_g=_p(P[_LY + "norm2.weight"]), ln2_b=_p(P[_LY + "norm2.bias"]), ln3_g=_p(P["encoder.encoder.norm.weight"]),
-                dr1=_p(b["dr1"]), dctx=_p(b["dctx"]), partials=_p(b["tb_part"]), df2p=df2p, dg1p=dg1p, da1p=da1p, dr1p=dr1p, dqkvp=dqkvp,
+                dr1=_p(b["dr1"]), dctx=None, dctxp=self._attn_io(b, B, "dctx", True), partials=_p(b["tb_part"]), df2p=df2p, dg1p=dg1p, da1p=da1p, dr1p=dr1p, dqkvp=dqkvp,
                 dln3_g=_p(G["encoder.encoder.norm.weight"]), dln3_b=_p(G["encoder.encoder.norm.bias"]), dln2_g=_p(G[_LY + "norm2.weight"]),
                 dln2_b=_p(G[_LY + "norm2.bias"]), dln1_g=_p(G[_LY + "norm1.weight"]), dln1_b=_p(G[_LY + "norm1.bias"]),
                 drop_p=pe_, seed=0, site_embed=SITE_EMBED, site_attn_out=SITE_ATTN_OUT, site_ffn_act=SITE_FFN_ACT, site_ffn_out=SITE_FFN_OUT)
@@ -891,7 +909,7 @@
                 late += ffn_out
             else:
                 wgrad_tok("ffn_out", ffn_out)
-            pl.call(attn_bwd, _p(b["qkv"]), _p(b["dctx"]), dqkvp, 1, B, L_TOK, N_HEADS, D_HEAD, 3 * HE, 1.0 / math.sqrt(D_HEAD),
+            pl.call(attn_bwd, self._attn_io(b, B, "qkv", True), _p(b["dctx"]), dqkvp, 3, B, L_TOK, N_HEADS, D_HEAD, 3 * HE, 1.0 / math.sqrt(D_HEAD),
                     pe_, 0, SITE_ATTN, seed_at=11)
             if merge >= 1:
                 late += qkv_w
@@ -909,6 +927,8 @@
             wgrad(_LY + "conv1.weight", _p(b["dg1"]), D_FF, _p(b["n1"]), D_MODEL, D_FF, D_MODEL, R, bias=_LY + "conv1.bias")
             pl.gemm(R, D_MODEL, D_FF, _p(b["dg1"]), D(D_FF), D(1), _p(P[_LY + "conv1.weight"]), D(D_MODEL), D(1), _p(b["dr2"]), D(D_MODEL), D(1),
                     accumulate=1)
+            self._attn_io(b, B, "qkv", False)
+            self._attn_io(b, B, "dctx", False)
             pl.call("eegclip_layernorm_bwd_full", _p(b["dr2"]), _p(b["r1"]), _p(P[_LY + "norm1.weight"]), _p(b["mu1"]), _p(b["rs1"]), _p(b["dr1"]),
                     _p(G[_LY + "norm1.weight"]), _p(G[_LY + "norm1.bias"]), R, D_MODEL, 0, _p(b["da1"]), pe_, 0, SITE_ATTN_OUT, lnf_ws, seed_at=13)
             wgrad(_LY + "attention.out_projection.weight", _p(b["da1"]), D_MODEL, _p(b["ctx"]), HE, D_MODEL, HE, R,
diff --git a/eeg_image_decode_amd/csrc/attention_x3.hip b/eeg_image_decode_amd/csrc/attention_x3.hip
--- a/eeg_image_decode_amd/csrc/attention_x3.hip
+++ b/eeg_image_decode_amd/csrc/attention_x3.hip
@@ -10,6 +10,8 @@
 struct ax_args {
     const float* qkv;
     const float* dctx;
+    const unsigned char* qkvp;
+    const unsigned char* dctxp;
     float* dqkv;
     unsigned char* dqkvp;
     int B, H, E, ld;
@@ -55,7 +57,7 @@
     *reinterpret_cast<u32x2_t*>(row_base + 32768 + 2 * e0) = lo;
 }
 
-template <bool TRAIN>
+template <bool TRAIN, bool PIN>
 __global__ __launch_bounds__(256, 2) void attention_bwd_x3_kernel(const ax_args a) {
     EEG_LDS_BASE(float, ldsf);
     unsigned char* lds = reinterpret_cast<unsigned char*>(ldsf);
@@ -66,10 +68,29 @@
     const int t = threadIdx.x, lane = t & 63, w = wave_uniform(t >> 6), fr = lane & 15, g = lane >> 4;
     const int bh = blockIdx.x, b = bh / a.H, h = bh - b * a.H;
     const int E = a.E, HE = a.H * E;
-    const float* qrow0 = a.qkv + (long long)b * AX_L * a.ld + h * E;
-    const float* orow0 = a.dctx + (long long)b * AX_L * HE + h * E;
-
-    {
+    if (PIN) {
+        typedef unsigned ax_u4 __attribute__((ext_vector_type(4)));
+        const long long grp = (long long)a.B * 65536;
+        const unsigned char* blk = a.qkvp + (long long)b * 65536;
+        const unsigned char* src[4] = {blk + 128 * h, blk + grp + 128 * h, blk + 2 * grp + 8192 * h, a.dctxp + (long long)b * 65536 + 128 * h};
+        ax_u4 v[4][4];
+#pragma unroll
+        for (int x = 0; x < 4; ++x)
+#pragma unroll
+            for (int j = 0; j < 4; ++j) {
+                const int idx = t + 256 * j, plane = idx >> 9, row = (idx >> 3) & 63, c = idx & 7;
+                v[x][j] = *reinterpret_cast<const ax_u4*>(src[x] + plane * 32768 + row * (x == 2 ? 128 : 512) + 16 * c);
+            }
+#pragma unroll
+        for (int x = 0; x < 4; ++x)
+#pragma unroll
+            for (int j = 0; j < 4; ++j) {
+                const int idx = t + 256 * j, plane = idx >> 9, row = (idx >> 3) & 63, c = idx & 7;
+                *reinterpret_cast<ax_u4*>(lds + x * AX_TENSOR + plane * AX_PLANE + row * AX_RS + 16 * c) = v[x][j];
+            }
+    } else {
+        const float* qrow0 = a.qkv + (long long)b * AX_L * a.ld + h * E;
+        const float* orow0 = a.dctx + (long long)b * AX_L * HE + h * E;
         ax_f2 v[4][8];
 #pragma unroll
         for (int j = 0; j < 8; ++j) {
@@ -106,7 +127,8 @@
 #pragma unroll
         for (int kt = 0; kt < 4; ++kt) {
             const bf16x8 kh = ax_frag(Kp, 16 * kt + fr, k0), kl = ax_frag(Kp + AX_PLANE, 16 * kt + fr, k0);
-            const bf16x8 vh = ax_frag(Vp, 16 * kt + fr, k0), vl = ax_frag(Vp + AX_PLANE, 16 * kt + fr, k0);
+            const bf16x8 vh = PIN ? ax_tr_frag(Vp, k0, k0 + 4, 16 * kt, lane) : ax_frag(Vp, 16 * kt + fr, k0);
+            const bf16x8 vl = PIN ? ax_tr_frag(Vp + AX_PLANE, k0, k0 + 4, 16 * kt, lane) : ax_frag(Vp + AX_PLANE, 16 * kt + fr, k0);
             s[kt] = ax_mfma3(kh, kl, qh, ql, s[kt]);
             dp[kt] = ax_mfma3(vh, vl, oh, ol, dp[kt]);
         }
@@ -251,16 +273,26 @@
 
 using namespace eeg;
 
-extern "C" int eegclip_attention_bwd_x3(const float* qkv, const float* dctx, void* dqkv, int dqkv_planes, int B, int L, int H, int E, int ld, float scale,
+extern "C" int eegclip_attention_bwd_x3(const void* qkv, const void* dctx, void* dqkv, int flags, int B, int L, int H, int E, int ld, float scale,
                                         float drop_p, unsigned long long seed, unsigned site, void* stream) {
-    if (dqkv_planes && (H > 4 || (reinterpret_cast<uintptr_t>(dqkv) & 15u))) return dqkv && H <= 4 ? EEGCLIP_EALIGN : EEGCLIP_EINVAL;
+    const bool pout = flags & 1, pin = flags & 2;
+    if (flags & ~3) return EEGCLIP_EINVAL;
+    if (pout && (H > 4 || (reinterpret_cast<uintptr_t>(dqkv) & 15u))) return dqkv && H <= 4 ? EEGCLIP_EALIGN : EEGCLIP_EINVAL;
     if (!qkv || !dctx || !dqkv || B < 1 || L != AX_L || H < 1 || E < 2 || E > 64 || (E & 1) || (ld & 1) || ld < 3 * H * E || drop_p < 0.f || drop_p >= 1.f)
         return EEGCLIP_EINVAL;
-    if ((reinterpret_cast<uintptr_t>(qkv) | reinterpret_cast<uintptr_t>(dctx) | reinterpret_cast<uintptr_t>(dqkv)) & 7u) return EEGCLIP_EALIGN;
-    const ax_args a{qkv, dctx, dqkv_planes ? nullptr : static_cast<float*>(dqkv), dqkv_planes ? static_cast<unsigned char*>(dqkv) : nullptr, B, H, E, ld, scale,
-                    drop_p, seed, site};
+    if (pin && H > 4) return EEGCLIP_EINVAL;
+    if ((reinterpret_cast<uintptr_t>(qkv) | reinterpret_cast<uintptr_t>(dctx)) & (pin ? 15u : 7u)) return EEGCLIP_EALIGN;
+    if (reinterpret_cast<uintptr_t>(dqkv) & 7u) return EEGCLIP_EALIGN;
+    const ax_args a{pin ? nullptr : static_cast<const float*>(qkv), pin ? nullptr : static_cast<const float*>(dctx),
+                    pin ? static_cast<const unsigned char*>(qkv) : nullptr, pin ? static_cast<const unsigned char*>(dctx) : nullptr,
+                    pout ? nullptr : static_cast<float*>(dqkv), pout ? static_cast<unsigned char*>(dqkv) : nullptr, B, H, E, ld, scale, drop_p, seed, site};
     const size_t lds = 4 * AX_TENSOR;
-    if (drop_p > 0.f) EEG_LAUNCH(attention_bwd_x3_kernel<true>, dim3(B * H), dim3(256), lds, stream, a);
-    else              EEG_LAUNCH(attention_bwd_x3_kernel<false>, dim3(B * H), dim3(256), lds, stream, a);
+    if (drop_p > 0.f) {
+        if (pin) EEG_LAUNCH((attention_bwd_x3_kernel<true, true>), dim3(B * H), dim3(256), lds, stream, a);
+        else     EEG_LAUNCH((attention_bwd_x3_kernel<true, false>), dim3(B * H), dim3(256), lds, stream, a);
+    } else {
+        if (pin) EEG_LAUNCH((attention_bwd_x3_kernel<false, true>), dim3(B * H), dim3(256), lds, stream, a);
+        else     EEG_LAUNCH((attention_bwd_x3_kernel<false, false>), dim3(B * H), dim3(256), lds, stream, a);
+    }
     return (int)hipGetLastError();
 }
diff --git a/eeg_image_decode_amd/csrc/token_block.hip b/eeg_image_decode_amd/csrc/token_block.hip
--- a/eeg_image_decode_amd/csrc/token_block.hip
+++ b/eeg_image_decode_amd/csrc/token_block.hip
@@ -234,6 +234,20 @@
     *reinterpret_cast<unsigned*>(hi_plane + plane_stride + off) = x3_pack2(r0, r1);
 }
 
+__device__ __forceinline__ void tb_store_planes8_global(unsigned char* row_hi, int plane_stride, int g, f32x4 a, f32x4 b) {
+    u32x2_t ha, la, hb, lb;
+    x3_split4(a[0], a[1], a[2], a[3], ha, la);
+    x3_split4(b[0], b[1], b[2], b[3], hb, lb);
+    const bool odd = g & 1;
+    const u32x2_t sh = odd ? ha : hb, sl = odd ? la : lb;
+    const unsigned rh0 = __shfl_xor(sh[0], 16, 64), rh1 = __shfl_xor(sh[1], 16, 64), rl0 = __shfl_xor(sl[0], 16, 64), rl1 = __shfl_xor(sl[1], 16, 64);
+    const tb_u4 H = odd ? tb_u4{rh0, rh1, hb[0], hb[1]} : tb_u4{ha[0], ha[1], rh0, rh1};
+    const tb_u4 Lo = odd ? tb_u4{rl0, rl1, lb[0], lb[1]} : tb_u4{la[0], la[1], rl0, rl1};
+    const int off = odd ? 32 + 8 * (g - 1) : 8 * g;
+    *reinterpret_cast<tb_u4*>(row_hi + off) = H;
+    *reinterpret_cast<tb_u4*>(row_hi + plane_stride + off) = Lo;
+}
+
 __device__ __forceinline__ f32x4 tb_ld4(const float* p, int valid) {
     if (valid >= 4) {
         const tb_f4u t = *reinterpret_cast<const tb_f4u*>(p);
@@ -283,6 +297,7 @@
     const float *cs_w25, *cs_bias;
     double* cs_rows;
     int cs_H;
+    unsigned char* qkvp;
 };
 
 template <class ARGS>
@@ -313,7 +328,7 @@
             const int m = 16 * mt + fr;
 #pragma unroll
             for (int i = 0; i < 4; ++i) v[mt][i] = i < valid ? v[mt][i] + bias[i] : 0.f;
-            if (!(a.dbg & 1u)) tb_st4(a.qkv + (long long)b * (TB_L * 3 * TB_HE) + (unsigned)(m * (3 * TB_HE) + cbase + d0), valid, v[mt]);
+            if (a.qkv && !(a.dbg & 1u)) tb_st4(a.qkv + (long long)b * (TB_L * 3 * TB_HE) + (unsigned)(m * (3 * TB_HE) + cbase + d0), valid, v[mt]);
         }
     } else {
         const int d = 16 * tt + fr;
@@ -322,24 +337,37 @@
 #pragma unroll
             for (int i = 0; i < 4; ++i) {
                 v[mt][i] = d < TB_E ? v[mt][i] + bias[0] : 0.f;
-                if (d < TB_E && !(a.dbg & 1u)) (a.qkv + (long long)b * (TB_L * 3 * TB_HE))[(unsigned)((16 * mt + 4 * g + i) * (3 * TB_HE) + cbase + d)] = v[mt][i];
+                if (d < TB_E && a.qkv && !(a.dbg & 1u)) (a.qkv + (long long)b * (TB_L * 3 * TB_HE))[(unsigned)((16 * mt + 4 * g + i) * (3 * TB_HE) + cbase + d)] = v[mt][i];
             }
     }
 }
 template <bool TRANS>
-__device__ __forceinline__ void tb_qkv_tile_lds(unsigned char* HQ, int which, int tt, int lane, const f32x4 (&v)[4]) {
+__device__ __forceinline__ void tb_qkv_tile_lds(unsigned char* HQ, unsigned char* gp, int head, int which, int tt, int lane, const f32x4 (&v)[4]) {
     const int fr = lane & 15, g = lane >> 4;
     unsigned char* base = HQ + which * (2 * TB_HQ_PLANE);
+    if (gp) gp += TRANS ? fr * 512 + 128 * head + 2 * (16 * tt + 4 * g) : (64 * head + 16 * tt + fr) * 128;
+    if (!TRANS && gp) {
+        tb_store_planes8_global(gp, TB_AP_PLANE, g, v[0], v[1]);
+        tb_store_planes8_global(gp + 64, TB_AP_PLANE, g, v[2], v[3]);
+    }
 #pragma unroll
     for (int mt = 0; mt < 4; ++mt) {
         const int off = TRANS ? hq_off(16 * mt + fr, 16 * tt + 4 * g) : hq_off(16 * tt + fr, 16 * mt + 4 * g);
-        tb_store_planes4(base, TB_HQ_PLANE, off, v[mt][0], v[mt][1], v[mt][2], v[mt][3]);
+        u32x2_t h, l;
+        x3_split4(v[mt][0], v[mt][1], v[mt][2], v[mt][3], h, l);
+        *reinterpret_cast<u32x2_t*>(base + off) = h;
+        *reinterpret_cast<u32x2_t*>(base + TB_HQ_PLANE + off) = l;
+        if (TRANS && gp) {
+            *reinterpret_cast<u32x2_t*>(gp + mt * 8192) = h;
+            *reinterpret_cast<u32x2_t*>(gp + TB_AP_PLANE + mt * 8192) = l;
+        }
     }
 }
 
 template <int V>
 struct tb_qkv_variant {
     static constexpr unsigned mask = V == 0 ? 7u : V == 1 ? 7u : V == 2 ? 3u : 0u;
+    static constexpr int pair = V == 0 ? 0 : V == 1 ? 1 : V == 2 ? 0 : -1;
 };
 
 template <int V, class PRE, class NEXT>
@@ -372,13 +400,22 @@
     }
 }
 template <int V>
-__device__ __forceinline__ void tb_qkv_to_lds(unsigned char* HQ, int lane, const f32x4 (&acc)[4][3]) {
+__device__ __forceinline__ void tb_qkv_to_lds(const tb_fwd_args& a, unsigned char* HQ, int b, int head, int lane, const f32x4 (&acc)[4][3]) {
 #pragma unroll
     for (int jj = 0; jj < 3; ++jj) {
         const int j = 3 * V + jj, which = j >> 2, tt = j & 3;
         const f32x4 v[4] = {acc[0][jj], acc[1][jj], acc[2][jj], acc[3][jj]};
-        if ((tb_qkv_variant<V>::mask >> jj) & 1u) tb_qkv_tile_lds<true>(HQ, which, tt, lane, v);
-        else tb_qkv_tile_lds<false>(HQ, which, tt, lane, v);
+        const bool paired = tb_qkv_variant<V>::pair >= 0 && (jj == tb_qkv_variant<V>::pair || jj == tb_qkv_variant<V>::pair + 1);
+        unsigned char* gp = a.qkvp && !paired ? a.qkvp + ((long long)which * gridDim.x + b) * (2 * TB_AP_PLANE) : nullptr;
+        if ((tb_qkv_variant<V>::mask >> jj) & 1u) tb_qkv_tile_lds<true>(HQ, gp, head, which, tt, lane, v);
+        else tb_qkv_tile_lds<false>(HQ, gp, head, which, tt, lane, v);
+    }
+    constexpr int PJ = tb_qkv_variant<V>::pair;
+    if (PJ >= 0 && a.qkvp) {
+        const int j = 3 * V + PJ, which = j >> 2, tt = j & 3, fr = lane & 15, g = lane >> 4;
+        unsigned char* row = a.qkvp + ((long long)which * gridDim.x + b) * (2 * TB_AP_PLANE) + fr * 512 + 128 * head + 32 * tt;
+#pragma unroll
+        for (int mt = 0; mt < 4; ++mt) tb_store_planes8_global(row + mt * 8192, TB_AP_PLANE, g, acc[mt][PJ > 0 ? PJ : 0], acc[mt][PJ + 1]);
     }
 }
 
@@ -387,10 +424,10 @@
                                              const unsigned short* wpn, NEXT& nxt) {
     f32x4 cur[4][3];
     switch (w & 3) {
-        case 0: tb_qkv_pass<0>(a, AP, b, head, lane, cur, pre, wpn, nxt); tb_qkv_to_lds<0>(HQ, lane, cur); break;
-        case 1: tb_qkv_pass<1>(a, AP, b, head, lane, cur, pre, wpn, nxt); tb_qkv_to_lds<1>(HQ, lane, cur); break;
-        case 2: tb_qkv_pass<2>(a, AP, b, head, lane, cur, pre, wpn, nxt); tb_qkv_to_lds<2>(HQ, lane, cur); break;
-        default: tb_qkv_pass<3>(a, AP, b, head, lane, cur, pre, wpn, nxt); tb_qkv_to_lds<3>(HQ, lane, cur); break;
+        case 0: tb_qkv_pass<0>(a, AP, b, head, lane, cur, pre, wpn, nxt); tb_qkv_to_lds<0>(a, HQ, b, head, lane, cur); break;
+        case 1: tb_qkv_pass<1>(a, AP, b, head, lane, cur, pre, wpn, nxt); tb_qkv_to_lds<1>(a, HQ, b, head, lane, cur); break;
+        case 2: tb_qkv_pass<2>(a, AP, b, head, lane, cur, pre, wpn, nxt); tb_qkv_to_lds<2>(a, HQ, b, head, lane, cur); break;
+        default: tb_qkv_pass<3>(a, AP, b, head, lane, cur, pre, wpn, nxt); tb_qkv_to_lds<3>(a, HQ, b, head, lane, cur); break;
     }
 }
 
@@ -865,6 +902,7 @@
     float drop_p;
     unsigned long long seed;
     unsigned site_embed, site_attn_out, site_ffn_act, site_ffn_out;
+    unsigned char* dctxp;
 };
 
 __device__ __forceinline__ float tb_lane_value(float v, int src) {
@@ -1128,8 +1166,13 @@
         tb_gemm<2, 3u, 2, true>(AP, q5.packed + TB_OFF_OT + (long long)(2 * w) * TB_KS * TB_TILE, lane, acc, c5, nullptr, none);
         tb_for_tiles(w, lane, 256, acc, [&](int m, int n0, int valid, f32x4& v) {
             const int head = n0 >> 6, d0 = n0 & 63;
-            if (d0 < TB_E) tb_st4(q5.dctx + (long long)b * (TB_L * TB_HE) + (unsigned)(m * TB_HE + head * TB_E + d0), TB_E - d0 >= 4 ? 4 : 2, v);
+            if (q5.dctx && d0 < TB_E) tb_st4(q5.dctx + (long long)b * (TB_L * TB_HE) + (unsigned)(m * TB_HE + head * TB_E + d0), TB_E - d0 >= 4 ? 4 : 2, v);
         });
+        if (q5.dctxp) {
+            unsigned char* row = q5.dctxp + (long long)b * (2 * TB_AP_PLANE) + (lane & 15) * 512 + 64 * w;
+#pragma unroll
+            for (int mt = 0; mt < 4; ++mt) tb_store_planes8_global(row + mt * 8192, TB_AP_PLANE, lane >> 4, acc[mt][0], acc[mt][1]);
+        }
         tb_planes_out<64>(AP, q5.da1p + (long long)b * (2 * TB_AP_PLANE), t);
     }
 }
@@ -1294,12 +1337,13 @@
 
 extern "C" int eegclip_token_block_fwd(const eegclip_token_block_desc* d, void* stream) {
     if (!d || d->B < 1 || !d->x || !d->packed || !d->bv || !d->pe || !d->tokens || !d->bqkv || !d->bo || !d->ln1_g || !d->ln1_b || !d->b1 || !d->b2 ||
-        !d->ln2_g || !d->ln2_b || !d->ln3_g || !d->ln3_b || !d->h || !d->qkv || !d->ctxp || !d->r1 || !d->n1p || !d->mu1 || !d->rs1 || !d->f1 || !d->g1p ||
+        !d->ln2_g || !d->ln2_b || !d->ln3_g || !d->ln3_b || !d->h || (!d->qkv && !d->qkvp) || !d->ctxp || !d->r1 || !d->n1p || !d->mu1 || !d->rs1 || !d->f1 || !d->g1p ||
         !d->hp || !d->r2 || !d->mu2 || !d->rs2 || !d->n3 || !d->mu3 || !d->rs3 || d->drop_p < 0.f || d->drop_p >= 1.f)
         return EEGCLIP_EINVAL;
     const uintptr_t al16 = reinterpret_cast<uintptr_t>(d->packed) | reinterpret_cast<uintptr_t>(d->h) | reinterpret_cast<uintptr_t>(d->f1) |
                            reinterpret_cast<uintptr_t>(d->b1) | reinterpret_cast<uintptr_t>(d->xp) | reinterpret_cast<uintptr_t>(d->hp) |
-                           reinterpret_cast<uintptr_t>(d->ctxp) | reinterpret_cast<uintptr_t>(d->n1p) | reinterpret_cast<uintptr_t>(d->g1p);
+                           reinterpret_cast<uintptr_t>(d->ctxp) | reinterpret_cast<uintptr_t>(d->n1p) | reinterpret_cast<uintptr_t>(d->g1p) |
+                           reinterpret_cast<uintptr_t>(d->qkvp);
     const uintptr_t al8 = reinterpret_cast<uintptr_t>(d->x) | reinterpret_cast<uintptr_t>(d->qkv) |
                           reinterpret_cast<uintptr_t>(d->r1) | reinterpret_cast<uintptr_t>(d->r2) |
                           reinterpret_cast<uintptr_t>(d->n2) | reinterpret_cast<uintptr_t>(d->n3) | reinterpret_cast<uintptr_t>(d->bv) |
@@ -1313,12 +1357,12 @@
                   d->n3, d->mu3, d->rs3, static_cast<unsigned char*>(d->xp), static_cast<unsigned char*>(d->hp), static_cast<unsigned char*>(d->ctxp),
                   static_cast<unsigned char*>(d->n1p), static_cast<unsigned char*>(d->g1p), d->drop_p, d->eps, d->scale, d->seed, d->site_embed, d->site_attn,
                   d->site_attn_out, d->site_ffn_act, d->site_ffn_out, 0u, nullptr, static_cast<const unsigned short*>(d->packed_embed), d->embed_subject,
-                  d->embed_subject ? d->bv_stride : 0, d->cs_w25, d->cs_bias, d->cs_rows, d->cs_H};
+                  d->embed_subject ? d->bv_stride : 0, d->cs_w25, d->cs_bias, d->cs_rows, d->cs_H, static_cast<unsigned char*>(d->qkvp)};
     if (d->cs_rows && (!d->cs_w25 || !d->cs_bias || d->cs_H < 1 || d->cs_H > CS_MAXH || (reinterpret_cast<uintptr_t>(d->cs_rows) & 7u))) return EEGCLIP_EINVAL;
     static_assert(CS_LDS_S + CS_LDS_PS <= TB_LDS && CS_NT == TB_THREADS, "the conv stack's statistics pass runs in the block kernel's workgroup");
     if (d->embed_subject && (!d->packed_embed || (reinterpret_cast<uintptr_t>(d->packed_embed) & 15u) || d->bv_stride < 0 || (d->bv_stride & 1))) return EEGCLIP_EINVAL;
     static const unsigned dbg = getenv("EEGCLIP_TB_DEBUG") ? (unsigned)atoi(getenv("EEGCLIP_TB_DEBUG")) : 0u;
-    if ((dbg & 1u) && (d->xp || d->hp || d->ctxp || d->n1p || d->g1p)) return EEGCLIP_EINVAL;
+    if ((dbg & 1u) && (d->xp || d->hp || d->ctxp || d->n1p || d->g1p || d->qkvp)) return EEGCLIP_EINVAL;
     a.dbg = dbg;
     a.tstamp = nullptr;
 #if !defined(EEG_EMU)
@@ -1361,13 +1405,13 @@
     tb_bwd_args a{static_cast<const unsigned short*>(d->packed), d->dn3, d->n2, d->r2, d->r1, d->f1, d->mu1, d->rs1, d->mu2, d->rs2, d->mu3, d->rs3,
                   d->ln1_g, d->ln2_g, d->ln2_b, d->ln3_g, d->dr1, d->dctx, d->partials, static_cast<unsigned char*>(d->df2p), static_cast<unsigned char*>(d->dg1p),
                   static_cast<unsigned char*>(d->da1p), static_cast<unsigned char*>(d->dr1p), static_cast<const unsigned char*>(d->dqkvp), d->drop_p, d->seed,
-                  d->site_embed, d->site_attn_out, d->site_ffn_act, d->site_ffn_out};
+                  d->site_embed, d->site_attn_out, d->site_ffn_act, d->site_ffn_out, static_cast<unsigned char*>(d->dctxp)};
     if (part == 0) {
         if (!d->dn3 || (!d->n2 && !d->ln2_b) || !d->r2 || !d->r1 || !d->f1 || !d->mu1 || !d->rs1 || !d->mu2 || !d->rs2 || !d->mu3 || !d->rs3 || !d->ln1_g || !d->ln2_g ||
-            !d->ln3_g || !d->df2p || !d->dg1p || !d->da1p || !d->dr1 || !d->dctx || !d->partials)
+            !d->ln3_g || !d->df2p || !d->dg1p || !d->da1p || !d->dr1 || (!d->dctx && !d->dctxp) || !d->partials)
             return EEGCLIP_EINVAL;
         const uintptr_t al16 = reinterpret_cast<uintptr_t>(d->packed) | reinterpret_cast<uintptr_t>(d->f1) | reinterpret_cast<uintptr_t>(d->df2p) |
-                               reinterpret_cast<uintptr_t>(d->dg1p) | reinterpret_cast<uintptr_t>(d->da1p);
+                               reinterpret_cast<uintptr_t>(d->dg1p) | reinterpret_cast<uintptr_t>(d->da1p) | reinterpret_cast<uintptr_t>(d->dctxp);
         const uintptr_t al8 = reinterpret_cast<uintptr_t>(d->dn3) | reinterpret_cast<uintptr_t>(d->n2) | reinterpret_cast<uintptr_t>(d->r2) |
                               reinterpret_cast<uintptr_t>(d->r1) | reinterpret_cast<uintptr_t>(d->ln1_g) | reinterpret_cast<uintptr_t>(d->ln2_g) |
                               reinterpret_cast<uintptr_t>(d->ln3_g) | reinterpret_cast<uintptr_t>(d->dr1) | reinterpret_cast<uintptr_t>(d->dctx);
diff --git a/include/eegclip.h b/include/eegclip.h
--- a/include/eegclip.h
+++ b/include/eegclip.h
@@ -5,7 +5,7 @@
 extern "C" {
 #endif
 
-#define EEGCLIP_ABI_VERSION 20
+#define EEGCLIP_ABI_VERSION 21
 #define EEGCLIP_EINVAL (-1)
 #define EEGCLIP_EALIGN (-2)
 
@@ -145,7 +145,7 @@
                           unsigned long long seed, unsigned int site, void* stream);
 int eegclip_attention_bwd(const float* qkv, const float* dctx, float* dqkv, int B, int L, int H, int E, int ld, float scale,
                           float drop_p, unsigned long long seed, unsigned int site, void* stream);
-int eegclip_attention_bwd_x3(const float* qkv, const float* dctx, void* dqkv, int dqkv_planes, int B, int L, int H, int E, int ld, float scale,
+int eegclip_attention_bwd_x3(const void* qkv, const void* dctx, void* dqkv, int flags, int B, int L, int H, int E, int ld, float scale,
                           float drop_p, unsigned long long seed, unsigned int site, void* stream);
 
 long long eegclip_tsconv_fwd_workspace_floats(int B, int H);
@@ -290,6 +290,7 @@
     const float *cs_w25, *cs_bias;
     double* cs_rows;
     int cs_H;
+    void* qkvp;
 } eegclip_token_block_desc;
 long long eegclip_token_block_packed_bytes(void);
 int eegclip_token_block_pack(const float* wv, const float* wqkv, const float* wo, const float* w1, const float* w2, void* packed, void* stream);
@@ -310,6 +311,7 @@
     float drop_p;
     unsigned long long seed;
     unsigned int site_embed, site_attn_out, site_ffn_act, site_ffn_out;
+    void* dctxp;
 } eegclip_token_block_bwd_desc;
 long long eegclip_token_block_bwd_workspace_floats(int B);
 int eegclip_token_block_bwd(const eegclip_token_block_bwd_desc* d, int part, void* stream);
```

Result: no change. 407,400 samples/s (median of 2 runs) (+0.3%).
